# google/speedy

Hardware: AMD Instinct MI355X
Metric: Msamples/s processed (16 kHz mono, 3.5x nonlinear) (higher is better)
Workload: dtype int16 samples; f64 DFT, f32 features, int32 AMDF/OLA

## Files before the change

include/speedy_hip.h:

```cpp
#ifndef SPEEDY_HIP_H_
#define SPEEDY_HIP_H_
#include <stddef.h>
#include <stdint.h>
#ifdef __cplusplus
extern "C" {
#endif

#ifndef SPX_FEATURE_COUNT
#define SPX_FEATURE_COUNT 15
#endif

typedef struct spx_plan* spx_plan_t;

typedef struct {
  int64_t in_off;
  int64_t n_in;
  int64_t out_off;
  int64_t out_cap;
  int32_t channels;
  float speed;
  float nonlinear;
  float feedback;
} spx_stream_job;

typedef struct {
  float* tension;
  float* speed;
  float* features;
  float* spectrogram;
  float* normalized;
} spx_taps;

const char* spx_last_error(void);
int spx_abi_version(void);

spx_plan_t spx_plan_create(int sample_rate, int match_matlab);
void spx_plan_destroy(spx_plan_t plan);
int spx_plan_frame_step(spx_plan_t plan);
int spx_plan_window_size(spx_plan_t plan);
int spx_plan_fft_size(spx_plan_t plan);
int spx_plan_future(spx_plan_t plan);
int spx_plan_max_required(spx_plan_t plan);
int64_t spx_plan_frames(spx_plan_t plan, int64_t n_in);
int64_t spx_plan_out_capacity(spx_plan_t plan, int64_t n_in, float speed);
int64_t spx_plan_out_capacity_for(spx_plan_t plan, int64_t n_in, float speed, float nonlinear);

size_t spx_batch_workspace_bytes(spx_plan_t plan, const spx_stream_job* jobs, int n_streams);

int spx_batch_run(spx_plan_t plan, const spx_stream_job* jobs, int n_streams, const int16_t* in,
                  int16_t* out, int64_t* n_out, void* workspace, size_t workspace_bytes,
                  const spx_taps* taps, void* hip_stream);

int spx_batch_run_rate(spx_plan_t plan, const spx_stream_job* jobs, const float* rates, int n_streams, const int16_t* in,
                       int16_t* out, int64_t* n_out, void* workspace, size_t workspace_bytes,
                       const spx_taps* taps, void* hip_stream);
size_t spx_batch_workspace_bytes_rate(spx_plan_t plan, const spx_stream_job* jobs, const float* rates, int n_streams);
int64_t spx_plan_out_capacity_rate(spx_plan_t plan, int64_t n_in, float speed, float nonlinear, float rate);

int spx_batch_run_ahead(spx_plan_t plan, const spx_stream_job* jobs, int n_streams, const int16_t* in,
                        int16_t* out, int64_t* n_out, void* workspace, size_t workspace_bytes,
                        const spx_taps* taps, void* hip_stream);

int spx_batch_run_overlapped(spx_plan_t plan, const spx_stream_job* jobs, int n_streams, const int16_t* in,
                             int16_t* out, int64_t* n_out, void* workspace, size_t workspace_bytes,
                             const spx_taps* taps, void* hip_stream);

int spx_batch_run_ahead_when(spx_plan_t plan, const spx_stream_job* jobs, int n_streams, const int16_t* in,
                             int16_t* out, int64_t* n_out, void* workspace, size_t workspace_bytes,
                             const spx_taps* taps, void* hip_stream, void* in_ready_event);

typedef struct spx_pipeline* spx_pipeline_t;
#define SPX_PIPELINE_DEVICE_OUT 1u
spx_pipeline_t spx_pipeline_create(spx_plan_t plan, const spx_stream_job* jobs, int n_streams, int depth, unsigned flags);
spx_pipeline_t spx_pipeline_create_mixed(const spx_plan_t* plans, int n_plans, const spx_stream_job* jobs, const int* plan_index,
                                         int n_streams, int depth, unsigned flags);
void spx_pipeline_destroy(spx_pipeline_t p);
int spx_pipeline_depth(spx_pipeline_t p);
size_t spx_pipeline_input_values(spx_pipeline_t p);
int16_t* spx_pipeline_host_input(spx_pipeline_t p);
int64_t spx_pipeline_submit(spx_pipeline_t p, const int16_t* in, int in_is_device);
int spx_pipeline_input_consumed(spx_pipeline_t p, int64_t ticket);
int spx_pipeline_wait(spx_pipeline_t p, int64_t ticket, const int16_t** out, const int64_t** offsets, const int64_t** counts);
void* spx_host_alloc(size_t bytes);
void spx_host_free(void* p);

int spx_batch_analyze(spx_plan_t plan, const spx_stream_job* jobs, int n_streams, const int16_t* in,
                      void* workspace, size_t workspace_bytes, const spx_taps* taps, void* hip_stream);
int spx_batch_walk(spx_plan_t plan, const spx_stream_job* jobs, int n_streams, const int16_t* in,
                   int16_t* out, int64_t* n_out, void* workspace, size_t workspace_bytes,
                   const spx_taps* taps, void* hip_stream);

size_t spx_batch_workspace_bytes_mixed(const spx_plan_t* plans, int n_plans, const spx_stream_job* jobs,
                                       const int* plan_index, int n_streams);
int spx_batch_run_mixed(const spx_plan_t* plans, int n_plans, const spx_stream_job* jobs, const int* plan_index,
                        int n_streams, const int16_t* in, int16_t* out, int64_t* n_out, void* workspace,
                        size_t workspace_bytes, void* hip_stream);

int spx_batch_run_mixed_taps(const spx_plan_t* plans, int n_plans, const spx_stream_job* jobs, const int* plan_index,
                             int n_streams, const int16_t* in, int16_t* out, int64_t* n_out, void* workspace,
                             size_t workspace_bytes, const spx_taps* taps, void* hip_stream);
int spx_batch_run_mixed_ahead(const spx_plan_t* plans, int n_plans, const spx_stream_job* jobs, const int* plan_index,
                              int n_streams, const int16_t* in, int16_t* out, int64_t* n_out, void* workspace,
                              size_t workspace_bytes, void* hip_stream);

void spx_set_timing(int enabled);
void spx_set_pipeline_chunks(int chunks);
void spx_set_concurrent(int on);
int spx_timing_collect(double* sum_ms_analyze, double* sum_ms_walk, int* n_calls);
const char* spx_batch_kernel_names(spx_plan_t plan, int n_streams, int max_channels, int speedup_only);
const char* spx_batch_kernel_names_lean(spx_plan_t plan, int n_streams, int max_channels, int speedup_only);
int spx_debug_last_walk_form(void);
int spx_debug_kernel_vgprs(int which);
int spx_debug_walk_info(int sample_rate, int channels, int n_streams, int speedup_only, int short_jobs, int lean, int* out5);
int spx_debug_analysis_info(int sample_rate, int* out4);
int spx_debug_mode_resources(int sample_rate, int channels, int n_streams, int speedup_only, long long* out22);
long long spx_debug_fdiv_check(unsigned seed, unsigned denominators, int exp_lo, int exp_hi);
long long spx_debug_xfade_check(int n_lo, int n_hi);
long long spx_debug_arith_check(unsigned seed, unsigned threads, unsigned per_thread);
int spx_debug_log_check(unsigned first_block, unsigned end_block, unsigned long long* sums);
int spx_debug_last_call_concurrent(void);
double spx_timing_last_tension_ms(void);
double spx_timing_last_rate_ms(void);

int spx_batch_read_steps(spx_plan_t plan, const spx_stream_job* jobs, int n_streams, const void* workspace,
                         int32_t* steps, void* hip_stream);
int spx_batch_read_steps_mixed(const spx_plan_t* plans, int n_plans, const spx_stream_job* jobs, const int* plan_index,
                               int n_streams, const void* workspace, int32_t* steps, void* hip_stream);

void* spx_device_alloc(size_t bytes);
void spx_device_free(void* p);
int spx_batch_pack_outputs(const spx_stream_job* jobs, int n_streams, const int16_t* out, const int64_t* n_out,
                           int16_t* packed, int64_t* offsets, void* hip_stream);
int spx_copy_to_device(void* dst, const void* src, size_t bytes, void* hip_stream);
int spx_copy_to_host(void* dst, const void* src, size_t bytes, void* hip_stream);
int spx_stream_synchronize(void* hip_stream);

#ifdef __cplusplus
}
#endif
#endif
```

speedy_amd/_lib.py:

```python
import ctypes as C
import os
import subprocess

_HERE = os.path.dirname(os.path.abspath(__file__))
LIB_PATH = os.environ.get("SPEEDY_HIP_LIB") or os.path.join(_HERE, "lib", "libspeedy_hip.so")
_LIB = None

c_short_p = C.POINTER(C.c_short)
c_float_p = C.POINTER(C.c_float)
c_int64_p = C.POINTER(C.c_int64)


class StreamJob(C.Structure):
    _fields_ = [("in_off", C.c_int64), ("n_in", C.c_int64), ("out_off", C.c_int64), ("out_cap", C.c_int64),
                ("channels", C.c_int32), ("speed", C.c_float), ("nonlinear", C.c_float), ("feedback", C.c_float)]


class Taps(C.Structure):
    _fields_ = [("tension", C.c_void_p), ("speed", C.c_void_p), ("features", C.c_void_p),
                ("spectrogram", C.c_void_p), ("normalized", C.c_void_p)]


TENSION_FN = C.CFUNCTYPE(None, C.c_void_p, C.c_int, C.c_float)
FEATURES_FN = C.CFUNCTYPE(None, C.c_void_p, C.c_int, c_float_p)

SYMBOLS = {
    "spx_last_error": (C.c_char_p, []),
    "spx_abi_version": (C.c_int, []),
    "spx_plan_create": (C.c_void_p, [C.c_int, C.c_int]),
    "spx_plan_destroy": (None, [C.c_void_p]),
    "spx_plan_frame_step": (C.c_int, [C.c_void_p]),
    "spx_plan_window_size": (C.c_int, [C.c_void_p]),
    "spx_plan_fft_size": (C.c_int, [C.c_void_p]),
    "spx_plan_future": (C.c_int, [C.c_void_p]),
    "spx_plan_max_required": (C.c_int, [C.c_void_p]),
    "spx_plan_frames": (C.c_int64, [C.c_void_p, C.c_int64]),
    "spx_plan_out_capacity": (C.c_int64, [C.c_void_p, C.c_int64, C.c_float]),
    "spx_plan_out_capacity_for": (C.c_int64, [C.c_void_p, C.c_int64, C.c_float, C.c_float]),
    "spx_batch_workspace_bytes": (C.c_size_t, [C.c_void_p, C.POINTER(StreamJob), C.c_int]),
    "spx_batch_run": (C.c_int, [C.c_void_p, C.POINTER(StreamJob), C.c_int, C.c_void_p, C.c_void_p, C.c_void_p,
                                C.c_void_p, C.c_size_t, C.POINTER(Taps), C.c_void_p]),
    "spx_batch_run_rate": (C.c_int, [C.c_void_p, C.POINTER(StreamJob), c_float_p, C.c_int, C.c_void_p, C.c_void_p, C.c_void_p,
                                     C.c_void_p, C.c_size_t, C.POINTER(Taps), C.c_void_p]),
    "spx_batch_workspace_bytes_rate": (C.c_size_t, [C.c_void_p, C.POINTER(StreamJob), c_float_p, C.c_int]),
    "spx_plan_out_capacity_rate": (C.c_int64, [C.c_void_p, C.c_int64, C.c_float, C.c_float, C.c_float]),
    "spx_batch_run_ahead": (C.c_int, [C.c_void_p, C.POINTER(StreamJob), C.c_int, C.c_void_p, C.c_void_p, C.c_void_p,
                                      C.c_void_p, C.c_size_t, C.POINTER(Taps), C.c_void_p]),
    "spx_batch_run_overlapped": (C.c_int, [C.c_void_p, C.POINTER(StreamJob), C.c_int, C.c_void_p, C.c_void_p, C.c_void_p,
                                           C.c_void_p, C.c_size_t, C.POINTER(Taps), C.c_void_p]),
    "spx_batch_run_ahead_when": (C.c_int, [C.c_void_p, C.POINTER(StreamJob), C.c_int, C.c_void_p, C.c_void_p, C.c_void_p,
                                           C.c_void_p, C.c_size_t, C.POINTER(Taps), C.c_void_p, C.c_void_p]),
    "spx_batch_workspace_bytes_mixed": (C.c_size_t, [C.POINTER(C.c_void_p), C.c_int, C.POINTER(StreamJob), C.POINTER(C.c_int), C.c_int]),
    "spx_batch_run_mixed": (C.c_int, [C.POINTER(C.c_void_p), C.c_int, C.POINTER(StreamJob), C.POINTER(C.c_int), C.c_int,
                                      C.c_void_p, C.c_void_p, C.c_void_p, C.c_void_p, C.c_size_t, C.c_void_p]),
    "spx_batch_run_mixed_ahead": (C.c_int, [C.POINTER(C.c_void_p), C.c_int, C.POINTER(StreamJob), C.POINTER(C.c_int), C.c_int,
                                      C.c_void_p, C.c_void_p, C.c_void_p, C.c_void_p, C.c_size_t, C.c_void_p]),
    "spx_batch_run_mixed_taps": (C.c_int, [C.POINTER(C.c_void_p), C.c_int, C.POINTER(StreamJob), C.POINTER(C.c_int), C.c_int,
                                           C.c_void_p, C.c_void_p, C.c_void_p, C.c_void_p, C.c_size_t, C.POINTER(Taps), C.c_void_p]),
    "spx_batch_read_steps": (C.c_int, [C.c_void_p, C.POINTER(StreamJob), C.c_int, C.c_void_p, C.POINTER(C.c_int32), C.c_void_p]),
    "spx_batch_read_steps_mixed": (C.c_int, [C.POINTER(C.c_void_p), C.c_int, C.POINTER(StreamJob), C.POINTER(C.c_int), C.c_int,
                                             C.c_void_p, C.POINTER(C.c_int32), C.c_void_p]),
    "spx_batch_analyze": (C.c_int, [C.c_void_p, C.POINTER(StreamJob), C.c_int, C.c_void_p, C.c_void_p,
                                    C.c_size_t, C.POINTER(Taps), C.c_void_p]),
    "spx_batch_walk": (C.c_int, [C.c_void_p, C.POINTER(StreamJob), C.c_int, C.c_void_p, C.c_void_p, C.c_void_p,
                                 C.c_void_p, C.c_size_t, C.POINTER(Taps), C.c_void_p]),
    "spx_set_timing": (None, [C.c_int]),
    "spx_set_pipeline_chunks": (None, [C.c_int]),
    "spx_set_concurrent": (None, [C.c_int]),
    "spx_timing_collect": (C.c_int, [C.POINTER(C.c_double), C.POINTER(C.c_double), C.POINTER(C.c_int)]),
    "spx_timing_last_tension_ms": (C.c_double, []),
    "spx_timing_last_rate_ms": (C.c_double, []),
    "spx_batch_kernel_names": (C.c_char_p, [C.c_void_p, C.c_int, C.c_int, C.c_int]),
    "spx_batch_kernel_names_lean": (C.c_char_p, [C.c_void_p, C.c_int, C.c_int, C.c_int]),
    "spx_debug_last_walk_form": (C.c_int, []),
    "spx_debug_kernel_vgprs": (C.c_int, [C.c_int]),
    "spx_debug_last_call_concurrent": (C.c_int, []),
    "spx_debug_fdiv_check": (C.c_longlong, [C.c_uint, C.c_uint, C.c_int, C.c_int]),
    "spx_debug_xfade_check": (C.c_longlong, [C.c_int, C.c_int]),
    "spx_debug_arith_check": (C.c_longlong, [C.c_uint, C.c_uint, C.c_uint]),
    "spx_debug_log_check": (C.c_int, [C.c_uint, C.c_uint, C.POINTER(C.c_ulonglong)]),
    "spx_debug_walk_info": (C.c_int, [C.c_int, C.c_int, C.c_int, C.c_int, C.c_int, C.c_int, C.POINTER(C.c_int)]),
    "spx_debug_analysis_info": (C.c_int, [C.c_int, C.POINTER(C.c_int)]),
    "spx_debug_mode_resources": (C.c_int, [C.c_int, C.c_int, C.c_int, C.c_int, C.POINTER(C.c_longlong)]),
    "spx_pipeline_create": (C.c_void_p, [C.c_void_p, C.POINTER(StreamJob), C.c_int, C.c_int, C.c_uint]),
    "spx_pipeline_create_mixed": (C.c_void_p, [C.POINTER(C.c_void_p), C.c_int, C.POINTER(StreamJob), C.POINTER(C.c_int), C.c_int, C.c_int, C.c_uint]),
    "spx_pipeline_destroy": (None, [C.c_void_p]),
    "spx_pipeline_depth": (C.c_int, [C.c_void_p]),
    "spx_pipeline_input_values": (C.c_size_t, [C.c_void_p]),
    "spx_pipeline_host_input": (C.c_void_p, [C.c_void_p]),
    "spx_pipeline_submit": (C.c_int64, [C.c_void_p, C.c_void_p, C.c_int]),
    "spx_pipeline_input_consumed": (C.c_int, [C.c_void_p, C.c_int64]),
    "spx_pipeline_wait": (C.c_int, [C.c_void_p, C.c_int64, C.POINTER(C.c_void_p), C.POINTER(C.c_void_p), C.POINTER(C.c_void_p)]),
    "spx_host_alloc": (C.c_void_p, [C.c_size_t]),
    "spx_host_free": (None, [C.c_void_p]),
    "spx_device_alloc": (C.c_void_p, [C.c_size_t]),
    "spx_device_free": (None, [C.c_void_p]),
    "spx_copy_to_device": (C.c_int, [C.c_void_p, C.c_void_p, C.c_size_t, C.c_void_p]),
    "spx_copy_to_host": (C.c_int, [C.c_void_p, C.c_void_p, C.c_size_t, C.c_void_p]),
    "spx_batch_pack_outputs": (C.c_int, [C.c_void_p, C.c_int, C.c_void_p, C.c_void_p, C.c_void_p, C.c_void_p, C.c_void_p]),
    "spx_stream_synchronize": (C.c_int, [C.c_void_p]),
    "sonicCreateStream": (C.c_void_p, [C.c_int, C.c_int]),
    "sonicDestroyStream": (None, [C.c_void_p]),
    "sonicWriteShortToStream": (C.c_int, [C.c_void_p, c_short_p, C.c_int]),
    "sonicReadShortFromStream": (C.c_int, [C.c_void_p, c_short_p, C.c_int]),
    "sonicWriteFloatToStream": (C.c_int, [C.c_void_p, c_float_p, C.c_int]),
    "sonicReadFloatFromStream": (C.c_int, [C.c_void_p, c_float_p, C.c_int]),
    "sonicSetRate": (None, [C.c_void_p, C.c_float]),
    "sonicSetSpeed": (None, [C.c_void_p, C.c_float]),
    "sonicFlushStream": (C.c_int, [C.c_void_p]),
    "sonicEnableNonlinearSpeedup": (None, [C.c_void_p, C.c_float]),
    "sonicSetDurationFeedbackStrength": (None, [C.c_void_p, C.c_float]),
    "getSonicBufferSize": (C.c_int, [C.c_void_p]),
    "sonicSpectrogramSize": (C.c_int, [C.c_void_p]),
    "sonicTensionCallback": (None, [C.c_void_p, TENSION_FN]),
    "getSonicTensionCallback": (C.c_void_p, [C.c_void_p]),
    "sonicSpeedCallback": (None, [C.c_void_p, TENSION_FN]),
    "getSonicSpeedCallback": (C.c_void_p, [C.c_void_p]),
    "sonicFeaturesCallback": (None, [C.c_void_p, FEATURES_FN]),
    "getSonicFeaturesCallback": (C.c_void_p, [C.c_void_p]),
    "sonicSpectrogramCallback": (None, [C.c_void_p, FEATURES_FN]),
    "getSonicSpectrogramCallback": (C.c_void_p, [C.c_void_p]),
    "sonicNormalizedSpectrogramCallback": (None, [C.c_void_p, FEATURES_FN]),
    "getSonicNormalizedSpectrogramCallback": (C.c_void_p, [C.c_void_p]),
    "sonicIntGetNumChannels": (C.c_int, [C.c_void_p]),
    "sonicIntGetSampleRate": (C.c_int, [C.c_void_p]),
    "sonicIntGetSpeed": (C.c_float, [C.c_void_p]),
    "sonicIntCreateStream": (C.c_void_p, [C.c_int, C.c_int]),
    "sonicIntDestroyStream": (None, [C.c_void_p]),
    "sonicIntSetSpeed": (None, [C.c_void_p, C.c_float]),
    "sonicIntSetRate": (None, [C.c_void_p, C.c_float]),
    "sonicIntWriteShortToStream": (C.c_int, [C.c_void_p, c_short_p, C.c_int]),
    "sonicIntWriteFloatToStream": (C.c_int, [C.c_void_p, c_float_p, C.c_int]),
    "sonicIntReadShortFromStream": (C.c_int, [C.c_void_p, c_short_p, C.c_int]),
    "sonicIntReadFloatFromStream": (C.c_int, [C.c_void_p, c_float_p, C.c_int]),
    "sonicIntFlushStream": (C.c_int, [C.c_void_p]),
    "sonicIntSamplesAvailable": (C.c_int, [C.c_void_p]),
    "sonicIntSetUserData": (None, [C.c_void_p, C.c_void_p]),
    "sonicIntGetUserData": (C.c_void_p, [C.c_void_p]),
    "speedyCreateStream": (C.c_void_p, [C.c_int]),
    "speedyDestroyStream": (None, [C.c_void_p]),
    "speedyInputFrameSize": (C.c_int, [C.c_void_p]),
    "speedyInputFrameStep": (C.c_int, [C.c_void_p]),
    "speedyFFTSize": (C.c_int, [C.c_void_p]),
    "speedyBinToFreq": (C.c_float, [C.c_void_p, C.c_int]),
    "speedyFreqToBin": (C.c_int, [C.c_void_p, C.c_float]),
    "speedyAddData": (None, [C.c_void_p, c_float_p, C.c_int64]),
    "speedyAddDataShort": (None, [C.c_void_p, c_short_p, C.c_int64]),
    "speedyComputeTension": (C.c_int, [C.c_void_p, C.c_int64, c_float_p]),
    "speedyComputeSpeedFromTension": (C.c_float, [C.c_float, C.c_float, C.c_float, C.c_void_p]),
    "speedyGetCurrentTime": (C.c_int64, [C.c_void_p]),
    "speedySpectrogram": (c_float_p, [C.c_void_p, c_float_p]),
    "speedyGetSpectrogram": (c_float_p, [C.c_void_p]),
    "speedyGetSpectrogramAtTime": (c_float_p, [C.c_void_p, C.c_int64]),
    "speedyGetNormalizedSpectrogram": (c_float_p, [C.c_void_p]),
    "speedyGetInternalState": (c_float_p, [C.c_void_p]),
    "speedyGetEnergyCompressed": (C.c_float, [C.c_void_p]),
    "speedyGetSpeechChanges": (C.c_float, [C.c_void_p]),
    "speedyHipHysteresisFuture": (C.c_int, [C.c_void_p]),
    "speedyHipHysteresisPast": (C.c_int, [C.c_void_p]),
    "speedyComputeSpectralDifference": (None, [C.c_void_p, c_float_p, c_float_p, C.c_int64]),
    "speedyComputeLocalEnergy": (None, [C.c_void_p, c_float_p, C.c_int64]),
    "speedySaveSpectrogramData": (None, [C.c_void_p, c_float_p, C.c_int64]),
    "speedyPreemphasisFilter": (None, [C.c_void_p, c_float_p, C.c_int]),
    "speedyEvaluateHysteresis": (C.c_float, [C.c_void_p, C.c_int64]),
    "speedyAddToHysteresisBuffer": (None, [C.c_void_p, C.c_float, C.c_int64]),
    "speedyGetInternalSpectrogram": (c_float_p, [C.c_void_p]),
    "speedyGetInternalNormalizedSpectrogram": (c_float_p, [C.c_void_p]),
    "speedyNormalizeByEnergy": (C.c_float, [c_float_p, c_float_p, C.c_int]),
    "CreateFirstOrderFilter": (C.c_void_p, [C.c_float]),
    "DesignFirstOrderLowpassFilter": (None, [C.c_void_p, C.c_float]),
    "IterateFirstOrderFilter": (C.c_float, [C.c_void_p, C.c_float]),
    "ResetFirstOrderFilter": (None, [C.c_void_p]),
    "DeleteFirstOrderFilter": (None, [C.c_void_p]),
    "speedyHipSetMatchMatlab": (None, [C.c_int]),
    "speedyHipCreateSonicStream": (C.c_void_p, [C.c_int, C.c_int, C.c_int]),
    "speedyHipSetCoalescing": (None, [C.c_int]),
    "speedyHipGetCoalescing": (C.c_int, []),
    "speedyHipCreateSonicStreamEx": (C.c_void_p, [C.c_int, C.c_int, C.c_int, C.c_int]),
    "speedyHipPoolStats": (None, [C.POINTER(C.c_ulonglong), C.POINTER(C.c_ulonglong)]),
    "sonicSamplesAvailable": (C.c_int, [C.c_void_p]),
    "speedyHipLastError": (C.c_char_p, []),
}


def build():
    subprocess.check_call(["make", "-s", "-C", os.path.join(_HERE, "csrc")])


def lib():
    global _LIB
    if _LIB is not None:
        return _LIB
    if not os.path.exists(LIB_PATH):
        raise RuntimeError(f"{LIB_PATH} is missing: run `python -c 'import __graft_entry__ as g; g.build()'` "
                           "(the product has no CPU fallback)")
    import torch
    L = C.CDLL(LIB_PATH)
    for name, (res, args) in SYMBOLS.items():
        if os.environ.get("SPEEDY_HIP_LIB") and not hasattr(L, name):
            continue
        fn = getattr(L, name)
        fn.restype = res
        fn.argtypes = args
    _LIB = L
    return L
```

speedy_amd/csrc/spx_analysis.hip:

```cpp
#include <stdlib.h>

#include "spx_internal.h"
#include "spx_walk_common.h"

#ifndef SPX_TF
#define SPX_TF 16
#endif

#ifdef SPX_STAMPS
__device__ unsigned long long g_spx_astamps[16];
#define ASTAMP_DECL unsigned long long as_last = __builtin_readcyclecounter(), as_acc[10] = {0,0,0,0,0,0,0,0,0,0};
#define ASTAMP(i) do { const unsigned long long t_ = __builtin_readcyclecounter(); as_acc[i] += t_ - as_last; as_last = t_; } while (0)
#define ASTAMP_FLUSH if (threadIdx.x == 0 && blockIdx.x == 7) for (int i_ = 0; i_ < 10; i_++) g_spx_astamps[i_] += as_acc[i_];
extern "C" void spx_debug_astamps(unsigned long long* out, int reset) {
  (void)hipMemcpyFromSymbol(out, HIP_SYMBOL(g_spx_astamps), sizeof(unsigned long long) * 16);
  if (reset) { unsigned long long z[16] = {0}; (void)hipMemcpyToSymbol(HIP_SYMBOL(g_spx_astamps), z, sizeof(z)); }
}
#else
#define ASTAMP_DECL
#define ASTAMP(i)
#define ASTAMP_FLUSH
#endif

#ifndef SPX_TF_SMALL
#define SPX_TF_SMALL 8
#endif
#define SPX_TF_TINY 4
int spx_analysis_tile_frames() { return SPX_TF; }
int spx_analysis_small_tile_frames() { return SPX_TF_SMALL; }
int spx_analysis_tiny_tile_frames() { return SPX_TF_TINY; }

#define SPX_CB 24
static __host__ __device__ constexpr int spx_mag_stride(int W) { return (W + 4) & ~3; }
static __host__ __device__ constexpr int spx_cb(int tf) { return tf <= 8 ? 2 * SPX_CB : SPX_CB; }
#ifdef SPX_LOG_V1
#define SPX_LOG_LDS_BYTES 0
#else
#define SPX_LOG_LDS_BYTES 2048
#endif
static __host__ __device__ inline size_t terms_bytes(int W, int tf, bool ct) {
  const size_t b = ct ? (size_t)2 * tf * (spx_cb(tf) + 1) * sizeof(double)
                      : (size_t)tf * (W + 1) * sizeof(double);
  return (b + 15) & ~(size_t)15;
}
static __host__ __device__ inline size_t work_bytes(int W, int tf, bool ct = false, int dft_waves = 4) {
  if (dft_waves < 1 || dft_waves > 4) dft_waves = 4;
  const size_t a = ct ? (size_t)4 * 2 * W * sizeof(double)
                      : (size_t)dft_waves * 2 * 2 * W * sizeof(double);
  const size_t b = terms_bytes(W, tf, ct) + SPX_LOG_LDS_BYTES;
  return (a > b ? a : b);
}
static inline int plan_ct_window(const SpxPlanDev& P) {
  auto is = [](const int* r, int n, std::initializer_list<int> want) {
    if (n != (int)want.size()) return false;
    int k = 0;
    for (int w : want) if (r[k++] != w) return false;
    return true;
  };
  if (!P.rader && P.W == 240 && is(P.radix, P.nstages, {4, 4, 3, 5})) return 240;
  if (!P.rader && P.W == 330 && is(P.radix, P.nstages, {2, 3, 5, 11})) return 330;
  if (P.tile_frames == SPX_TF_SMALL && P.dft_waves == 4) {
    if (!P.rader && P.W == 720 && is(P.radix, P.nstages, {4, 4, 3, 3, 5})) return 720;
    if (P.rader && P.W == 661 && is(P.radixM, P.nstagesM, {4, 3, 5, 11})) return 661;
  }
  if (!P.rader && P.dft_waves == 4) {
    if (P.W == 120 && is(P.radix, P.nstages, {4, 2, 3, 5}) && (P.tile_frames == SPX_TF || P.tile_frames == SPX_TF_SMALL)) return 120;
    if (P.W == 180 && is(P.radix, P.nstages, {4, 3, 3, 5}) && P.tile_frames == SPX_TF) return 180;
    if (P.W == 360 && is(P.radix, P.nstages, {4, 2, 3, 3, 5}) && P.tile_frames == SPX_TF) return 360;
    if (P.W == 480 && is(P.radix, P.nstages, {4, 4, 2, 3, 5}) && P.tile_frames == SPX_TF) return 480;
  }
  return 0;
}
int spx_analysis_prefers_small_tile(const SpxPlanDev& P) {
  SpxPlanDev Q = P;
  Q.tile_frames = SPX_TF_SMALL;
  Q.dft_waves = 4;
  const int w = plan_ct_window(Q);
  return w == 720 || w == 661;
}
static __host__ __device__ inline size_t stage_samples(const SpxPlanDev& P, int tf) {
  return (size_t)(tf + 1) * P.B + (P.W - P.B) + 8;
}
static size_t analysis_lds_bytes(const SpxPlanDev& P, bool ct) {
  const int tf = P.tile_frames > 0 ? P.tile_frames : SPX_TF;
  size_t mags = (size_t)(tf + 1) * spx_mag_stride(P.W) * sizeof(float);
  size_t small = (size_t)3 * (tf + 1) * sizeof(float);
  size_t stage = (stage_samples(P, tf) * sizeof(short) + 15) & ~(size_t)15;
  return work_bytes(P.W, tf, ct, P.dft_waves) + ((mags + 15) & ~(size_t)15) + ((small + 15) & ~(size_t)15) + stage;
}
size_t spx_analysis_lds_bytes(const SpxPlanDev& P) { return analysis_lds_bytes(P, plan_ct_window(P) != 0); }
int spx_analysis_ct_window(const SpxPlanDev& P) { return plan_ct_window(P); }

__device__ __forceinline__ void wave_sync() {
  __builtin_amdgcn_fence(__ATOMIC_RELEASE, "wavefront");
  __builtin_amdgcn_wave_barrier();
  __builtin_amdgcn_fence(__ATOMIC_ACQUIRE, "wavefront");
}

#include "spx_log.h"

__device__ __forceinline__ float spx_untangle_mag(double ar, double ai, double b_r, double b_i, double2 w) {
  const double dr = ar - b_r, di = ai - b_i;
#ifdef SPX_DFT_V1
  const double er = 0.5 * (ar + b_r), ei = 0.5 * (ai + b_i);
  const double o_r = 0.5 * di, o_i = -0.5 * dr;
  const double xr = er + (w.x * o_r - w.y * o_i);
  const double xi = ei + (w.x * o_i + w.y * o_r);
  return spx_sqrt64_to_f32(xr * xr + xi * xi);
#else
  const double xr2 = __builtin_fma(w.x, di, __builtin_fma(w.y, dr, ar + b_r));
  const double xi2 = __builtin_fma(w.y, di, __builtin_fma(-w.x, dr, ai + b_i));
  return spx_sqrt64_to_f32(0.25 * __builtin_fma(xr2, xr2, xi2 * xi2));
#endif
}

#define C5_1 0.30901699437494742
#define C5_2 (-0.80901699437494742)
#define S5_1 0.95105651629515357
#define S5_2 0.58778525229247313
#define S3_1 0.86602540378443865

struct cplx {
  double r, i;
};

#ifdef SPX_DFT_V1
#define SPX_FMA_OR(a, b, c, unfused) (unfused)
#else
#define SPX_FMA_OR(a, b, c, unfused) __builtin_fma((a), (b), (c))
#endif
__host__ __device__ __forceinline__ cplx spx_cmul(cplx b, double wx, double wy) {
  return {SPX_FMA_OR(b.r, wx, -(b.i * wy), b.r * wx - b.i * wy), SPX_FMA_OR(b.r, wy, b.i * wx, b.r * wy + b.i * wx)};
}
__host__ __device__ __forceinline__ double spx_bf3h(double a0, double t1) { return SPX_FMA_OR(-0.5, t1, a0, a0 - 0.5 * t1); }
__host__ __device__ __forceinline__ double spx_bf5m(double a0, double c1, double t1, double c2, double t2) {
  return SPX_FMA_OR(c2, t2, __builtin_fma(c1, t1, a0), (a0 + c1 * t1) + c2 * t2);
}
__host__ __device__ __forceinline__ double spx_bf5n(double s1, double t3, double s2, double t4) { return SPX_FMA_OR(s1, t3, s2 * t4, s1 * t3 + s2 * t4); }
__host__ __device__ __forceinline__ double spx_bf5d(double s2, double t3, double s1, double t4) { return SPX_FMA_OR(s2, t3, -(s1 * t4), s2 * t3 - s1 * t4); }
__host__ __device__ __forceinline__ double spx_acc(double p, double w, double u) { return SPX_FMA_OR(w, u, p, p + w * u); }

__host__ __device__ __forceinline__ cplx ld(const double* buf, int idx) {
  const double2 v = *reinterpret_cast<const double2*>(buf + 2 * idx);
  return {v.x, v.y};
}
__host__ __device__ __forceinline__ void st_tw(double* buf, int idx, cplx b, const double* tw, int t) {
  const double2 w = *reinterpret_cast<const double2*>(tw + 2 * t);
  const cplx v = spx_cmul(b, w.x, w.y);
  *reinterpret_cast<double2*>(buf + 2 * idx) = make_double2(v.r, v.i);
}

__host__ __device__ void dft_stage(const int W, const double* tw, int r, int s, int cur, const double* x, double* y,
                                   int lane, const int nl) {
  const int m = cur / r;
  const int span = W / r;
  const unsigned inv_s = ((1u << 20) + (unsigned)s - 1u) / (unsigned)s;
  if (r == 4) {
    for (int b = lane; b < span; b += nl) {
      const int p = (int)(((unsigned)b * inv_s) >> 20), q = b - p * s;
      cplx a0 = ld(x, b), a1 = ld(x, b + span), a2 = ld(x, b + 2 * span), a3 = ld(x, b + 3 * span);
      cplx t0 = {a0.r + a2.r, a0.i + a2.i}, t1 = {a0.r - a2.r, a0.i - a2.i};
      cplx t2 = {a1.r + a3.r, a1.i + a3.i}, t3 = {a1.r - a3.r, a1.i - a3.i};
      cplx b0 = {t0.r + t2.r, t0.i + t2.i}, b2 = {t0.r - t2.r, t0.i - t2.i};
      cplx b1 = {t1.r + t3.i, t1.i - t3.r}, b3 = {t1.r - t3.i, t1.i + t3.r};
      const int o = q + s * 4 * p;
      const int tp = s * p;
      st_tw(y, o, b0, tw, 0);
      st_tw(y, o + s, b1, tw, tp);
      st_tw(y, o + 2 * s, b2, tw, 2 * tp);
      st_tw(y, o + 3 * s, b3, tw, 3 * tp);
    }
  } else if (r == 2) {
    for (int b = lane; b < span; b += nl) {
      const int p = (int)(((unsigned)b * inv_s) >> 20), q = b - p * s;
      cplx a0 = ld(x, b), a1 = ld(x, b + span);
      cplx b0 = {a0.r + a1.r, a0.i + a1.i}, b1 = {a0.r - a1.r, a0.i - a1.i};
      const int o = q + s * 2 * p;
      st_tw(y, o, b0, tw, 0);
      st_tw(y, o + s, b1, tw, s * p);
    }
  } else if (r == 3) {
    for (int b = lane; b < span; b += nl) {
      const int p = (int)(((unsigned)b * inv_s) >> 20), q = b - p * s;
      cplx a0 = ld(x, b), a1 = ld(x, b + span), a2 = ld(x, b + 2 * span);
      cplx t1 = {a1.r + a2.r, a1.i + a2.i};
      cplx t2 = {spx_bf3h(a0.r, t1.r), spx_bf3h(a0.i, t1.i)};
      cplx t3 = {S3_1 * (a1.r - a2.r), S3_1 * (a1.i - a2.i)};
      cplx b0 = {a0.r + t1.r, a0.i + t1.i};
      cplx b1 = {t2.r + t3.i, t2.i - t3.r}, b2 = {t2.r - t3.i, t2.i + t3.r};
      const int o = q + s * 3 * p;
      const int tp = s * p;
      st_tw(y, o, b0, tw, 0);
      st_tw(y, o + s, b1, tw, tp);
      st_tw(y, o + 2 * s, b2, tw, 2 * tp);
    }
  } else if (r == 5) {
    for (int b = lane; b < span; b += nl) {
      const int p = (int)(((unsigned)b * inv_s) >> 20), q = b - p * s;
      cplx a0 = ld(x, b), a1 = ld(x, b + span), a2 = ld(x, b + 2 * span), a3 = ld(x, b + 3 * span),
           a4 = ld(x, b + 4 * span);
      cplx t1 = {a1.r + a4.r, a1.i + a4.i}, t2 = {a2.r + a3.r, a2.i + a3.i};
      cplx t3 = {a1.r - a4.r, a1.i - a4.i}, t4 = {a2.r - a3.r, a2.i - a3.i};
      cplx b0 = {(a0.r + t1.r) + t2.r, (a0.i + t1.i) + t2.i};
      cplx m1 = {spx_bf5m(a0.r, C5_1, t1.r, C5_2, t2.r), spx_bf5m(a0.i, C5_1, t1.i, C5_2, t2.i)};
      cplx m2 = {spx_bf5m(a0.r, C5_2, t1.r, C5_1, t2.r), spx_bf5m(a0.i, C5_2, t1.i, C5_1, t2.i)};
      cplx n1 = {spx_bf5n(S5_1, t3.r, S5_2, t4.r), spx_bf5n(S5_1, t3.i, S5_2, t4.i)};
      cplx n2 = {spx_bf5d(S5_2, t3.r, S5_1, t4.r), spx_bf5d(S5_2, t3.i, S5_1, t4.i)};
      cplx b1 = {m1.r + n1.i, m1.i - n1.r}, b4 = {m1.r - n1.i, m1.i + n1.r};
      cplx b2 = {m2.r + n2.i, m2.i - n2.r}, b3 = {m2.r - n2.i, m2.i + n2.r};
      const int o = q + s * 5 * p;
      const int tp = s * p;
      st_tw(y, o, b0, tw, 0);
      st_tw(y, o + s, b1, tw, tp);
      st_tw(y, o + 2 * s, b2, tw, 2 * tp);
      st_tw(y, o + 3 * s, b3, tw, 3 * tp);
      st_tw(y, o + 4 * s, b4, tw, 4 * tp);
    }
  } else {
    const int step = W / r;
    const int h = (r - 1) >> 1;
    for (int item = lane; item < span * h; item += nl) {
      const int b = item / h, j = item - b * h + 1;
      const int p = (int)(((unsigned)b * inv_s) >> 20), q = b - p * s;
      const cplx a0 = ld(x, b);
      cplx P = a0, Q = {0.0, 0.0}, B0 = a0;
      int t = 0;
      for (int i = 1; i <= h; i++) {
        t += j;
        t -= (t >= r) ? r : 0;
        const cplx ai = ld(x, b + i * span), ar = ld(x, b + (r - i) * span);
        const cplx u = {ai.r + ar.r, ai.i + ar.i}, v = {ai.r - ar.r, ai.i - ar.i};
        const double2 w = *reinterpret_cast<const double2*>(tw + 2 * (t * step));
        B0.r = B0.r + u.r; B0.i = B0.i + u.i;
        P.r = spx_acc(P.r, w.x, u.r); P.i = spx_acc(P.i, w.x, u.i);
        if (i == 1) { Q.r = w.y * v.r; Q.i = w.y * v.i; }
        else { Q.r = spx_acc(Q.r, w.y, v.r); Q.i = spx_acc(Q.i, w.y, v.i); }
      }
      const cplx bj = {P.r - Q.i, P.i + Q.r}, brj = {P.r + Q.i, P.i - Q.r};
      const int o = q + s * r * p;
      st_tw(y, o + s * j, bj, tw, s * p * j);
      st_tw(y, o + s * (r - j), brj, tw, s * p * (r - j));
      if (j == 1) st_tw(y, o, B0, tw, 0);
    }
  }
  (void)m;
}

void spx_host_dft(int n, const int* radix, int nstages, const double* tw, const double* in, double* out) {
  double* a = new double[4 * (size_t)n];
  double* x = a;
  double* y = a + 2 * (size_t)n;
  for (int i = 0; i < 2 * n; i++) x[i] = in[i];
  int s = 1, cur = n;
  for (int st = 0; st < nstages; st++) {
    dft_stage(n, tw, radix[st], s, cur, x, y, 0, 1);
    double* t = x; x = y; y = t;
    s *= radix[st];
    cur /= radix[st];
  }
  for (int i = 0; i < 2 * n; i++) out[i] = x[i];
  delete[] a;
}

__device__ __forceinline__ int mono_sample(const int16_t* __restrict__ in, int64_t a, int C) {
  if (C == 1) return in[a];
  int sum = 0;
  const int16_t* p = in + a * C;
  for (int c = 0; c < C; c++) sum += p[c];
  return sum / C;
}

__device__ __forceinline__ cplx cmul_tw(cplx b, double2 w) { return spx_cmul(b, w.x, w.y); }
__device__ __forceinline__ void st(double* buf, int idx, cplx v) {
  *reinterpret_cast<double2*>(buf + 2 * idx) = make_double2(v.r, v.i);
}

template <int R>
__device__ __forceinline__ void ct_bfly(const cplx (&a)[R], cplx (&o)[R]) {
  static_assert(R == 2 || R == 3 || R == 4 || R == 5, "fixed-formula radices");
  if constexpr (R == 2) {
    o[0] = {a[0].r + a[1].r, a[0].i + a[1].i};
    o[1] = {a[0].r - a[1].r, a[0].i - a[1].i};
  } else if constexpr (R == 3) {
    const cplx t1 = {a[1].r + a[2].r, a[1].i + a[2].i};
    const cplx t2 = {spx_bf3h(a[0].r, t1.r), spx_bf3h(a[0].i, t1.i)};
    const cplx t3 = {S3_1 * (a[1].r - a[2].r), S3_1 * (a[1].i - a[2].i)};
    o[0] = {a[0].r + t1.r, a[0].i + t1.i};
    o[1] = {t2.r + t3.i, t2.i - t3.r};
    o[2] = {t2.r - t3.i, t2.i + t3.r};
  } else if constexpr (R == 4) {
    const cplx t0 = {a[0].r + a[2].r, a[0].i + a[2].i}, t1 = {a[0].r - a[2].r, a[0].i - a[2].i};
    const cplx t2 = {a[1].r + a[3].r, a[1].i + a[3].i}, t3 = {a[1].r - a[3].r, a[1].i - a[3].i};
    o[0] = {t0.r + t2.r, t0.i + t2.i};
    o[2] = {t0.r - t2.r, t0.i - t2.i};
    o[1] = {t1.r + t3.i, t1.i - t3.r};
    o[3] = {t1.r - t3.i, t1.i + t3.r};
  } else {
    const cplx t1 = {a[1].r + a[4].r, a[1].i + a[4].i}, t2 = {a[2].r + a[3].r, a[2].i + a[3].i};
    const cplx t3 = {a[1].r - a[4].r, a[1].i - a[4].i}, t4 = {a[2].r - a[3].r, a[2].i - a[3].i};
    o[0] = {(a[0].r + t1.r) + t2.r, (a[0].i + t1.i) + t2.i};
    const cplx m1 = {spx_bf5m(a[0].r, C5_1, t1.r, C5_2, t2.r), spx_bf5m(a[0].i, C5_1, t1.i, C5_2, t2.i)};
    const cplx m2 = {spx_bf5m(a[0].r, C5_2, t1.r, C5_1, t2.r), spx_bf5m(a[0].i, C5_2, t1.i, C5_1, t2.i)};
    const cplx n1 = {spx_bf5n(S5_1, t3.r, S5_2, t4.r), spx_bf5n(S5_1, t3.i, S5_2, t4.i)};
    const cplx n2 = {spx_bf5d(S5_2, t3.r, S5_1, t4.r), spx_bf5d(S5_2, t3.i, S5_1, t4.i)};
    o[1] = {m1.r + n1.i, m1.i - n1.r};
    o[4] = {m1.r - n1.i, m1.i + n1.r};
    o[2] = {m2.r + n2.i, m2.i - n2.r};
    o[3] = {m2.r - n2.i, m2.i + n2.r};
  }
}

template <int W> struct ct_plan { static constexpr int n = 0; };
template <> struct ct_plan<120> { static constexpr int n = 4; static constexpr int r[4] = {4, 2, 3, 5}; };
template <> struct ct_plan<180> { static constexpr int n = 4; static constexpr int r[4] = {4, 3, 3, 5}; };
template <> struct ct_plan<360> { static constexpr int n = 5; static constexpr int r[5] = {4, 2, 3, 3, 5}; };
template <> struct ct_plan<480> { static constexpr int n = 5; static constexpr int r[5] = {4, 4, 2, 3, 5}; };
template <> struct ct_plan<720> { static constexpr int n = 5; static constexpr int r[5] = {4, 4, 3, 3, 5}; };

template <int NPTS, int R, int S, class Load>
__device__ __forceinline__ void ct_stage(double* buf, const double2* __restrict__ twp, const int lane, Load load) {
  constexpr int SPAN = NPTS / R, NP = (SPAN + 63) / 64;
  constexpr bool LAST = (S * R == NPTS);
  cplx a[NP][R];
#pragma unroll
  for (int u = 0; u < NP; u++) {
#pragma unroll
    for (int i = 0; i < R; i++) a[u][i] = load(u, i);
  }
  wave_sync();
#pragma unroll
  for (int u = 0; u < NP; u++) {
    const int b = lane + 64 * u;
    if (b < SPAN) {
      cplx o[R];
      ct_bfly<R>(a[u], o);
      const int p = b / S, q = b - p * S;
      const int base = q + S * R * p, tp = S * p;
      st(buf, base, o[0]);
#pragma unroll
      for (int j = 1; j < R; j++) st(buf, base + j * S, LAST ? o[j] : cmul_tw(o[j], twp[j * tp]));
    }
  }
  wave_sync();
}
template <int NPTS, int R>
struct ct_from_buf {
  const double* buf;
  int lane;
  __device__ __forceinline__ cplx operator()(int u, int i) const {
    constexpr int SPAN = NPTS / R;
    const int b = (lane + 64 * u < SPAN) ? lane + 64 * u : 0;
    return ld(buf, b + i * SPAN);
  }
};

template <int W, int ST, int S>
__device__ __forceinline__ void ct_stages_from(double* buf, const double2* __restrict__ twp, const int lane) {
  if constexpr (ST < ct_plan<W>::n) {
    constexpr int R = ct_plan<W>::r[ST];
    ct_stage<W, R, S>(buf, twp, lane, ct_from_buf<W, R>{buf, lane});
    ct_stages_from<W, ST + 1, S * R>(buf, twp, lane);
  }
}

template <int NPTS, int R>
__device__ __forceinline__ void ct_stage_prime_last(double* buf, const int lane, const double (&wc)[R - 1], const double (&ws)[R - 1]) {
  constexpr int SPAN = NPTS / R, H = (R - 1) / 2;
  static_assert(SPAN <= 64, "one pass");
  if (lane < SPAN) {
    cplx a[R];
#pragma unroll
    for (int i = 0; i < R; i++) a[i] = ld(buf, lane + SPAN * i);
    cplx uu[H], vv[H];
    cplx B0 = a[0];
#pragma unroll
    for (int i = 1; i <= H; i++) {
      uu[i - 1] = {a[i].r + a[R - i].r, a[i].i + a[R - i].i};
      vv[i - 1] = {a[i].r - a[R - i].r, a[i].i - a[R - i].i};
      B0.r = B0.r + uu[i - 1].r; B0.i = B0.i + uu[i - 1].i;
    }
    st(buf, lane, B0);
#pragma unroll
    for (int jj = 1; jj <= H; jj++) {
      cplx Pj = a[0], Qj = {0.0, 0.0};
#pragma unroll
      for (int i = 1; i <= H; i++) {
        const double wx = wc[(i * jj) % R - 1], wy = ws[(i * jj) % R - 1];
        Pj.r = spx_acc(Pj.r, wx, uu[i - 1].r); Pj.i = spx_acc(Pj.i, wx, uu[i - 1].i);
        if (i == 1) { Qj.r = wy * vv[0].r; Qj.i = wy * vv[0].i; }
        else { Qj.r = spx_acc(Qj.r, wy, vv[i - 1].r); Qj.i = spx_acc(Qj.i, wy, vv[i - 1].i); }
      }
      st(buf, lane + SPAN * jj, cplx{Pj.r - Qj.i, Pj.i + Qj.r});
      st(buf, lane + SPAN * (R - jj), cplx{Pj.r + Qj.i, Pj.i - Qj.r});
    }
  }
  wave_sync();
}

template <class T>
__device__ __forceinline__ const T* per_frame(const T* p) {
  asm volatile("" : "+s"(p));
  return p;
}
__device__ __forceinline__ double uniform_f64(double v) {
  return __longlong_as_double(((long long)__builtin_amdgcn_readfirstlane((int)(__double_as_longlong(v) >> 32)) << 32) |
                              (unsigned)__builtin_amdgcn_readfirstlane((int)__double_as_longlong(v)));
}

#ifdef SPX_PREEMPH_V1
#define SPX_WIN_SCALE 1.0f
__device__ __forceinline__ float spx_preemph_win_f32(double md, double mpd, float w) {
  const float x = (float)(md / 32768.0), xp = (float)(mpd / 32768.0);
  const float y = (float)(1.0 * (double)x - 0.97 * (double)xp);
  return y * w;
}
#else
#define SPX_WIN_SCALE 0x1p-15f
__device__ __forceinline__ float spx_preemph_win_f32(double md, double mpd, float w15) {
  const float yy = (float)(md - 0.97 * mpd);
  return yy * w15;
}
#endif
__device__ __forceinline__ double spx_preemph_win(double md, double mpd, float w) { return (double)spx_preemph_win_f32(md, mpd, w); }
__device__ __forceinline__ cplx packed_point(const short* fr, int n, int j, int prev0, float w0, float w1) {
  const int i0 = 2 * n;
  const int m0 = fr[i0], m1 = fr[i0 + 1];
  const int mp0 = (i0 > 0) ? (int)fr[i0 - 1] : ((j > 0) ? (int)fr[prev0] : 0);
  const double d0 = (double)m0;
  return {spx_preemph_win(d0, (double)mp0, w0 * SPX_WIN_SCALE), spx_preemph_win((double)m1, d0, w1 * SPX_WIN_SCALE)};
}

#ifndef SPX_AN_W_330
#define SPX_AN_W_330 3
#endif
#ifndef SPX_AN_W_BIG
#define SPX_AN_W_BIG 2
#endif
template <int TF, int WCT>
__global__ void __launch_bounds__(SPX_BLOCK, (WCT == 240 || WCT == 120 || WCT == 180) ? 4 : WCT == 330 ? SPX_AN_W_330 : (WCT == 661 || WCT == 720) ? SPX_AN_W_BIG : (WCT == 480 || WCT == 360) ? 2 : 1)
spx_analysis_kernel(SpxPlanDev P, const SpxStreamDev* __restrict__ streams, int n_streams,
                    const int16_t* __restrict__ in_base, SpxFrameRec* __restrict__ rec, SpxTapsDev taps,
                    const int* __restrict__ tile_order, int* tile_flags, const float* __restrict__ frames,
                    int frame_mode) {
  extern __shared__ __attribute__((aligned(16))) unsigned char lds[];
  const int W = WCT ? WCT : P.W, B = P.B, N = 2 * W;
  const int tid = threadIdx.x, lane = tid & 63, wave = tid >> 6;

  const int tile = tile_order ? tile_order[blockIdx.x] : (int)blockIdx.x;
  int lo = 0, hi = n_streams - 1;
  while (lo < hi) {
    int mid = (lo + hi + 1) >> 1;
    if (streams[mid].first_tile <= tile) lo = mid; else hi = mid - 1;
  }
  const SpxStreamDev S = streams[lo];
  const int T = S.n_frames;
  const int j0 = S.frame_begin + (tile - S.first_tile) * TF;
  const int j1 = min(j0 + TF, T);
  const int C = S.channels;
  const int16_t* __restrict__ in = in_base + S.in_off;

  double* work = reinterpret_cast<double*>(lds);
  const size_t wb = work_bytes(W, TF, WCT != 0, (WCT != 0) ? 4 : P.dft_waves);
  float* mags = reinterpret_cast<float*>(lds + wb);
  const size_t mags_b = (((size_t)(TF + 1) * spx_mag_stride(W) * sizeof(float)) + 15) & ~(size_t)15;
  float* fE = reinterpret_cast<float*>(lds + wb + mags_b);
  float* fThr = fE + (TF + 1);
  float* fInv = fThr + (TF + 1);
  const int MS = spx_mag_stride(W);

  const size_t small_b = (((size_t)3 * (TF + 1) * sizeof(float)) + 15) & ~(size_t)15;
  const double* ltw = P.tw;
  const double* ltw2 = P.tw2;
  short* smono = reinterpret_cast<short*>(lds + wb + mags_b + small_b);

  double* bufA = work + (size_t)wave * (WCT != 0 ? 2 : 4) * W;
  double* bufB = (WCT != 0) ? bufA : bufA + 2 * W;

  const int jfirst = (j0 > 0) ? j0 - 1 : 0;
  const int64_t sbase = (int64_t)jfirst * B;
  const int nstage = (j1 - jfirst) * B + (W - B);
  if (frames != nullptr) {
  } else if (C == 1) {
    const int16_t* __restrict__ src = in + sbase;
    for (int k0 = tid; k0 < nstage; k0 += 8 * SPX_BLOCK) {
      short v[8];
#pragma unroll
      for (int u = 0; u < 8; u++) { const int k = k0 + u * SPX_BLOCK; v[u] = (k < nstage) ? src[k] : (short)0; }
#pragma unroll
      for (int u = 0; u < 8; u++) { const int k = k0 + u * SPX_BLOCK; if (k < nstage) smono[k] = v[u]; }
    }
  } else {
    for (int k = tid; k < nstage; k += SPX_BLOCK) smono[k] = (short)mono_sample(in, sbase + k, C);
  }
  __syncthreads();

  ASTAMP_DECL
  if constexpr (WCT == 240) {
    const double2* twp = reinterpret_cast<const double2*>(P.tw);
    const double2* tw2p = reinterpret_cast<const double2*>(P.tw2);
    const int b = lane;
    const bool on60 = b < 60, on48 = b < 48;
    const int bb = on60 ? b : 0;
    double2 w1[3], w2[3], w3[2][2], wu[4];
    float wn[4];
#pragma unroll
    for (int j = 1; j < 4; j++) { w1[j - 1] = twp[bb * j]; w2[j - 1] = twp[4 * (bb >> 2) * j]; }
#pragma unroll
    for (int u = 0; u < 2; u++) {
      const int b3 = lane + 64 * u, p3 = (b3 < 80) ? (b3 >> 4) : 0;
      w3[u][0] = twp[16 * p3];
      w3[u][1] = twp[32 * p3];
    }
#pragma unroll
    for (int u = 0; u < 4; u++) { const int k = lane + 64 * u; wu[u] = tw2p[k < 240 ? k : 0]; }
    wn[0] = P.window[2 * bb]; wn[1] = P.window[2 * bb + 1]; wn[2] = P.window[2 * bb + 120]; wn[3] = P.window[2 * bb + 121];
#pragma unroll
    for (int k = 0; k < 4; k++) wn[k] *= SPX_WIN_SCALE;
    for (int s = wave; s <= TF; s += 4) {
      const int j = j0 - 1 + s;
      float* mrow = mags + (size_t)s * MS;
      if (j < 0 || j >= j1) {
        for (int k = lane; k < 240; k += SPX_WAVE) mrow[k] = 0.0f;
        continue;
      }
      const short* fr = smono + (size_t)(j - jfirst) * B;
      if (on60) {
        const int i0 = 2 * b, i1 = 2 * b + 120;
        const int m0 = fr[i0], m1 = fr[i0 + 1], m2 = fr[i1], m3 = fr[i1 + 1];
        const int mp0 = (i0 > 0) ? (int)fr[i0 - 1] : ((j > 0) ? (int)fr[(240 - B) - 1] : 0);
        const int mp2 = fr[i1 - 1];
        const double d0 = (double)m0, d2 = (double)m2;
        const cplx a0 = {spx_preemph_win(d0, (double)mp0, wn[0]), spx_preemph_win((double)m1, d0, wn[1])},
                   a1 = {spx_preemph_win(d2, (double)mp2, wn[2]), spx_preemph_win((double)m3, d2, wn[3])};
        const cplx b0 = {a0.r + a1.r, a0.i + a1.i}, b2 = {a0.r - a1.r, a0.i - a1.i};
        const cplx b1 = {a0.r + a1.i, a0.i - a1.r}, b3 = {a0.r - a1.i, a0.i + a1.r};
        st(bufA, 4 * b, b0);
        st(bufA, 4 * b + 1, cmul_tw(b1, w1[0]));
        st(bufA, 4 * b + 2, cmul_tw(b2, w1[1]));
        st(bufA, 4 * b + 3, cmul_tw(b3, w1[2]));
      }
      wave_sync();
      ASTAMP(0);
      if (on60) {
        const cplx a0 = ld(bufA, b), a1 = ld(bufA, b + 60), a2 = ld(bufA, b + 120), a3 = ld(bufA, b + 180);
        wave_sync();
        const cplx t0 = {a0.r + a2.r, a0.i + a2.i}, t1 = {a0.r - a2.r, a0.i - a2.i};
        const cplx t2 = {a1.r + a3.r, a1.i + a3.i}, t3 = {a1.r - a3.r, a1.i - a3.i};
        const cplx b0 = {t0.r + t2.r, t0.i + t2.i}, b2 = {t0.r - t2.r, t0.i - t2.i};
        const cplx b1 = {t1.r + t3.i, t1.i - t3.r}, b3 = {t1.r - t3.i, t1.i + t3.r};
        const int o = (b & 3) + 16 * (b >> 2);
        st(bufB, o, b0);
        st(bufB, o + 4, cmul_tw(b1, w2[0]));
        st(bufB, o + 8, cmul_tw(b2, w2[1]));
        st(bufB, o + 12, cmul_tw(b3, w2[2]));
      }
      wave_sync();
      {
        cplx q0[2], q1[2], q2[2];
#pragma unroll
        for (int u = 0; u < 2; u++) {
          const int b3i = (lane + 64 * u < 80) ? lane + 64 * u : 0;
          q0[u] = ld(bufB, b3i); q1[u] = ld(bufB, b3i + 80); q2[u] = ld(bufB, b3i + 160);
        }
        wave_sync();
#pragma unroll
        for (int u = 0; u < 2; u++) {
          const int b3i = lane + 64 * u;
          if (b3i < 80) {
            const cplx a0 = q0[u], a1 = q1[u], a2 = q2[u];
            const cplx t1 = {a1.r + a2.r, a1.i + a2.i};
            const cplx t2 = {spx_bf3h(a0.r, t1.r), spx_bf3h(a0.i, t1.i)};
            const cplx t3 = {S3_1 * (a1.r - a2.r), S3_1 * (a1.i - a2.i)};
            const cplx b0 = {a0.r + t1.r, a0.i + t1.i};
            const cplx b1 = {t2.r + t3.i, t2.i - t3.r}, b2 = {t2.r - t3.i, t2.i + t3.r};
            const int o = (b3i & 15) + 48 * (b3i >> 4);
            st(bufA, o, b0);
            st(bufA, o + 16, cmul_tw(b1, w3[u][0]));
            st(bufA, o + 32, cmul_tw(b2, w3[u][1]));
          }
        }
      }
      wave_sync();
      if (on48) {
        const cplx a0 = ld(bufA, b), a1 = ld(bufA, b + 48), a2 = ld(bufA, b + 96), a3 = ld(bufA, b + 144),
                   a4 = ld(bufA, b + 192);
        wave_sync();
        const cplx t1 = {a1.r + a4.r, a1.i + a4.i}, t2 = {a2.r + a3.r, a2.i + a3.i};
        const cplx t3 = {a1.r - a4.r, a1.i - a4.i}, t4 = {a2.r - a3.r, a2.i - a3.i};
        const cplx b0 = {(a0.r + t1.r) + t2.r, (a0.i + t1.i) + t2.i};
        const cplx m1 = {spx_bf5m(a0.r, C5_1, t1.r, C5_2, t2.r), spx_bf5m(a0.i, C5_1, t1.i, C5_2, t2.i)};
        const cplx m2 = {spx_bf5m(a0.r, C5_2, t1.r, C5_1, t2.r), spx_bf5m(a0.i, C5_2, t1.i, C5_1, t2.i)};
        const cplx n1 = {spx_bf5n(S5_1, t3.r, S5_2, t4.r), spx_bf5n(S5_1, t3.i, S5_2, t4.i)};
        const cplx n2 = {spx_bf5d(S5_2, t3.r, S5_1, t4.r), spx_bf5d(S5_2, t3.i, S5_1, t4.i)};
        const cplx b1 = {m1.r + n1.i, m1.i - n1.r}, b4 = {m1.r - n1.i, m1.i + n1.r};
        const cplx b2 = {m2.r + n2.i, m2.i - n2.r}, b3 = {m2.r - n2.i, m2.i + n2.r};
        st(bufB, b, b0);
        st(bufB, b + 48, b1);
        st(bufB, b + 96, b2);
        st(bufB, b + 144, b3);
        st(bufB, b + 192, b4);
      }
      wave_sync();
      ASTAMP(1);
      float* spec_out = taps.spectrogram ? taps.spectrogram + (size_t)(S.frame_off + j) * 480 : nullptr;
#pragma unroll
      for (int u = 0; u < 4; u++) {
        const int k = lane + 64 * u;
        if (k < 240) {
          const int k2 = (k == 0) ? 0 : 240 - k;
          const cplx a = ld(bufB, k), c = ld(bufB, k2);
          const double b_r = c.r, b_i = -c.i;
          const float mag = spx_untangle_mag(a.r, a.i, b_r, b_i, wu[u]);
          mrow[k] = mag;
          if (spec_out) {
            spec_out[k] = mag;
            if (k > 0) spec_out[480 - k] = mag;
            else spec_out[240] = (float)__builtin_fabs(a.r - a.i);
          }
        }
      }
      wave_sync();
      ASTAMP(2);
    }
  } else if constexpr (WCT == 330) {
    const double2* twp = reinterpret_cast<const double2*>(P.tw);
    const double2* tw2p = reinterpret_cast<const double2*>(P.tw2);
    double2 w1[3], w2[2][2];
    float wn[3][2];
#pragma unroll
    for (int u = 0; u < 3; u++) {
      const int b1 = (lane + 64 * u < 165) ? lane + 64 * u : 0;
      w1[u] = twp[b1];
      wn[u][0] = P.window[2 * b1] * SPX_WIN_SCALE; wn[u][1] = P.window[2 * b1 + 1] * SPX_WIN_SCALE;
    }
#pragma unroll
    for (int u = 0; u < 2; u++) {
      const int p2 = (lane + 64 * u < 110) ? ((lane + 64 * u) >> 1) : 0;
      w2[u][0] = twp[2 * p2];
      w2[u][1] = twp[4 * p2];
    }
    double wc[10], ws[10];
#pragma unroll
    for (int k = 1; k <= 10; k++) {
      const double2 w = twp[k * 30];
      wc[k - 1] = __longlong_as_double(((long long)__builtin_amdgcn_readfirstlane((int)(__double_as_longlong(w.x) >> 32)) << 32) |
                                       (unsigned)__builtin_amdgcn_readfirstlane((int)__double_as_longlong(w.x)));
      ws[k - 1] = __longlong_as_double(((long long)__builtin_amdgcn_readfirstlane((int)(__double_as_longlong(w.y) >> 32)) << 32) |
                                       (unsigned)__builtin_amdgcn_readfirstlane((int)__double_as_longlong(w.y)));
    }
    for (int s = wave; s <= TF; s += 4) {
      const int j = j0 - 1 + s;
      float* mrow = mags + (size_t)s * MS;
      if (j < 0 || j >= j1) {
        for (int k = lane; k < 330; k += SPX_WAVE) mrow[k] = 0.0f;
        continue;
      }
      const short* fr = smono + (size_t)(j - jfirst) * B;
#pragma unroll
      for (int u = 0; u < 3; u++) {
        const int b = lane + 64 * u;
        if (b < 165) {
          const int i0 = 2 * b;
          const int m0 = fr[i0], m1 = fr[i0 + 1];
          const int mp0 = (i0 > 0) ? (int)fr[i0 - 1] : ((j > 0) ? (int)fr[(330 - B) - 1] : 0);
          const double d0 = (double)m0;
          const cplx a0 = {spx_preemph_win(d0, (double)mp0, wn[u][0]), spx_preemph_win((double)m1, d0, wn[u][1])};
          st(bufA, 2 * b, a0);
          st(bufA, 2 * b + 1, cmul_tw(a0, w1[u]));
        }
      }
      wave_sync();
      ASTAMP(0);
      {
        cplx q0[2], q1[2], q2[2];
#pragma unroll
        for (int u = 0; u < 2; u++) {
          const int b = (lane + 64 * u < 110) ? lane + 64 * u : 0;
          q0[u] = ld(bufA, b); q1[u] = ld(bufA, b + 110); q2[u] = ld(bufA, b + 220);
        }
        wave_sync();
#pragma unroll
        for (int u = 0; u < 2; u++) {
          const int b = lane + 64 * u;
          if (b < 110) {
            const cplx a0 = q0[u], a1 = q1[u], a2 = q2[u];
            const cplx t1 = {a1.r + a2.r, a1.i + a2.i};
            const cplx t2 = {spx_bf3h(a0.r, t1.r), spx_bf3h(a0.i, t1.i)};
            const cplx t3 = {S3_1 * (a1.r - a2.r), S3_1 * (a1.i - a2.i)};
            const cplx b0 = {a0.r + t1.r, a0.i + t1.i};
            const cplx b1 = {t2.r + t3.i, t2.i - t3.r}, b2 = {t2.r - t3.i, t2.i + t3.r};
            const int o = (b & 1) + 6 * (b >> 1);
            st(bufA, o, b0);
            st(bufA, o + 2, cmul_tw(b1, w2[u][0]));
            st(bufA, o + 4, cmul_tw(b2, w2[u][1]));
          }
        }
      }
      wave_sync();
      {
        cplx q[2][5];
#pragma unroll
        for (int u = 0; u < 2; u++) {
          const int b = (lane + 64 * u < 66) ? lane + 64 * u : 0;
#pragma unroll
          for (int i = 0; i < 5; i++) q[u][i] = ld(bufA, b + 66 * i);
        }
        wave_sync();
#pragma unroll
        for (int u = 0; u < 2; u++) {
          const int b = lane + 64 * u;
          if (b < 66) {
            const cplx a0 = q[u][0], a1 = q[u][1], a2 = q[u][2], a3 = q[u][3], a4 = q[u][4];
            const cplx t1 = {a1.r + a4.r, a1.i + a4.i}, t2 = {a2.r + a3.r, a2.i + a3.i};
            const cplx t3 = {a1.r - a4.r, a1.i - a4.i}, t4 = {a2.r - a3.r, a2.i - a3.i};
            const cplx b0 = {(a0.r + t1.r) + t2.r, (a0.i + t1.i) + t2.i};
            const cplx m1 = {spx_bf5m(a0.r, C5_1, t1.r, C5_2, t2.r), spx_bf5m(a0.i, C5_1, t1.i, C5_2, t2.i)};
            const cplx m2 = {spx_bf5m(a0.r, C5_2, t1.r, C5_1, t2.r), spx_bf5m(a0.i, C5_2, t1.i, C5_1, t2.i)};
            const cplx n1 = {spx_bf5n(S5_1, t3.r, S5_2, t4.r), spx_bf5n(S5_1, t3.i, S5_2, t4.i)};
            const cplx n2 = {spx_bf5d(S5_2, t3.r, S5_1, t4.r), spx_bf5d(S5_2, t3.i, S5_1, t4.i)};
            const cplx b1 = {m1.r + n1.i, m1.i - n1.r}, b4 = {m1.r - n1.i, m1.i + n1.r};
            const cplx b2 = {m2.r + n2.i, m2.i - n2.r}, b3 = {m2.r - n2.i, m2.i + n2.r};
            const int p = (int)(((unsigned)b * 10923u) >> 16);
            const int o = (b - 6 * p) + 30 * p, tp = 6 * p;
            st(bufA, o, b0);
            st(bufA, o + 6, cmul_tw(b1, twp[tp]));
            st(bufA, o + 12, cmul_tw(b2, twp[2 * tp]));
            st(bufA, o + 18, cmul_tw(b3, twp[3 * tp]));
            st(bufA, o + 24, cmul_tw(b4, twp[4 * tp]));
          }
        }
      }
      wave_sync();
      if (lane < 30) {
        cplx a[11];
#pragma unroll
        for (int i = 0; i < 11; i++) a[i] = ld(bufA, lane + 30 * i);
        cplx u5[5], v5[5];
        cplx B0 = a[0];
#pragma unroll
        for (int i = 1; i <= 5; i++) {
          u5[i - 1] = {a[i].r + a[11 - i].r, a[i].i + a[11 - i].i};
          v5[i - 1] = {a[i].r - a[11 - i].r, a[i].i - a[11 - i].i};
          B0.r = B0.r + u5[i - 1].r; B0.i = B0.i + u5[i - 1].i;
        }
        st(bufA, lane, B0);
#pragma unroll
// ... 248 lines not shown
            const double2 b = *reinterpret_cast<const double2*>(P.bfft + 2 * k);
            const cplx cc = spx_cmul(a, b.x, b.y);
            *reinterpret_cast<double2*>(x + 2 * k) = make_double2(cc.r, -cc.i);
          }
          wave_sync();
        }
      }
      const double inv = 1.0 / (double)M;
      const double* abuf = (P.nstagesM & 1) ? y : x;
      const cplx A0 = ld(abuf, M);
      wave_sync();
      for (int q = lane; q < M; q += SPX_WAVE) {
        const cplx c = ld(x, q);
        const double cr = c.r * inv, ci = -c.i * inv;
        *reinterpret_cast<double2*>(y + 2 * P.iperm[q]) = make_double2(x0.r + cr, x0.i + ci);
      }
      if (lane == 0) *reinterpret_cast<double2*>(y) = make_double2(x0.r + A0.r, x0.i + A0.i);
      wave_sync();
      { double* t = x; x = y; y = t; }
    } else {
      int sprod = 1, cur = W;
      for (int stg = 0; stg < P.nstages; stg++) {
        const int r = P.radix[stg];
        dft_stage(W, ltw, r, sprod, cur, x, y, lane, SPX_WAVE);
        wave_sync();
        double* t = x; x = y; y = t;
        sprod *= r;
        cur /= r;
      }
    }
    ASTAMP(1);
    float* spec_out = taps.spectrogram ? taps.spectrogram + (size_t)(S.frame_off + j) * N : nullptr;
    for (int k = lane; k < W; k += SPX_WAVE) {
      const int k2 = (k == 0) ? 0 : W - k;
      cplx a = ld(x, k), bb = ld(x, k2);
      const double b_r = bb.r, b_i = -bb.i;
      const float mag = spx_untangle_mag(a.r, a.i, b_r, b_i, *reinterpret_cast<const double2*>(ltw2 + 2 * k));
      mrow[k] = mag;
      if (spec_out) {
        spec_out[k] = mag;
        if (k > 0) spec_out[N - k] = mag;
        else spec_out[W] = (float)__builtin_fabs(a.r - a.i);
      }
    }
    wave_sync();
    ASTAMP(2);
  }
  ASTAMP(3);
  __syncthreads();
  ASTAMP(4);

  if (wave > 0) {
#ifdef SPX_ROWMAX_V1
    for (int s = wave - 1; s <= TF; s += 3) {
      const float* mrow = mags + (size_t)s * MS;
      float mx = 0.0f;
      for (int i = 1 + lane; i < W; i += SPX_WAVE) mx = fmaxf(mx, mrow[i]);
#pragma unroll
      for (int d = 32; d >= 1; d >>= 1) mx = fmaxf(mx, __shfl_xor(mx, d));
      if (lane == 0) fThr[s] = (float)((double)mx / 100.0);
    }
#else
    unsigned keep = 0u;
    int nrows = 0;
    for (int s = wave - 1; s <= TF; s += 3, nrows++) {
      const unsigned* mrow = reinterpret_cast<const unsigned*>(mags + (size_t)s * MS);
      unsigned m = 0u;
      for (int q = lane; 4 * q < W; q += SPX_WAVE) {
        const uint4 v = *reinterpret_cast<const uint4*>(mrow + 4 * q);
        const unsigned a = (q == 0) ? 0u : v.x;
        const unsigned b = (4 * q + 1 < W) ? v.y : 0u, c = (4 * q + 2 < W) ? v.z : 0u, d = (4 * q + 3 < W) ? v.w : 0u;
        const unsigned ab = a > b ? a : b, cd = c > d ? c : d;
        const unsigned abcd = ab > cd ? ab : cd;
        m = m > abcd ? m : abcd;
      }
      const float mx = wave_max_f(__builtin_bit_cast(float, m));
      if (lane == nrows) keep = __builtin_bit_cast(unsigned, mx);
    }
    if (lane < nrows) fThr[wave - 1 + 3 * lane] = (float)((double)__builtin_bit_cast(float, keep) / 100.0);
#endif
#ifndef SPX_LOG_V1
    if (tid < SPX_WAVE + 128)
      reinterpret_cast<uint4*>(reinterpret_cast<unsigned char*>(work) + terms_bytes(W, TF, WCT != 0))[tid - SPX_WAVE] =
          reinterpret_cast<const uint4*>(spx_log_table_dev)[tid - SPX_WAVE];
#endif
  } else if (tid <= TF) {
    const float4* r4 = reinterpret_cast<const float4*>(mags + (size_t)tid * MS);
    float e = 0.0f;
    __builtin_amdgcn_s_setprio(3);
    auto acc8 = [&](const float4& p, const float4& q) {
      const float4 pp = {p.x * p.x, p.y * p.y, p.z * p.z, p.w * p.w}, qq = {q.x * q.x, q.y * q.y, q.z * q.z, q.w * q.w};
      e += pp.x; e += pp.y; e += pp.z; e += pp.w;
      e += qq.x; e += qq.y; e += qq.z; e += qq.w;
    };
    {
      const float4 h = r4[0];
      if (1 < W) e += h.y * h.y;
      if (2 < W) e += h.z * h.z;
      if (3 < W) e += h.w * h.w;
    }
    int i = 4;
    float4 c0 = r4[1], c1 = r4[2], c2 = r4[3], c3 = r4[4];
#pragma unroll 1
    for (; i + 16 <= W; i += 16) {
      const float4 n0 = r4[(i >> 2) + 4], n1 = r4[(i >> 2) + 5], n2 = r4[(i >> 2) + 6], n3 = r4[(i >> 2) + 7];
      __builtin_amdgcn_sched_barrier(0);
      acc8(c0, c1);
      acc8(c2, c3);
      c0 = n0; c1 = n1; c2 = n2; c3 = n3;
    }
    {
      const float t[16] = {c0.x, c0.y, c0.z, c0.w, c1.x, c1.y, c1.z, c1.w, c2.x, c2.y, c2.z, c2.w, c3.x, c3.y, c3.z, c3.w};
#pragma unroll
      for (int u = 0; u < 16; u++)
        if (i + u < W) e += t[u] * t[u];
    }
    __builtin_amdgcn_s_setprio(0);
    const float eps = 2.2204e-16f;
    fE[tid] = e;
    fInv[tid] = (float)(1.0 / (__builtin_sqrt((double)e) + (double)eps));
  }
  __syncthreads();
  ASTAMP(5);

  const int nfr = j1 - j0;
#ifndef SPX_LOG_V1
  const SpxLogEntry* ltab = reinterpret_cast<const SpxLogEntry*>(reinterpret_cast<const unsigned char*>(work) + terms_bytes(W, TF, WCT != 0));
  auto log_of_ratio = [&](float ratio) -> double {
    double v = spx_log_v2_f32(ratio, ltab);
    if (__builtin_expect(!spx_log_v2_domain(ratio), 0)) v = spx_log_v1((double)ratio);
    return v;
  };
#else
  auto log_of_ratio = [&](float ratio) -> double { return spx_log_v1((double)ratio); };
#endif
  auto log_term = [&](int f, int i) -> double {
    const int sl = f + 1;
    const float cur = mags[(size_t)sl * MS + i], last = mags[(size_t)(sl - 1) * MS + i];
    const float thr = fThr[sl];
    double term = 0.0;
    if (cur > thr && last > thr) {
      const float eps = 2.2204e-16f;
      const float nc = cur * fInv[sl], nl = last * fInv[sl - 1];
      const float ratio = spx_fdiv32(nc + eps, nl + eps);
      term = __builtin_fabs(log_of_ratio(ratio));
    }
    return term;
  };
  auto write_rec = [&](int f, float lsd) {
    const float lowthr = (float)(0.04 * (double)1.41421f);
    const float e = fE[f + 1];
    SpxFrameRec r;
    r.energy = e;
    r.lsd = (e <= lowthr) ? 0.0f : lsd;
    rec[S.frame_off + j0 + f] = r;
  };
  if (taps.normalized) {
    for (int idx = tid; idx < nfr * W; idx += SPX_BLOCK) {
      const int f = idx / W, i = idx - f * W;
      const int j = j0 + f;
      const int row = j + (S.unit_time0 ? 0 : 1);
      if (row < T + (S.unit_time0 ? 1 : 0))
        taps.normalized[(size_t)(S.frame_off + row) * W + i] = mags[(size_t)(f + 1) * MS + i] * fInv[f + 1];
    }
    if (S.unit_time0) {
    } else if (j0 == 0) {
      for (int i = tid; i < W; i += SPX_BLOCK) taps.normalized[(size_t)S.frame_off * W + i] = 0.0f;
    } else if (j0 == S.frame_begin) {
      for (int i = tid; i < W; i += SPX_BLOCK)
        taps.normalized[(size_t)(S.frame_off + j0) * W + i] = mags[i] * fInv[0];
    }
  }
  if constexpr (WCT != 0) {
    constexpr int CB = spx_cb(TF);
    constexpr int CBS = CB + 1;
    static_assert(TF * CB == 2 * (SPX_BLOCK - SPX_WAVE), "two terms per lane of waves 1..3 and block");
    double* tblk = work;
    constexpr int NBLK = (WCT - 1 + CB - 1) / CB;
    float lsd = 0.0f;
    int fi[2], ci[2];
    bool ok[2];
#ifndef SPX_TERMS_V1
    const float* rowc[2];
    const float* rowl[2];
    float thrv[2], invc[2], invl[2];
#endif
#pragma unroll
    for (int t = 0; t < 2; t++) {
      const int it = tid - SPX_WAVE + t * (SPX_BLOCK - SPX_WAVE);
      fi[t] = wave > 0 ? it / CB : 0;
      ci[t] = wave > 0 ? it - fi[t] * CB : 0;
      ok[t] = wave > 0 && fi[t] < nfr;
#ifndef SPX_TERMS_V1
      const int fl = ok[t] ? fi[t] : 0;
      rowc[t] = mags + (size_t)(fl + 1) * MS;
      rowl[t] = mags + (size_t)fl * MS;
      thrv[t] = fThr[fl + 1];
      invc[t] = fInv[fl + 1];
      invl[t] = fInv[fl];
#endif
    }
    for (int k = 0; k <= NBLK; k++) {
      if (wave > 0) {
        if (k < NBLK) {
          double* tb = tblk + (size_t)(k & 1) * TF * CBS;
          bool gate[2];
          float xr[2];
#pragma unroll
          for (int t = 0; t < 2; t++) {
            const int i = 1 + k * CB + ci[t];
            const bool in = ok[t] && i < WCT;
#ifdef SPX_TERMS_V1
            const int fl = in ? fi[t] : 0, il = in ? i : 1;
            const float cur = mags[(size_t)(fl + 1) * MS + il], last = mags[(size_t)fl * MS + il];
            const float thr = fThr[fl + 1];
            const float fic = fInv[fl + 1], fil = fInv[fl];
#else
            const int il = (i < WCT) ? i : 1;
            const float cur = rowc[t][il], last = rowl[t][il];
            const float thr = thrv[t], fic = invc[t], fil = invl[t];
#endif
            gate[t] = in && cur > thr && last > thr;
            const float eps = 2.2204e-16f;
            const float nc = cur * fic, nl = last * fil;
            const float ratio = spx_fdiv32(nc + eps, nl + eps);
            xr[t] = gate[t] ? ratio : 2.0f;
          }
#ifdef SPX_LOG_V1
          const spx_log_parts p0 = spx_log_main((double)xr[0]), p1 = spx_log_main((double)xr[1]);
          const double t0 = gate[0] ? __builtin_fabs(spx_log_finish(p0, (double)xr[0])) : 0.0;
          const double t1 = gate[1] ? __builtin_fabs(spx_log_finish(p1, (double)xr[1])) : 0.0;
#else
          const double l0 = log_of_ratio(xr[0]), l1 = log_of_ratio(xr[1]);
          const double t0 = gate[0] ? __builtin_fabs(l0) : 0.0;
          const double t1 = gate[1] ? __builtin_fabs(l1) : 0.0;
#endif
          if (ok[0]) tb[fi[0] * CBS + ci[0]] = t0;
          if (ok[1]) tb[fi[1] * CBS + ci[1]] = t1;
        }
      } else if (k > 0 && tid < nfr) {
        const double* tb = tblk + (size_t)((k - 1) & 1) * TF * CBS + tid * CBS;
        const int i0 = 1 + (k - 1) * CB;
        __builtin_amdgcn_s_setprio(3);
        (void)i0;
        static_assert(CB % 8 == 0, "batches of eight");
        double tv[8];
#pragma unroll
        for (int u = 0; u < 8; u++) tv[u] = tb[u];
#pragma unroll
        for (int c = 0; c < CB; c += 8) {
          double nx[8];
          if (c + 8 < CB) {
#pragma unroll
            for (int u = 0; u < 8; u++) nx[u] = tb[c + 8 + u];
          }
#pragma unroll
          for (int u = 0; u < 8; u++) lsd = (float)((double)lsd + tv[u]);
          if (c + 8 < CB) {
#pragma unroll
            for (int u = 0; u < 8; u++) tv[u] = nx[u];
          }
        }
        __builtin_amdgcn_s_setprio(0);
      }
      ASTAMP(6);
      __syncthreads();
      ASTAMP(7);
    }
    if (tid < nfr) write_rec(tid, lsd);
  } else {
  double* terms = work;
  for (int idx = tid; idx < nfr * (W - 1); idx += SPX_BLOCK) {
    const int f = idx / (W - 1);
    const int i = 1 + (idx - f * (W - 1));
    terms[(size_t)f * (W + 1) + i] = log_term(f, i);
  }
  __syncthreads();
  ASTAMP(6);

  if (tid < nfr) {
    const double* trow = terms + (size_t)tid * (W + 1);
    float lsd = 0.0f;
    int i = 1;
    for (; i + 8 <= W; i += 8) {
      double tv[8];
#pragma unroll
      for (int u = 0; u < 8; u++) tv[u] = trow[i + u];
#pragma unroll
      for (int u = 0; u < 8; u++) lsd = (float)((double)lsd + tv[u]);
    }
    for (; i < W; i++) lsd = (float)((double)lsd + trow[i]);
    write_rec(tid, lsd);
  }
  }
  if (tile_flags) {
    asm volatile("s_waitcnt vmcnt(0)" ::: "memory");
    __syncthreads();
    if (tid == 0) {
      __builtin_amdgcn_fence(__ATOMIC_RELEASE, "agent");
      asm volatile("s_waitcnt vmcnt(0)" ::: "memory");
      __hip_atomic_store(&tile_flags[tile], 1, __ATOMIC_RELAXED, __HIP_MEMORY_SCOPE_AGENT);
    }
  }
  ASTAMP(7);
  ASTAMP_FLUSH
}

__global__ void spx_arith_check_kernel(unsigned seed, unsigned per_thread, unsigned long long* bad) {
  unsigned long long st = (unsigned long long)seed * 0x9E3779B97F4A7C15ull + (blockIdx.x * blockDim.x + threadIdx.x) * 0xD1B54A32D192ED03ull + 1;
  auto next = [&]() { st ^= st >> 12; st ^= st << 25; st ^= st >> 27; return st * 0x2545F4914F6CDD1Dull; };
  unsigned long long miss = 0;
  for (unsigned i = 0; i < per_thread; i++) {
    const unsigned long long a = next(), b = next(), c = next();
    const float fn = __uint_as_float((unsigned)((127 - 53 + (a % 57)) << 23) | (unsigned)((a >> 8) & 0x7fffff));
    const float fd = __uint_as_float((unsigned)((127 - 53 + (b % 57)) << 23) | (unsigned)((b >> 8) & 0x7fffff));
    if (__float_as_uint(spx_fdiv32(fn, fd)) != __float_as_uint(fn / fd)) miss++;
    const long long fb = ((long long)(1023 - 21 + (c % 20)) << 52) | (long long)((c >> 8) & 0xfffffffffffffll) | ((c >> 63) ? (1ll << 63) : 0);
    const double f = __longlong_as_double(fb);
    if (__double_as_longlong(spx_fdiv64(f, 2.0 + f)) != __double_as_longlong(f / (2.0 + f))) miss++;
    const long long xb = ((long long)(1023 - 800 + (a >> 33) % 1811) << 52) | (long long)((b >> 10) & 0xfffffffffffffll);
    const double x = ((c & 1023) == 0) ? 0.0 : __longlong_as_double(xb);
    if (__float_as_uint(spx_sqrt64_to_f32(x)) != __float_as_uint((float)__builtin_sqrt(x))) miss++;
  }
  if (miss) atomicAdd(bad, miss);
}
extern "C" long long spx_debug_arith_check(unsigned seed, unsigned threads, unsigned per_thread) {
  unsigned long long* d = nullptr;
  unsigned long long h = 0;
  if (hipMalloc(&d, sizeof(h)) != hipSuccess) return -1;
  if (hipMemcpy(d, &h, sizeof(h), hipMemcpyHostToDevice) != hipSuccess) { (void)hipFree(d); return -1; }
  const unsigned blocks = (threads + 255) / 256;
  hipLaunchKernelGGL(spx_arith_check_kernel, dim3(blocks), dim3(256), 0, nullptr, seed, per_thread, d);
  const bool ok = hipDeviceSynchronize() == hipSuccess && hipMemcpy(&h, d, sizeof(h), hipMemcpyDeviceToHost) == hipSuccess;
  (void)hipFree(d);
  return ok ? (long long)h : -1;
}

__global__ void __launch_bounds__(256) spx_log_check_kernel(unsigned first_block, unsigned long long* __restrict__ sums) {
#ifndef SPX_LOG_V1
  __shared__ SpxLogEntry tab[128];
  __shared__ unsigned long long acc;
  if (threadIdx.x < 128) reinterpret_cast<uint4*>(tab)[threadIdx.x] = reinterpret_cast<const uint4*>(spx_log_table_dev)[threadIdx.x];
  if (threadIdx.x == 0) acc = 0;
  __syncthreads();
  const unsigned b = first_block + blockIdx.x;
  unsigned long long sum = 0;
  for (unsigned i = threadIdx.x; i < (1u << 20); i += 256) {
    const float x = __uint_as_float((b << 20) | i);
    sum += (unsigned long long)__double_as_longlong(spx_log_v2_f32(x, tab));
  }
  atomicAdd(&acc, sum);
  __syncthreads();
  if (threadIdx.x == 0) sums[b] = acc;
#endif
}
extern "C" int spx_debug_log_check(unsigned first_block, unsigned end_block, unsigned long long* sums) {
#ifdef SPX_LOG_V1
  (void)first_block; (void)end_block; (void)sums;
  return -3;
#else
  if (first_block < 8) first_block = 8;
  if (end_block > 2040) end_block = 2040;
  if (!sums || first_block >= end_block) return -1;
  unsigned long long* d = nullptr;
  if (hipMalloc(&d, 2040 * sizeof(unsigned long long)) != hipSuccess) return -1;
  bool ok = hipMemset(d, 0, 2040 * sizeof(unsigned long long)) == hipSuccess;
  if (ok) hipLaunchKernelGGL(spx_log_check_kernel, dim3(end_block - first_block), dim3(256), 0, nullptr, first_block, d);
  ok = ok && hipDeviceSynchronize() == hipSuccess && hipMemcpy(sums, d, 2040 * sizeof(unsigned long long), hipMemcpyDeviceToHost) == hipSuccess;
  (void)hipFree(d);
  return ok ? 0 : -1;
#endif
}

void spx_launch_analysis(const SpxPlanDev& P, const SpxStreamDev* streams, int n_streams, int n_tiles,
                         const int16_t* in, SpxFrameRec* rec, SpxTapsDev taps, const int* tile_order, int* tile_flags,
                         hipStream_t st) {
  if (n_tiles <= 0) return;
  const size_t lds = spx_analysis_lds_bytes(P);
  const int ctw = plan_ct_window(P);
#define SPX_LAUNCH_ANALYSIS(TFV, WV)                                                                                   \
  hipLaunchKernelGGL((spx_analysis_kernel<TFV, WV>), dim3(n_tiles), dim3(SPX_BLOCK), lds, st, P, streams, n_streams, in, \
                     rec, taps, tile_order, tile_flags, (const float*)nullptr, 0)
  if (P.tile_frames == SPX_TF_TINY) {
    SPX_LAUNCH_ANALYSIS(SPX_TF_TINY, 0);
  } else if (P.tile_frames == SPX_TF_SMALL) {
    if (ctw == 240) SPX_LAUNCH_ANALYSIS(SPX_TF_SMALL, 240); else if (ctw == 330) SPX_LAUNCH_ANALYSIS(SPX_TF_SMALL, 330);
    else if (ctw == 720) SPX_LAUNCH_ANALYSIS(SPX_TF_SMALL, 720); else if (ctw == 661) SPX_LAUNCH_ANALYSIS(SPX_TF_SMALL, 661);
    else if (ctw == 120) SPX_LAUNCH_ANALYSIS(SPX_TF_SMALL, 120);
    else SPX_LAUNCH_ANALYSIS(SPX_TF_SMALL, 0);
  } else {
    if (ctw == 240) SPX_LAUNCH_ANALYSIS(SPX_TF, 240); else if (ctw == 330) SPX_LAUNCH_ANALYSIS(SPX_TF, 330);
    else if (ctw == 120) SPX_LAUNCH_ANALYSIS(SPX_TF, 120); else if (ctw == 360) SPX_LAUNCH_ANALYSIS(SPX_TF, 360);
    else if (ctw == 180) SPX_LAUNCH_ANALYSIS(SPX_TF, 180);
    else if (ctw == 480) SPX_LAUNCH_ANALYSIS(SPX_TF, 480);
    else SPX_LAUNCH_ANALYSIS(SPX_TF, 0);
  }
#undef SPX_LAUNCH_ANALYSIS
}

int spx_analysis_vgprs(const SpxPlanDev& P, int* scratch_bytes) {
  const int ctw = plan_ct_window(P);
  const bool small = P.tile_frames == SPX_TF_SMALL;
  const void* fn;
#define SPX_AN_FN(TFV, WV) reinterpret_cast<const void*>(spx_analysis_kernel<TFV, WV>)
  if (P.tile_frames == SPX_TF_TINY) fn = SPX_AN_FN(SPX_TF_TINY, 0);
  else if (small) fn = ctw == 240 ? SPX_AN_FN(SPX_TF_SMALL, 240) : ctw == 330 ? SPX_AN_FN(SPX_TF_SMALL, 330)
                     : ctw == 720 ? SPX_AN_FN(SPX_TF_SMALL, 720) : ctw == 661 ? SPX_AN_FN(SPX_TF_SMALL, 661)
                     : ctw == 120 ? SPX_AN_FN(SPX_TF_SMALL, 120) : SPX_AN_FN(SPX_TF_SMALL, 0);
  else fn = ctw == 240 ? SPX_AN_FN(SPX_TF, 240) : ctw == 330 ? SPX_AN_FN(SPX_TF, 330) : ctw == 120 ? SPX_AN_FN(SPX_TF, 120)
          : ctw == 360 ? SPX_AN_FN(SPX_TF, 360) : ctw == 480 ? SPX_AN_FN(SPX_TF, 480) : ctw == 180 ? SPX_AN_FN(SPX_TF, 180)
          : SPX_AN_FN(SPX_TF, 0);
#undef SPX_AN_FN
  return spx_kernel_vgprs(fn, scratch_bytes);
}

void spx_launch_analysis_frames(const SpxPlanDev& P, const SpxStreamDev* streams, int n_tiles, const float* frames,
                                bool preemph, SpxFrameRec* rec, SpxTapsDev taps, hipStream_t st) {
  if (n_tiles <= 0) return;
  SpxPlanDev Q = P;
  if (Q.tile_frames != SPX_TF_SMALL && Q.tile_frames != SPX_TF_TINY) Q.tile_frames = SPX_TF;
  const size_t lds = analysis_lds_bytes(Q, false);
  if (Q.tile_frames == SPX_TF_TINY)
    hipLaunchKernelGGL((spx_analysis_kernel<SPX_TF_TINY, 0>), dim3(n_tiles), dim3(SPX_BLOCK), lds, st, Q, streams, 1,
                       (const int16_t*)nullptr, rec, taps, (const int*)nullptr, (int*)nullptr, frames, preemph ? 1 : 2);
  else if (Q.tile_frames == SPX_TF_SMALL)
    hipLaunchKernelGGL((spx_analysis_kernel<SPX_TF_SMALL, 0>), dim3(n_tiles), dim3(SPX_BLOCK), lds, st, Q, streams, 1,
                       (const int16_t*)nullptr, rec, taps, (const int*)nullptr, (int*)nullptr, frames, preemph ? 1 : 2);
  else
    hipLaunchKernelGGL((spx_analysis_kernel<SPX_TF, 0>), dim3(n_tiles), dim3(SPX_BLOCK), lds, st, Q, streams, 1,
                       (const int16_t*)nullptr, rec, taps, (const int*)nullptr, (int*)nullptr, frames, preemph ? 1 : 2);
}
```

speedy_amd/csrc/spx_diag.hip:

```cpp
#include "spx_engine.h"

extern "C" {
static const char* kernel_names(spx_plan_t plan, int n_streams, int max_channels, int speedup_only, bool lean);
const char* spx_batch_kernel_names(spx_plan_t plan, int n_streams, int max_channels, int speedup_only) {
  return kernel_names(plan, n_streams, max_channels, speedup_only, false);
}
const char* spx_batch_kernel_names_lean(spx_plan_t plan, int n_streams, int max_channels, int speedup_only) {
  return kernel_names(plan, n_streams, max_channels, speedup_only, true);
}
static const char* kernel_names(spx_plan_t plan, int n_streams, int max_channels, int speedup_only, bool lean) {
  static thread_local char buf[256];
  const SpxPlanDev& d = plan->dev;
  const SpxWalkConfig c = spx_walk_config(d, n_streams, max_channels < 1 ? 1 : max_channels, speedup_only != 0, false, lean, speedup_only == 0);
  char walk[96];
  if (c.fast_kernel && c.slow)
    snprintf(walk, sizeof(walk), "spx_walk_fast_kernel<%d, %d, 0, 0, %d>", c.nwm, c.nwc, max_channels > 1 ? 3 : 2);
  else if (c.fast_kernel)
    {
      const bool ct_rate = d.rate == 16000 || d.rate == 22050;
      const bool lng = ct_rate && c.nwm == 4 && c.nwc == 4 && c.wcap == 8192;
      snprintf(walk, sizeof(walk), "spx_walk_fast_kernel<%d, %d, %d, %d, %d>", c.nwm, c.nwc,
               (ct_rate && (lng || c.wcap == ((c.nwc == 0 && c.nwm <= 2) ? 1536 : 4096))) ? d.rate : 0, lng ? 1 : 0, max_channels > 1 ? 1 : 0);
    }
  else
    snprintf(walk, sizeof(walk), "spx_walk_kernel<%d, %d>", c.nw, c.mode);
  snprintf(buf, sizeof(buf), "spx_analysis_kernel<%d, %d>;spx_tension_kernel;%s", d.tile_frames, spx_analysis_ct_window(d), walk);
  return buf;
}

int spx_debug_last_call_concurrent(void) { return g_last_concurrent.load(std::memory_order_relaxed); }
int spx_debug_kernel_vgprs(int which) {
  if (which == 0) return spx_tension_vgprs();
  const int rate = (which == 2 || which == 4) ? 22050 : 16000;
  const SpxPlanDev* P = spx_internal_shared_plan(rate, 0);
  if (!P) return -1;
  switch (which) {
    case 1: return spx_walk_vgprs(*P, 256, 1, true, false);
    case 2: return spx_walk_vgprs(*P, 256, 1, true, true);
    case 3: case 4: return spx_analysis_vgprs(*P);
    case 5: return spx_walk_vgprs(*P, 256, 2, true, false);
    default: return -1;
  }
}

int spx_debug_walk_info(int sample_rate, int channels, int n_streams, int speedup_only, int short_jobs, int lean, int* out) {
  const SpxPlanDev* P = spx_internal_shared_plan(sample_rate, 0);
  if (!P || !out) return -1;
  const SpxWalkConfig c = spx_walk_config(*P, n_streams, channels < 1 ? 1 : channels, speedup_only != 0, short_jobs != 0, lean != 0, speedup_only == 0);
  int scratch = -1;
  out[0] = spx_walk_kernel_regs(*P, n_streams, channels, speedup_only != 0, short_jobs != 0, lean != 0, &scratch, speedup_only == 0);
  out[1] = scratch;
  out[2] = (int)c.lds;
  out[3] = c.fast_kernel ? 16 * c.nwm + c.nwc : 0;
  out[4] = c.waves;
  return 0;
}
int spx_debug_analysis_info(int sample_rate, int* out) {
  const SpxPlanDev* P = spx_internal_shared_plan(sample_rate, 0);
  if (!P || !out) return -1;
  int scratch = -1;
  out[0] = spx_analysis_vgprs(*P, &scratch);
  out[1] = scratch;
  out[2] = (int)spx_analysis_lds_bytes(*P);
  out[3] = P->dft_waves;
  return 0;
}

void spx_set_timing(int enabled) { g_timing = enabled != 0; }
void spx_set_concurrent(int on) { g_concurrent = on != 0; }
void spx_set_pipeline_chunks(int chunks) { g_chunks_set = true; g_chunks = chunks < 1 ? 1 : (chunks > SPX_MAX_CHUNKS ? SPX_MAX_CHUNKS : chunks); }
static double g_last_tension_ms = 0.0, g_last_rate_ms = 0.0;
double spx_timing_last_tension_ms(void) { return g_last_tension_ms; }
double spx_timing_last_rate_ms(void) { return g_last_rate_ms; }
int spx_timing_collect(double* sum_ms_analyze, double* sum_ms_walk, int* n_calls) {
  std::lock_guard<std::mutex> g(g_tmu);
  double a = 0, w = 0, t = 0, r = 0;
  for (auto& ev : g_ev_pending) {
    HIPCHK(hipEventSynchronize(ev.b));
    float ms = 0;
    HIPCHK(hipEventElapsedTime(&ms, ev.a, ev.b));
    if (ev.kind == 0) a += ms; else if (ev.kind == 1) w += ms; else if (ev.kind == 3) r += ms; else t += ms;
    g_ev_free.push_back(ev.a);
    g_ev_free.push_back(ev.b);
  }
  g_ev_pending.clear();
  g_last_tension_ms = t;
  g_last_rate_ms = r;
  if (sum_ms_analyze) *sum_ms_analyze = a;
  if (sum_ms_walk) *sum_ms_walk = w;
  if (n_calls) *n_calls = g_calls_pending;
  g_calls_pending = 0;
  return 0;
}

void* spx_device_alloc(size_t bytes) {
  void* p = nullptr;
  if (hipMalloc(&p, bytes ? bytes : 1) != hipSuccess) { fail(-2, "spx_device_alloc failed"); return nullptr; }
  return p;
}
void spx_device_free(void* p) { if (p) (void)hipFree(p); }
int spx_copy_to_device(void* dst, const void* src, size_t bytes, void* hs) {
  HIPCHK(hipMemcpyAsync(dst, src, bytes, hipMemcpyHostToDevice, static_cast<hipStream_t>(hs)));
  return 0;
}
}

__global__ void __launch_bounds__(256)
spx_pack_offsets_kernel(const int64_t* __restrict__ n_out, const int* __restrict__ channels,
                        const int64_t* __restrict__ caps, int n, int64_t* __restrict__ offsets) {
  __shared__ int64_t sh[256];
  __shared__ int64_t carry;
  const int t = threadIdx.x;
  if (t == 0) carry = 0;
  __syncthreads();
  for (int i0 = 0; i0 < n; i0 += 256) {
    const int i = i0 + t;
    int64_t v = 0;
    if (i < n) {
      const int64_t k = n_out[i];
      int64_t f = (k == INT64_MIN ? 0 : (k > 0 ? k : -k));
      if (f > caps[i]) f = caps[i];
      v = f * channels[i];
    }
    sh[t] = v;
    __syncthreads();
    for (int d = 1; d < 256; d <<= 1) {
      const int64_t add = (t >= d) ? sh[t - d] : 0;
      __syncthreads();
      sh[t] += add;
      __syncthreads();
    }
    const int64_t base = carry;
    if (i < n) offsets[i] = base + sh[t] - v;
    __syncthreads();
    if (t == 255) carry = base + sh[255];
    __syncthreads();
  }
  if (t == 0) offsets[n] = carry;
}
__global__ void __launch_bounds__(256)
spx_pack_copy_kernel(const int16_t* __restrict__ out, const int64_t* __restrict__ out_offs,
                     const int64_t* __restrict__ offsets, int16_t* __restrict__ packed) {
  const int i = blockIdx.x;
  const int16_t* src = out + out_offs[i];
  int16_t* dst = packed + offsets[i];
  const int64_t cnt = offsets[i + 1] - offsets[i];
  const int64_t stride = (int64_t)gridDim.y * 256 * 8;
  for (int64_t e0 = ((int64_t)blockIdx.y * 256 + threadIdx.x); e0 < cnt; e0 += stride) {
    int16_t v[8];
#pragma unroll
    for (int u = 0; u < 8; u++) { const int64_t e = e0 + (int64_t)u * gridDim.y * 256; v[u] = (e < cnt) ? src[e] : (int16_t)0; }
#pragma unroll
    for (int u = 0; u < 8; u++) { const int64_t e = e0 + (int64_t)u * gridDim.y * 256; if (e < cnt) dst[e] = v[u]; }
  }
}

extern "C" {
int spx_batch_pack_outputs(const spx_stream_job* jobs, int n, const int16_t* out, const int64_t* n_out, int16_t* packed,
                           int64_t* offsets, void* hs) {
  if (!jobs || n <= 0 || !out || !n_out || !packed || !offsets) return fail(-1, "spx_batch_pack_outputs: bad arguments");
  hipStream_t st = static_cast<hipStream_t>(hs);
  const size_t need = (size_t)n * (2 * sizeof(int64_t) + sizeof(int));
  void* d_tab = nullptr;
  if (hipMallocAsync(&d_tab, need, st) != hipSuccess) return fail(-2, "spx_batch_pack_outputs: allocation failed");
  static thread_local SpxStage G;
  if (G.done) HIPCHK(hipEventSynchronize(G.done));
  else HIPCHK(hipEventCreateWithFlags(&G.done, hipEventDisableTiming));
  if (G.cap < need) {
    if (G.p) (void)hipHostFree(G.p);
    G.p = nullptr; G.cap = 0;
    HIPCHK(hipHostMalloc(&G.p, need * 2 + 1024, hipHostMallocDefault));
    G.cap = need * 2 + 1024;
  }
  unsigned char* h = static_cast<unsigned char*>(G.p);
  int64_t* h_off = reinterpret_cast<int64_t*>(h);
  int64_t* h_cap = h_off + n;
  int* h_ch = reinterpret_cast<int*>(h + (size_t)n * 2 * sizeof(int64_t));
  for (int i = 0; i < n; i++) { h_off[i] = jobs[i].out_off; h_cap[i] = jobs[i].out_cap; h_ch[i] = jobs[i].channels; }
  HIPCHK(hipMemcpyAsync(d_tab, h, need, hipMemcpyHostToDevice, st));
  HIPCHK(hipEventRecord(G.done, st));
  const int64_t* d_off = reinterpret_cast<const int64_t*>(d_tab);
  const int* d_ch = reinterpret_cast<const int*>(static_cast<unsigned char*>(d_tab) + (size_t)n * 2 * sizeof(int64_t));
  hipLaunchKernelGGL(spx_pack_offsets_kernel, dim3(1), dim3(256), 0, st, n_out, d_ch, d_off + n, n, offsets);
  hipLaunchKernelGGL(spx_pack_copy_kernel, dim3(n, 4), dim3(256), 0, st, out, d_off, offsets, packed);
  (void)hipFreeAsync(d_tab, st);
  HIPCHK(hipGetLastError());
  return 0;
}

int spx_copy_to_host(void* dst, const void* src, size_t bytes, void* hs) {
  HIPCHK(hipMemcpyAsync(dst, src, bytes, hipMemcpyDeviceToHost, static_cast<hipStream_t>(hs)));
  return 0;
}
int spx_stream_synchronize(void* hs) {
  HIPCHK(hipStreamSynchronize(static_cast<hipStream_t>(hs)));
  return 0;
}

}
```

speedy_amd/csrc/spx_engine.h:

```cpp
#pragma once
#include <algorithm>
#include <math.h>
#include <cmath>
#include <stdio.h>
#include <string.h>

#include <atomic>
#include <map>
#include <mutex>
#include <string>
#include <vector>

#include "../../include/speedy_hip.h"
#include "spx_internal.h"
#include "spx_mode.h"

#ifndef M_PI
#define M_PI 3.14159265358979323846
#endif


extern thread_local std::string g_spx_err;
static inline int fail(int code, const std::string& msg) {
  g_spx_err = msg;
  return code;
}
#define HIPCHK(expr)                                                                          \
  do {                                                                                        \
    hipError_t e_ = (expr);                                                                   \
    if (e_ != hipSuccess) return fail(-2, std::string(#expr) + ": " + hipGetErrorString(e_)); \
  } while (0)

#include <dlfcn.h>
struct SpxRoctx {
  int (*push)(const char*) = nullptr;
  int (*pop)() = nullptr;
  SpxRoctx() {
    void* h = dlopen("librocprofiler-sdk-roctx.so", RTLD_LAZY | RTLD_LOCAL);
    if (!h) h = dlopen("librocprofiler-sdk-roctx.so.1", RTLD_LAZY | RTLD_LOCAL);
    if (!h) h = dlopen("libroctx64.so", RTLD_LAZY | RTLD_LOCAL);
    if (!h) h = dlopen("libroctx64.so.4", RTLD_LAZY | RTLD_LOCAL);
    if (h) {
      push = reinterpret_cast<int (*)(const char*)>(dlsym(h, "roctxRangePushA"));
      pop = reinterpret_cast<int (*)()>(dlsym(h, "roctxRangePop"));
      if (!push || !pop) { push = nullptr; pop = nullptr; }
    }
  }
};
struct SpxRange {
  static SpxRoctx& api() { static SpxRoctx a; return a; }
  explicit SpxRange(const char* name) { if (api().push) api().push(name); }
  ~SpxRange() { if (api().pop) api().pop(); }
};

#define SPX_MAX_CHUNKS 16
#define SPX_MAX_WALK_STREAMS 4
#define SPX_RING (2 * SPX_MAX_WALK_STREAMS)
struct SpxStage {
  void* p = nullptr;
  size_t cap = 0;
  hipEvent_t done = nullptr;
};
struct spx_plan {
  SpxPlanDev dev;
  int device = 0;
  int cu_count = 1;
  size_t lds_per_cu = 65536;
  std::mutex mu;
  SpxStage stage[2];
  int stage_next = 0;
  struct Trial {
    SpxModeTrial state = {-1, 0, -1};
    hipEvent_t ev[4] = {nullptr, nullptr, nullptr, nullptr};
  } trial;
  std::map<long long, SpxModeResources> res_cache;
  std::map<const void*, int> split_of;
  void* tables = nullptr;
  hipStream_t side = nullptr;
  hipStream_t side2 = nullptr;
  hipEvent_t ev_tension = nullptr;
  hipEvent_t ev_start = nullptr;
  hipEvent_t ev_chunk[SPX_MAX_CHUNKS] = {};
  hipEvent_t ev_walk[SPX_RING] = {};
  bool ev_walk_valid[SPX_RING] = {};
  void* ring_ws[SPX_RING] = {};
  hipStream_t ring_st[SPX_RING] = {};
  int ahead_calls = 0;
  hipEvent_t ev_call[2] = {nullptr, nullptr};
  const void* ahead_last_out = nullptr;
  const void* ahead_last_nout = nullptr;
  bool ev_call_valid[2] = {false, false};
  hipStream_t ev_call_st[2] = {nullptr, nullptr};
  std::vector<std::pair<const int*, int>> mixed_started;
  const int* ahead_started = nullptr;
  int ahead_n = 0;
  hipStream_t mix = nullptr;
  hipEvent_t ev_join = nullptr, ev_fork = nullptr, ev_an = nullptr;
  std::mutex mix_mu;
  SpxStage mix_stage[2];
  int mix_next = 0;
};

struct EvPair { hipEvent_t a, b; int kind; };
extern std::atomic<bool> g_timing;
extern std::atomic<int> g_last_concurrent;
extern std::atomic<int> g_concurrent;
extern std::atomic<bool> g_chunks_set;
extern std::atomic<int> g_chunks;
extern std::mutex g_tmu;
extern std::vector<EvPair> g_ev_pending;
extern std::vector<hipEvent_t> g_ev_free;
extern int g_calls_pending;
struct SpxDevGuard {
  std::mutex mu;
  hipEvent_t last = nullptr;
  hipStream_t last_stream = nullptr;
  bool valid = false;
};
extern SpxDevGuard g_guard[64];

static inline int64_t frames_for(const SpxPlanDev& d, int64_t n_in) {
  if (n_in < d.W + 1) return 0;
  return (n_in - d.W - 1) / d.B + 1;
}
spx_plan* shared_plan_full(int sample_rate, int match_matlab);

struct Layout {
  size_t off_streams, off_states, off_rec, off_scratch, off_order, off_flags, off_ready, total;
  int64_t max_tiles;
  int64_t total_frames;
};
Layout layout_for(const SpxPlanDev& d, const spx_stream_job* jobs, int n);
int dev_side_streams(int dev, hipStream_t* side, hipStream_t* side2);
int walk_stream_count();
int dev_walk_streams(int dev, hipStream_t* w, int n);
int ring_note(spx_plan* plan, hipStream_t st);
int ring_wait(spx_plan* plan, hipStream_t sa, const void* ws, hipStream_t st, bool* waited_prev);
bool ring_previous_in_flight(spx_plan* plan);
int ring_record(spx_plan* plan, hipStream_t on, void* ws, hipStream_t st, const void* out, const void* n_out, bool detached = false);
SpxModeEnv mode_env();
bool device_ours_cb(void* ctx);
struct SpxSpeedClass { int maxC; bool speedup_only, any_speed; };
SpxSpeedClass speed_class(const spx_stream_job* jobs, int n);
SpxModeWalk mode_walk(const SpxPlanDev& d, int n, int maxC, bool speedup_only, bool lean, bool any_speed = false, bool short_window = false);
void spx_launch_gate(const int* started, int n_walk, unsigned max_spins, hipStream_t st);
struct SpxForce { int concurrent; bool idle_start; int total_streams; hipEvent_t after_analysis; hipStream_t ahead_sa; const int** started_out;
                  bool no_exclusive;
};
struct SpxRateCall {
  std::vector<int64_t> walk_out_off, walk_out_cap;
  std::vector<unsigned char> no_trunc;
  std::vector<int> table;
  SpxRateJob* d_table = nullptr;
  int64_t* d_tsm_n = nullptr;
  const int16_t* tsm_base = nullptr;
  int max_blocks = 1;
};
struct SpxCallOpts {
  const SpxForce* force = nullptr;
  const SpxRateCall* rate = nullptr;
  bool ahead_req = false;
  bool overlap_req = false;
  void* in_ready = nullptr;
  bool split_part = false;
  bool sub = false;
  void* done_event = nullptr;
  bool detached = false;
};
int run_impl(spx_plan_t plan, const spx_stream_job* jobs, int n, const int16_t* in, int16_t* out, int64_t* n_out, void* ws, size_t ws_bytes,
             const spx_taps* taps, void* hs, bool do_a, bool do_w, const SpxCallOpts& opt = SpxCallOpts());
int spx_read_steps(const SpxPlanDev& d, const spx_stream_job* jobs, int n, const void* ws, int32_t* steps, hipStream_t st);
```

speedy_amd/csrc/spx_engine.hip:

```cpp
#include "spx_engine.h"

__attribute__((constructor(101))) static void spx_default_hw_queues() {
  if (getenv("SPX_KEEP_HW_QUEUES") || getenv("GPU_MAX_HW_QUEUES")) return;
  setenv("GPU_MAX_HW_QUEUES", "8", 0);
  if (getenv("SPX_DEBUG_MODE")) fprintf(stderr, "[spx] GPU_MAX_HW_QUEUES was unset: set to 8 at load time (SPX_KEEP_HW_QUEUES=1 leaves the environment alone)\n");
}

thread_local std::string g_spx_err;

std::atomic<bool> g_timing{false};
std::atomic<int> g_last_concurrent{0};
std::atomic<int> g_concurrent{1};
std::atomic<bool> g_chunks_set{false};
std::atomic<int> g_chunks{1};
std::mutex g_tmu;
std::vector<EvPair> g_ev_pending;
std::vector<hipEvent_t> g_ev_free;
int g_calls_pending = 0;

SpxDevGuard g_guard[64];

int spx_kernel_vgprs(const void* fn, int* scratch_bytes) {
  static std::mutex mu;
  static std::map<const void*, std::pair<int, int>> cache;
  std::lock_guard<std::mutex> g(mu);
  auto it = cache.find(fn);
  if (it == cache.end()) {
    hipFuncAttributes a;
    int regs = 128, scratch = -1;
    if (hipFuncGetAttributes(&a, fn) == hipSuccess) { regs = (a.numRegs + 7) & ~7; scratch = (int)a.localSizeBytes; }
    (void)hipGetLastError();
    it = cache.emplace(fn, std::make_pair(regs, scratch)).first;
  }
  if (scratch_bytes) *scratch_bytes = it->second.second;
  return it->second.first;
}

#include <fcntl.h>
#include <sys/file.h>
#include <unistd.h>
static bool device_is_ours(int dev) {
  static std::mutex mu;
  static int state[64];
  static int lock_fd[64];
  static pid_t owner = 0;
  if (dev < 0 || dev >= 64) return false;
  std::lock_guard<std::mutex> g(mu);
  if (owner != getpid()) {
    for (int d = 0; d < 64; d++) { if (owner && state[d] > 0 && lock_fd[d] > 0) close(lock_fd[d]); state[d] = 0; lock_fd[d] = -1; }
    owner = getpid();
  }
  if (state[dev]) return state[dev] > 0;
  state[dev] = -1;
  if (getenv("SPX_SHARED_GPU")) return false;
  char bus[64] = "dev";
  if (hipDeviceGetPCIBusId(bus, (int)sizeof(bus), dev) != hipSuccess) { (void)hipGetLastError(); snprintf(bus, sizeof(bus), "ordinal%d", dev); }
  for (char* c = bus; *c; c++) if (*c == ':' || *c == '/') *c = '_';
  const char* dir = getenv("SPX_LOCK_DIR");
  if (!dir) dir = "/tmp";
  char path[256];
  snprintf(path, sizeof(path), "%s/spx_concurrent_%s.lock", dir, bus);
  int fd = open(path, O_CREAT | O_RDWR | O_CLOEXEC | O_NOFOLLOW, 0644);
  if (fd < 0) fd = open(path, O_RDONLY | O_CLOEXEC | O_NOFOLLOW);
  if (fd < 0) return false;
  if (flock(fd, LOCK_EX | LOCK_NB) != 0) { close(fd); return false; }
  state[dev] = 1;
  lock_fd[dev] = fd;
  return true;
}

extern "C" {

}
Layout layout_for(const SpxPlanDev& d, const spx_stream_job* jobs, int n) {
  Layout L;
  int64_t tf = 0;
  for (int i = 0; i < n; i++) tf += (jobs[i].nonlinear != 0.0f) ? frames_for(d, jobs[i].n_in) : 0;
  L.total_frames = tf;
  size_t o = 0;
  L.off_streams = o; o += ((sizeof(SpxStreamDev) * (size_t)n * SPX_MAX_CHUNKS + 255) & ~(size_t)255);
  L.off_states = o;  o += ((sizeof(SpxStreamState) * (size_t)n + 255) & ~(size_t)255);
  L.off_rec = o;     o += ((sizeof(SpxFrameRec) * (size_t)(tf + 1) + 255) & ~(size_t)255);
  L.off_scratch = o; o += ((sizeof(float) * 4 * (size_t)(tf + 1) + 255) & ~(size_t)255);
  const int TFr = std::min(spx_analysis_small_tile_frames(), d.tile_frames > 0 ? d.tile_frames : spx_analysis_small_tile_frames());
  L.max_tiles = tf / TFr + n + 1;
  L.off_order = o;   o += ((sizeof(int) * (size_t)L.max_tiles + 255) & ~(size_t)255);
  L.off_flags = o;   o += ((sizeof(int) * (size_t)L.max_tiles + 255) & ~(size_t)255);
  L.off_ready = o;   o += ((sizeof(int) * ((size_t)n + 1) + 255) & ~(size_t)255);
  L.total = o;
  return L;
}


static int build_streams(const SpxPlanDev& d, const spx_stream_job* jobs, int n, int nch,
                         std::vector<SpxStreamDev>& v, std::vector<int>& tiles_per_chunk, const SpxRateCall* rc = nullptr) {
  v.resize((size_t)n * nch);
  tiles_per_chunk.assign(nch, 0);
  int64_t fo = 0;
  const int TF = d.tile_frames;
  for (int i = 0; i < n; i++) {
    const spx_stream_job& j = jobs[i];
    if (j.channels < 1 || j.n_in < 0 || j.in_off < 0 || j.out_off < 0 || j.out_cap < 0)
      return fail(-1, "spx_batch: bad job (channels < 1 or a negative count / offset)");
    if (!(j.speed > 0.0f) || !std::isfinite(j.speed)) return fail(-1, "spx_batch: speed must be finite and > 0");
    if (!(j.nonlinear >= 0.0f && j.nonlinear <= 1.0f))
      return fail(-1, "spx_batch: nonlinear factor outside [0, 1] (sonic2.h:73-76; the blended speed could reach 0)");
    if (!std::isfinite(j.feedback)) return fail(-1, "spx_batch: feedback strength is not finite");
    if (j.nonlinear != 0.0f && !spx_internal_analysis_fits(d))
      return fail(-1, "spx_batch: sample rate too high for the nonlinear path (the analysis tile does not fit one CU's LDS); linear jobs only");
    if (j.n_in >= (1ll << 30)) return fail(-1, "spx_batch: stream of 2^30 frames or more (in-kernel positions are 32-bit)");
    const bool nonlinear = j.nonlinear != 0.0f;
    const int64_t Ttot = nonlinear ? frames_for(d, j.n_in) : 0;
    if (Ttot > 0x7fffff00) return fail(-1, "spx_batch: stream too long");
    int64_t Tprev = 0;
    for (int c = 0; c < nch; c++) {
      int64_t n_c = j.n_in;
      if (c < nch - 1) n_c = (j.n_in * (c + 1) / nch) / d.B * d.B;
      SpxStreamDev& s = v[(size_t)c * n + i];
      s.in_off = j.in_off; s.n_in = n_c; s.out_off = j.out_off; s.out_cap = j.out_cap;
      s.channels = j.channels; s.speed = j.speed; s.nonlinear = j.nonlinear; s.feedback = j.feedback;
      const int64_t T = nonlinear ? frames_for(d, n_c) : 0;
      s.n_frames = (int32_t)T;
      s.frame_begin = (int32_t)Tprev;
      s.flags = (c == 0 ? SPX_F_INIT : 0) | (c == nch - 1 ? SPX_F_FLUSH : 0);
      if (rc) {
        s.out_off = rc->walk_out_off[i]; s.out_cap = rc->walk_out_cap[i];
        if (rc->no_trunc[i]) s.flags |= SPX_F_NO_TRUNC;
      }
      s.frame_off = fo;
      s.first_tile = tiles_per_chunk[c];
      tiles_per_chunk[c] += (int)((T - Tprev + TF - 1) / TF);
      Tprev = T;
    }
    fo += Ttot;
  }
  return 0;
}

static SpxTapsDev taps_of(const spx_taps* t) {
  SpxTapsDev d = {nullptr, nullptr, nullptr, nullptr, nullptr};
  if (t) { d.tension = t->tension; d.speed = t->speed; d.features = t->features;
           d.spectrogram = t->spectrogram; d.normalized = t->normalized; }
  return d;
}

__global__ void spx_gate_kernel(const int* started, int n_walk, unsigned max_spins) {
  if (threadIdx.x == 0) {
    for (unsigned i = 0; i < max_spins; i++) {
      if (__hip_atomic_load(started, __ATOMIC_RELAXED, __HIP_MEMORY_SCOPE_AGENT) >= n_walk) break;
      __builtin_amdgcn_s_sleep(8);
    }
  }
}
void spx_launch_gate(const int* started, int n_walk, unsigned max_spins, hipStream_t st) {
  hipLaunchKernelGGL(spx_gate_kernel, dim3(1), dim3(64), 0, st, started, n_walk, max_spins);
}
__global__ void __launch_bounds__(256)
spx_stage_kernel(const unsigned* __restrict__ src, unsigned* __restrict__ dst_a, unsigned n_a, unsigned* __restrict__ dst_b,
                 unsigned n_b, unsigned* __restrict__ zero_a, unsigned nz_a, unsigned* __restrict__ zero_b, unsigned nz_b,
                 const int* gate_started, int gate_n, unsigned gate_spins) {
  const unsigned stride = gridDim.x * blockDim.x, t0 = blockIdx.x * blockDim.x + threadIdx.x;
  for (unsigned i = t0; i < n_a; i += stride) dst_a[i] = src[i];
  for (unsigned i = t0; i < n_b; i += stride) dst_b[i] = src[n_a + i];
  for (unsigned i = t0; i < nz_a; i += stride) zero_a[i] = 0u;
  for (unsigned i = t0; i < nz_b; i += stride) zero_b[i] = 0u;
  if (gate_started != nullptr && t0 == 0) {
    for (unsigned i = 0; i < gate_spins; i++) {
      if (__hip_atomic_load(gate_started, __ATOMIC_RELAXED, __HIP_MEMORY_SCOPE_AGENT) >= gate_n) break;
      __builtin_amdgcn_s_sleep(8);
    }
  }
}
extern "C" {

static hipEvent_t take_event() {
  std::lock_guard<std::mutex> g(g_tmu);
  if (!g_ev_free.empty()) { hipEvent_t e = g_ev_free.back(); g_ev_free.pop_back(); return e; }
  hipEvent_t e;
  (void)hipEventCreate(&e);
  return e;
}

}
int dev_side_streams(int dev, hipStream_t* side, hipStream_t* side2) {
  static std::mutex mu;
  static hipStream_t s1[64], s2[64];
  const int d = (dev >= 0 && dev < 64) ? dev : 0;
  std::lock_guard<std::mutex> g(mu);
  if (!s1[d]) {
    if (hipStreamCreateWithFlags(&s1[d], hipStreamNonBlocking) != hipSuccess) { s1[d] = nullptr; return -1; }
    if (hipStreamCreateWithFlags(&s2[d], hipStreamNonBlocking) != hipSuccess) { (void)hipStreamDestroy(s1[d]); s1[d] = nullptr; s2[d] = nullptr; return -1; }
  }
  *side = s1[d]; *side2 = s2[d];
  return 0;
}

int walk_stream_count() { return 2; }
int dev_walk_streams(int dev, hipStream_t* w, int n) {
  static std::mutex mu;
  static hipStream_t s3[64][SPX_MAX_WALK_STREAMS];
  hipStream_t side = nullptr, side2 = nullptr;
  if (dev_side_streams(dev, &side, &side2)) return -1;
  const int d = (dev >= 0 && dev < 64) ? dev : 0;
  std::lock_guard<std::mutex> g(mu);
  w[0] = side2;
  for (int i = 1; i < n && i < SPX_MAX_WALK_STREAMS; i++) {
    if (!s3[d][i] && hipStreamCreateWithFlags(&s3[d][i], hipStreamNonBlocking) != hipSuccess) { s3[d][i] = nullptr; return -1; }
    w[i] = s3[d][i];
  }
  return 0;
}

int ring_note(spx_plan* plan, hipStream_t st) {
  const int cur = plan->ahead_calls & 1;
  if (!plan->ev_call[cur]) HIPCHK(hipEventCreateWithFlags(&plan->ev_call[cur], hipEventDisableTiming));
  HIPCHK(hipEventRecord(plan->ev_call[cur], st));
  plan->ev_call_valid[cur] = true;
  plan->ev_call_st[cur] = st;
  return 0;
}
int ring_wait(spx_plan* plan, hipStream_t sa, const void* ws, hipStream_t st, bool* waited_prev) {
  const int c = plan->ahead_calls % SPX_RING;
  if (waited_prev) *waited_prev = false;
  for (int back = SPX_RING; back >= 1; back--) {
    const int j = (c + SPX_RING - back) % SPX_RING;
    if (!plan->ev_walk_valid[j]) continue;
    if (back > SPX_RING / 2 || plan->ring_ws[j] == ws || plan->ring_st[j] != st) {
      HIPCHK(hipStreamWaitEvent(sa, plan->ev_walk[j], 0));
      if (back == 1 && waited_prev) *waited_prev = true;
    }
  }
  return 0;
}
bool ring_previous_in_flight(spx_plan* plan) {
  const int j = (plan->ahead_calls + SPX_RING - 1) % SPX_RING;
  const bool f = plan->ev_walk_valid[j] && hipEventQuery(plan->ev_walk[j]) == hipErrorNotReady;
  (void)hipGetLastError();
  return f;
}
int ring_record(spx_plan* plan, hipStream_t on, void* ws, hipStream_t st, const void* out, const void* n_out, bool detached) {
  const int c = plan->ahead_calls % SPX_RING;
  if (!plan->ev_walk[c]) HIPCHK(hipEventCreateWithFlags(&plan->ev_walk[c], hipEventDisableTiming));
  HIPCHK(hipEventRecord(plan->ev_walk[c], on));
  if (on != st && !detached) HIPCHK(hipStreamWaitEvent(st, plan->ev_walk[c], 0));
  plan->ev_walk_valid[c] = true;
  plan->ring_ws[c] = ws;
  plan->ring_st[c] = st;
  plan->ahead_last_out = out;
  plan->ahead_last_nout = n_out;
  plan->ahead_calls++;
  return 0;
}

SpxModeEnv mode_env() {
  SpxModeEnv e;
  e.concurrent_enabled = g_concurrent.load() != 0;
  e.chunks_set = g_chunks_set.load();
  e.chunks = g_chunks.load();
  return e;
}
bool device_ours_cb(void* ctx) { return device_is_ours(*static_cast<int*>(ctx)); }
SpxSpeedClass speed_class(const spx_stream_job* jobs, int n) {
  SpxSpeedClass c = {1, true, true};
  for (int i = 0; i < n; i++) {
    if (jobs[i].channels > c.maxC) c.maxC = jobs[i].channels;
    const bool ok = jobs[i].speed > 0.0f && jobs[i].speed < SPX_FAST_MAX_SPEED && jobs[i].nonlinear >= 0.0f && jobs[i].nonlinear <= 1.0f;
    if (!(ok && jobs[i].speed > 1.0f)) c.speedup_only = false;
    if (!ok) c.any_speed = false;
  }
  if (c.speedup_only) c.any_speed = false;
  return c;
}
SpxModeWalk mode_walk(const SpxPlanDev& d, int n, int maxC, bool speedup_only, bool lean, bool any_speed, bool short_window) {
  const SpxWalkConfig c = spx_walk_config(d, n, maxC, speedup_only, false, lean, any_speed, short_window);
  SpxModeWalk w;
  w.lds = c.lds; w.waves = c.waves; w.fast_kernel = c.fast_kernel; w.nwc = c.nwc;
  w.vgprs = spx_walk_vgprs(d, n, maxC, speedup_only, lean, any_speed, short_window);
  return w;
}
static const SpxModeResources& mode_resources(spx_plan* plan, int n, int maxC, bool speedup_only, bool any_speed = false, bool short_window = false) {
  const long long key = ((long long)n << 16) ^ ((long long)maxC << 3) ^ (short_window ? 4 : 0) ^ (any_speed ? 2 : 0) ^ (speedup_only ? 1 : 0);
  auto it = plan->res_cache.find(key);
  if (it != plan->res_cache.end()) return it->second;
  const SpxPlanDev& d = plan->dev;
  SpxModeResources R;
  memset(&R, 0, sizeof(R));
  R.cu_count = plan->cu_count;
  R.lds_per_cu = plan->lds_per_cu;
  R.walk = mode_walk(d, n, maxC, speedup_only, false, any_speed, short_window);
  R.walk_lean = R.walk;
  if (maxC == 1 && n <= plan->cu_count && R.walk.fast_kernel && R.walk.nwc > 0) {
    R.walk_lean = mode_walk(d, n, maxC, speedup_only, true, any_speed);
    R.lean_valid = true;
  }
  R.tension_lds = spx_tension_lds_bytes();
  R.tension_vgprs = spx_tension_vgprs();
  R.tile_default = d.tile_frames;
  R.tile_big = spx_analysis_tile_frames();
  R.tile_small = spx_analysis_small_tile_frames();
  SpxPlanDev d8 = d;
  d8.tile_frames = R.tile_small;
  R.an_lds_default = spx_analysis_lds_bytes(d);
  R.an_vgprs_default = spx_analysis_vgprs(d);
  R.an_lds_small = spx_analysis_lds_bytes(d8);
  R.an_vgprs_small = spx_analysis_vgprs(d8);
  if (plan->res_cache.size() > 64) plan->res_cache.clear();
  return plan->res_cache.emplace(key, R).first->second;
}
extern "C" int spx_debug_mode_resources(int sample_rate, int channels, int n_streams, int speedup_only, long long* out) {
  spx_plan* plan = shared_plan_full(sample_rate, 0);
  if (!plan || !out || n_streams < 1) return -1;
  std::lock_guard<std::mutex> g(plan->mu);
  const SpxModeResources& R = mode_resources(plan, n_streams, channels < 1 ? 1 : channels, speedup_only != 0, speedup_only == 0);
  const long long v[22] = {R.cu_count, (long long)R.lds_per_cu, (long long)R.walk.lds, R.walk.waves, R.walk.vgprs, R.walk.fast_kernel, R.walk.nwc,
                           (long long)R.walk_lean.lds, R.walk_lean.waves, R.walk_lean.vgprs, R.walk_lean.fast_kernel, R.walk_lean.nwc, R.lean_valid,
                           (long long)R.tension_lds, R.tension_vgprs, R.tile_default, R.tile_big, R.tile_small, (long long)R.an_lds_default,
                           (long long)R.an_lds_small, R.an_vgprs_default, R.an_vgprs_small};
  for (int i = 0; i < 22; i++) out[i] = v[i];
  return 0;
}

static int stage_tables(spx_plan* plan, const std::vector<SpxStreamDev>& sv, const std::vector<int>& order, SpxStreamDev* dstreams,
                        int* d_order, int* d_flags, unsigned n_flags, int* d_ready, unsigned n_ready, hipStream_t on, hipEvent_t* done,
                        const int* gate_started = nullptr, int gate_n = 0, unsigned gate_spins = 0) {
  const size_t b_sv = sizeof(SpxStreamDev) * sv.size(), b_or = sizeof(int) * order.size();
  SpxStage& G = plan->stage[plan->stage_next];
  plan->stage_next ^= 1;
  if (G.done) HIPCHK(hipEventSynchronize(G.done));
  else HIPCHK(hipEventCreateWithFlags(&G.done, hipEventDisableTiming));
  if (G.cap < b_sv + b_or) {
    if (G.p) (void)hipHostFree(G.p);
    G.p = nullptr; G.cap = 0;
    const size_t cap = (b_sv + b_or) * 2 + 4096;
    HIPCHK(hipHostMalloc(&G.p, cap, hipHostMallocDefault));
    G.cap = cap;
  }
  unsigned char* hp = static_cast<unsigned char*>(G.p);
  memcpy(hp, sv.data(), b_sv);
  if (b_or) memcpy(hp + b_sv, order.data(), b_or);
  hipLaunchKernelGGL(spx_stage_kernel, dim3(64), dim3(256), 0, on, reinterpret_cast<const unsigned*>(hp),
                     reinterpret_cast<unsigned*>(dstreams), (unsigned)(b_sv / 4), reinterpret_cast<unsigned*>(d_order), (unsigned)(b_or / 4),
                     reinterpret_cast<unsigned*>(d_flags), n_flags, reinterpret_cast<unsigned*>(d_ready), n_ready, gate_started, gate_n, gate_spins);
  HIPCHK(hipEventRecord(G.done, on));
  *done = G.done;
  return 0;
}

struct SpxTimed {
  hipEvent_t a = nullptr, b = nullptr;
  hipStream_t s = nullptr;
  int kind = 0;
  SpxTimed(bool on, int kind_, hipStream_t s_) : s(s_), kind(kind_) {
    if (on) { a = take_event(); b = take_event(); (void)hipEventRecord(a, s); }
  }
  ~SpxTimed() {
    if (!a) return;
    (void)hipEventRecord(b, s);
    std::lock_guard<std::mutex> g(g_tmu);
    g_ev_pending.push_back({a, b, kind});
  }
};

int run_impl(spx_plan_t plan, const spx_stream_job* jobs, int n, const int16_t* in, int16_t* out,
             int64_t* n_out, void* ws, size_t ws_bytes, const spx_taps* taps, void* hs, bool do_a,
             bool do_w, const SpxCallOpts& opt) {
  if (!plan || !jobs || n <= 0) return fail(-1, "spx_batch: bad arguments");
  SpxRange range_(do_a && do_w ? "spx_batch_run" : (do_a ? "spx_batch_analyze" : "spx_batch_walk"));
  const SpxForce* force = opt.force;
  SpxPlanDev d = plan->dev;
  Layout L = layout_for(d, jobs, n);
  if (ws_bytes < L.total || !ws) return fail(-1, "spx_batch: workspace too small");
  const SpxSpeedClass SC = speed_class(jobs, n);
  const int maxC = SC.maxC;
  const bool speedup_only = SC.speedup_only && !opt.rate, any_speed = SC.any_speed && !opt.rate;
  std::lock_guard<std::mutex> plan_lock(plan->mu);
  if (!opt.split_part) plan->split_of.erase(ws);
  const bool short_window_res = opt.force && opt.force->no_exclusive;
  const SpxModeResources& R = mode_resources(plan, n, maxC, speedup_only, any_speed, short_window_res);
  if (R.walk.lds > 160 * 1024)
    return fail(-1, "spx_batch: too many channels for the walk kernel's LDS window");
  hipStream_t st = static_cast<hipStream_t>(hs);
  SpxModeShape S;
  S.n = n; S.max_channels = maxC; S.do_a = do_a; S.do_w = do_w; S.has_frames = L.total_frames > 0;
  S.forced = force != nullptr;
  S.force_concurrent = force && force->concurrent != 0;
  S.force_ahead = force && force->ahead_sa != nullptr;
  S.force_total_streams = force ? force->total_streams : n;
  S.ahead_req = opt.ahead_req; S.overlap_req = opt.overlap_req;
  SpxModeEnv E = mode_env();
  if (opt.rate) E.concurrent_enabled = false;
  SpxModeRuntime T;
  memset(&T, 0, sizeof(T));
  const int two_back = (plan->ahead_calls + SPX_RING - 2) % SPX_RING;
  T.two_workspaces = plan->ev_walk_valid[two_back] && plan->ring_ws[two_back] == ws;
  T.trial_key = ((long long)n << 40) ^ ((long long)L.total_frames << 8) ^ (maxC << 3) ^ (any_speed ? 4 : 0) ^ (speedup_only ? 2 : 0) ^ (opt.overlap_req ? 1 : 0);
  T.device_ours = device_ours_cb;
  T.device_ctx = &plan->device;
  spx_plan::Trial& TR = plan->trial;
  if (TR.state.key == T.trial_key && TR.state.choice < 0 && TR.state.calls >= 3 && TR.ev[1] && TR.ev[3] &&
      hipEventQuery(TR.ev[1]) == hipSuccess && hipEventQuery(TR.ev[3]) == hipSuccess)
    T.trial_times_ready = hipEventElapsedTime(&T.ms_seq, TR.ev[0], TR.ev[1]) == hipSuccess &&
                          hipEventElapsedTime(&T.ms_con, TR.ev[2], TR.ev[3]) == hipSuccess;
  (void)hipGetLastError();
  SpxMode M = spx_choose_mode(S, R, E, T, TR.state);
  SpxDevGuard& guard = g_guard[(plan->device >= 0 && plan->device < 64) ? plan->device : 0];
  std::unique_lock<std::mutex> guard_lock(guard.mu, std::defer_lock);
  bool idle_start = force ? force->idle_start : false;
  if (M.want_concurrent && !force) {
    guard_lock.lock();
    const hipError_t q = guard.valid ? hipEventQuery(guard.last) : hipSuccess;
    (void)hipGetLastError();
    idle_start = (q == hipSuccess);
    if (guard.valid && guard.last_stream != st && q == hipErrorNotReady) {
      T.guard_busy = true;
      M = spx_choose_mode(S, R, E, T, TR.state);
      guard_lock.unlock();
    }
  }
  static const bool dbg_trial = getenv("SPX_DEBUG_TRIAL") != nullptr;
  if (dbg_trial && TR.state.choice < 0 && M.trial_next.choice >= 0 && T.trial_times_ready)
    fprintf(stderr, "[spx trial] n=%d maxC=%d: concurrent %.3f ms, in sequence %.3f ms -> %s\n", n, maxC, T.ms_con, T.ms_seq,
            M.trial_next.choice ? "concurrent" : "sequence");
  TR.state = M.trial_next;
  d.tile_frames = M.tile_frames;
  const int nch = M.nch;
  const bool concurrent = M.concurrent, ahead = M.ahead;
  const bool chunk_ahead = M.chunk_ahead && !force;
  std::vector<SpxStreamDev> sv;
  std::vector<int> tiles;
  int rc = build_streams(d, jobs, n, nch, sv, tiles, opt.rate);
  if (rc) return rc;
  if (opt.rate && (concurrent || ahead || chunk_ahead || !do_a || !do_w || force)) return fail(-1, "spx_batch_run_rate: internal: not a plain call in sequence");
  unsigned char* w = static_cast<unsigned char*>(ws);
  SpxStreamDev* dstreams = reinterpret_cast<SpxStreamDev*>(w + L.off_streams);
  SpxStreamState* states = reinterpret_cast<SpxStreamState*>(w + L.off_states);
  SpxFrameRec* rec = reinterpret_cast<SpxFrameRec*>(w + L.off_rec);
  float* scratch = reinterpret_cast<float*>(w + L.off_scratch);
  int* d_order = reinterpret_cast<int*>(w + L.off_order);
  int* d_flags = reinterpret_cast<int*>(w + L.off_flags);
  int* d_ready = reinterpret_cast<int*>(w + L.off_ready);
  SpxTapsDev td = taps_of(taps);
  const bool timed = g_timing.load() && do_a && do_w;
  if (do_a && do_w) g_last_concurrent.store(concurrent ? 1 : (ahead ? 2 : 0), std::memory_order_relaxed);
  static const bool dbg_mode = getenv("SPX_DEBUG_MODE") != nullptr;
  if (dbg_mode)
    fprintf(stderr, "[spx mode] rate %d n %d maxC %d: co_resident %d doubtful %d lean %d want_concurrent %d chunks %d tiles %d -> %s%s\n",
            d.rate, n, maxC, (int)M.co_resident, (int)M.doubtful, (int)M.launch_lean, (int)M.want_concurrent, nch, tiles[0],
            concurrent ? "concurrent" : (ahead ? (M.seq_ahead ? "ahead (kernels in sequence)" : "ahead") : (chunk_ahead ? "sequence, producers ahead" : "sequence")),
            M.walk2 ? ", walk kernels overlapping" : "");
  hipStream_t stw = st;
  const bool detached = opt.detached && M.walk2 && !force;
  if (do_w && !force && !detached && ring_note(plan, st)) return -2;
  if (do_w && !force && detached) { plan->ev_call_valid[plan->ahead_calls & 1] = false; plan->ev_call_st[plan->ahead_calls & 1] = nullptr; }
  if (M.walk2) {
    hipStream_t wst[SPX_MAX_WALK_STREAMS];
    const int nws = walk_stream_count();
    if (dev_walk_streams(plan->device, wst, nws)) return fail(-1, "spx_batch: no walk streams");
    const int cur = plan->ahead_calls & 1;
    stw = wst[plan->ahead_calls % nws];
    const bool same_out = !opt.sub && (out == plan->ahead_last_out || n_out == plan->ahead_last_nout);
    const bool foreign_prev = !plan->ev_call_valid[cur ^ 1] || plan->ev_call_st[cur ^ 1] != st;
    if (detached) { }
    else if (same_out || (foreign_prev && plan->ahead_calls > 0)) HIPCHK(hipStreamWaitEvent(stw, plan->ev_call[cur], 0));
    else if (plan->ev_call_valid[cur ^ 1]) HIPCHK(hipStreamWaitEvent(stw, plan->ev_call[cur ^ 1], 0));
  }
  hipStream_t sa = st;
  if (nch > 1 || concurrent || ahead) {
    if (!plan->side) {
      if (dev_side_streams(plan->device, &plan->side, &plan->side2)) return fail(-1, "spx_batch: no side streams");
      HIPCHK(hipEventCreateWithFlags(&plan->ev_start, hipEventDisableTiming));
      HIPCHK(hipEventCreateWithFlags(&plan->ev_tension, hipEventDisableTiming));
      for (auto& e : plan->ev_chunk) HIPCHK(hipEventCreateWithFlags(&e, hipEventDisableTiming));
    }
    sa = M.ahead_forced ? force->ahead_sa : plan->side;
  }
  std::vector<int> order;
  if (concurrent) {
    order.reserve((size_t)tiles[0]);
    std::vector<int> cnt(n);
    int maxT = 0;
    for (int i = 0; i < n; i++) {
      cnt[i] = (i + 1 < n ? sv[i + 1].first_tile : tiles[0]) - sv[i].first_tile;
      if (cnt[i] > maxT) maxT = cnt[i];
    }
    for (int t = 0; t < maxT; t++)
      for (int i = 0; i < n; i++)
        if (t < cnt[i]) order.push_back(sv[i].first_tile + t);
  }
  bool waited_prev = false;
  if ((ahead || chunk_ahead) && !force) {
    if (ring_wait(plan, sa, ws, st, &waited_prev)) return -2;
    if (opt.in_ready) HIPCHK(hipStreamWaitEvent(sa, static_cast<hipEvent_t>(opt.in_ready), 0));
  }
  if (!ahead && !chunk_ahead && opt.in_ready) HIPCHK(hipStreamWaitEvent(st, static_cast<hipEvent_t>(opt.in_ready), 0));
  hipEvent_t staged_ev = nullptr;
  const bool ahead_gate = ahead && !force && plan->ahead_started != nullptr && plan->ahead_n > 0 && !waited_prev &&
                          ring_previous_in_flight(plan);
  rc = stage_tables(plan, sv, opt.rate ? opt.rate->table : order, dstreams, opt.rate ? reinterpret_cast<int*>(opt.rate->d_table) : d_order, d_flags, concurrent ? (unsigned)tiles[0] : 0u, d_ready,
                    (concurrent || ahead) ? (unsigned)n + 1u : 0u, (ahead || chunk_ahead) ? sa : st, &staged_ev,
                    ahead_gate ? plan->ahead_started : nullptr, plan->ahead_n, 8000u);
  if (rc) return rc;
  if (M.trial_slot >= 0) {
    hipEvent_t& e0 = TR.ev[2 * M.trial_slot];
    if (!e0) HIPCHK(hipEventCreate(&e0));
    HIPCHK(hipEventRecord(e0, st));
  }
  if (sa != st && !ahead && !chunk_ahead) {
    HIPCHK(hipStreamWaitEvent(sa, staged_ev, 0));
    if (concurrent) HIPCHK(hipStreamWaitEvent(plan->side2, staged_ev, 0));
  }
  for (int c = 0; c < nch; c++) {
    SpxStreamDev* dj = dstreams + (size_t)c * n;
    if (concurrent && do_w && idle_start)
      hipLaunchKernelGGL(spx_gate_kernel, dim3(1), dim3(64), 0, sa, d_ready + n, n, 1200u);
    if (do_a && tiles[c] > 0) {
      SpxTimed tm(timed, 0, sa);
      spx_launch_analysis(d, dj, n, tiles[c], in, rec, td, concurrent ? d_order : nullptr, concurrent ? d_flags : nullptr, sa);
    }
    if (force && force->after_analysis && c == nch - 1) HIPCHK(hipEventRecord(force->after_analysis, sa));
    if (sa != st) HIPCHK(hipEventRecord(plan->ev_chunk[c], sa));
    if (sa != st && !concurrent && !ahead) HIPCHK(hipStreamWaitEvent(st, plan->ev_chunk[c], 0));
    if (do_w) {
      hipStream_t stn = concurrent ? plan->side2 : (ahead ? sa : st);
      {
        SpxTimed tm(timed, 2, stn);
        spx_launch_tension(d, dj, n, states, rec, scratch, td, concurrent ? d_flags : nullptr, (concurrent || ahead) ? d_ready : nullptr, stn);
      }
      if (concurrent || ahead) HIPCHK(hipEventRecord(plan->ev_tension, stn));
      if (ahead) HIPCHK(hipStreamWaitEvent(stw, plan->ev_tension, 0));
      {
        SpxTimed tm(timed, 1, stw);
        spx_launch_walk(d, dj, n, maxC, in, out, opt.rate ? opt.rate->d_tsm_n : n_out, states, scratch, (concurrent || ahead) ? d_ready : nullptr,
                        speedup_only, stw, false, (M.exclusive_cu && !(force && force->no_exclusive)) ? R.lds_per_cu / 2 + 1024 : 0, M.launch_lean, any_speed,
                        short_window_res || (!force && M.walk2 && !M.launch_lean && maxC > 1));
      }
      if (opt.rate && c == nch - 1) {
        SpxTimed tm(timed, 3, stw);
        spx_launch_rate_batch(opt.rate->d_table, n, opt.rate->max_blocks, states, opt.rate->d_tsm_n, opt.rate->tsm_base, out, n_out, stw);
      }
      if (M.ahead_forced && force->started_out) *force->started_out = d_ready + n;
      if (c == nch - 1 && !force) {
        if (ring_record(plan, stw, ws, st, out, n_out, detached)) return -2;
        plan->ahead_started = (concurrent || ahead) ? d_ready + n : nullptr;
        plan->ahead_n = n;
        plan->mixed_started.clear();
      }
    }
    if (concurrent) {
      HIPCHK(hipStreamWaitEvent(st, plan->ev_chunk[c], 0));
      HIPCHK(hipStreamWaitEvent(st, plan->ev_tension, 0));
    }
  }
  if (concurrent && !force) {
    if (!guard.last) HIPCHK(hipEventCreateWithFlags(&guard.last, hipEventDisableTiming));
    HIPCHK(hipEventRecord(guard.last, st));
    guard.last_stream = st;
    guard.valid = true;
  }
  if (M.trial_slot >= 0) {
    hipEvent_t& e1 = TR.ev[2 * M.trial_slot + 1];
    if (!e1) HIPCHK(hipEventCreate(&e1));
    HIPCHK(hipEventRecord(e1, st));
  }
  if (opt.done_event && do_w) HIPCHK(hipEventRecord(static_cast<hipEvent_t>(opt.done_event), detached ? stw : st));
  if (timed) { std::lock_guard<std::mutex> g(g_tmu); g_calls_pending++; }
  HIPCHK(hipGetLastError());
  return 0;
}

#define SPX_SPLIT_LIMIT 4
struct SplitPlan { int k; std::vector<int> first; std::vector<size_t> ws_off, ws_bytes; size_t total; };
static SplitPlan split_geometry(const spx_plan* plan, const spx_stream_job* jobs, int n, int max_mult) {
  SplitPlan P;
  P.k = 1; P.total = 0;
  const int cu = plan->cu_count > 0 ? plan->cu_count : 1;
  if (max_mult > SPX_SPLIT_LIMIT) max_mult = SPX_SPLIT_LIMIT;
  if (n <= cu || n > max_mult * cu) return P;
  P.k = (n + cu - 1) / cu;
  size_t o = 0;
  for (int i = 0; i < P.k; i++) {
    const int a = (int)((long long)n * i / P.k), b = (int)((long long)n * (i + 1) / P.k);
    P.first.push_back(a);
    const size_t bytes = layout_for(plan->dev, jobs + a, b - a).total;
    P.ws_off.push_back(o); P.ws_bytes.push_back(bytes);
    o += (bytes + 255) & ~(size_t)255;
  }
  P.first.push_back(n);
  P.total = o;
  return P;
}
static int run_split(spx_plan_t plan, const spx_stream_job* jobs, int n, const int16_t* in, int16_t* out, int64_t* n_out, void* ws,
                     size_t ws_bytes, const spx_taps* taps, void* hs, const SpxCallOpts& opt) {
  if (!plan || !jobs || n <= 0) return fail(-1, "spx_batch: bad arguments");
  SplitPlan P = split_geometry(plan, jobs, n, opt.ahead_req && opt.overlap_req ? 2 : 1);
  if (P.k > 1 && (g_chunks_set.load() || ws_bytes < P.total)) P.k = 1;
  if (P.k > 1) {
    const SpxSpeedClass SC = speed_class(jobs, n);
    const int maxC = SC.maxC;
    std::lock_guard<std::mutex> plan_lock(plan->mu);
    const int m = P.first[1] - P.first[0];
    const SpxModeResources& R = mode_resources(plan, m, maxC, SC.speedup_only, SC.any_speed);
    SpxModeShape S;
    memset(&S, 0, sizeof(S));
    S.n = m; S.max_channels = maxC; S.do_a = S.do_w = true; S.has_frames = true; S.force_total_streams = m;
    S.ahead_req = S.overlap_req = true;
    SpxModeRuntime T;
    memset(&T, 0, sizeof(T));
    T.trial_key = -2;
    T.device_ours = device_ours_cb;
    T.device_ctx = &plan->device;
    const SpxModeTrial none = {-1, 0, -1};
    const SpxMode M = spx_choose_mode(S, R, mode_env(), T, none);
    if (!(M.ahead && M.walk2)) P.k = 1;
  }
  if (P.k <= 1) return run_impl(plan, jobs, n, in, out, n_out, ws, ws_bytes, taps, hs, true, true, opt);
  { std::lock_guard<std::mutex> g(plan->mu); if (plan->split_of.size() > 64) plan->split_of.clear(); plan->split_of[ws] = P.k; }
  int64_t rows = 0;
  for (int i = 0; i < P.k; i++) {
    const int a = P.first[i], m = P.first[i + 1] - a;
    spx_taps t;
    if (taps) {
      t = *taps;
      if (t.tension) t.tension += rows;
      if (t.speed) t.speed += rows;
      if (t.features) t.features += rows * SPX_FEATURE_COUNT;
      if (t.spectrogram) t.spectrogram += rows * (int64_t)plan->dev.N;
      if (t.normalized) t.normalized += rows * (int64_t)plan->dev.W;
      for (int j = a; j < a + m; j++) rows += jobs[j].nonlinear != 0.0f ? frames_for(plan->dev, jobs[j].n_in) : 0;
    }
    SpxCallOpts o;
    o.ahead_req = o.overlap_req = true;
    o.split_part = true;
    o.sub = i > 0;
    o.in_ready = opt.in_ready;
    if (i == P.k - 1) o.done_event = opt.done_event;
    const int rc = run_impl(plan, jobs + a, m, in, out, n_out + a, static_cast<unsigned char*>(ws) + P.ws_off[i], P.ws_bytes[i],
                            taps ? &t : nullptr, hs, true, true, o);
    if (rc) return rc;
  }
  return 0;
}

int spx_internal_run(spx_plan_t plan, const spx_stream_job* jobs, int n, const int16_t* in, int16_t* out, int64_t* n_out, void* ws,
                     size_t ws_bytes, const spx_taps* taps, void* hs, bool ahead, bool overlap, void* in_ready, void* done_event,
                     bool detached) {
  SpxCallOpts o;
  o.ahead_req = ahead; o.overlap_req = overlap; o.in_ready = in_ready; o.done_event = done_event; o.detached = detached;
  return run_split(plan, jobs, n, in, out, n_out, ws, ws_bytes, taps, hs, o);
}

extern "C" {
size_t spx_batch_workspace_bytes(spx_plan_t plan, const spx_stream_job* jobs, int n_streams) {
  if (!plan || !jobs || n_streams < 1) return 0;
  return std::max(layout_for(plan->dev, jobs, n_streams).total, split_geometry(plan, jobs, n_streams, SPX_SPLIT_LIMIT).total);
}
int spx_batch_run(spx_plan_t plan, const spx_stream_job* jobs, int n, const int16_t* in, int16_t* out,
                  int64_t* n_out, void* ws, size_t ws_bytes, const spx_taps* taps, void* hs) {
  return run_split(plan, jobs, n, in, out, n_out, ws, ws_bytes, taps, hs, SpxCallOpts());
}
int spx_batch_run_ahead(spx_plan_t plan, const spx_stream_job* jobs, int n, const int16_t* in, int16_t* out,
                        int64_t* n_out, void* ws, size_t ws_bytes, const spx_taps* taps, void* hs) {
  return spx_internal_run(plan, jobs, n, in, out, n_out, ws, ws_bytes, taps, hs, true, false, nullptr, nullptr, false);
}
int spx_batch_run_overlapped(spx_plan_t plan, const spx_stream_job* jobs, int n, const int16_t* in, int16_t* out,
                             int64_t* n_out, void* ws, size_t ws_bytes, const spx_taps* taps, void* hs) {
  return spx_internal_run(plan, jobs, n, in, out, n_out, ws, ws_bytes, taps, hs, true, true, nullptr, nullptr, false);
}
int spx_batch_run_ahead_when(spx_plan_t plan, const spx_stream_job* jobs, int n, const int16_t* in, int16_t* out,
                             int64_t* n_out, void* ws, size_t ws_bytes, const spx_taps* taps, void* hs, void* in_ready_event) {
  return spx_internal_run(plan, jobs, n, in, out, n_out, ws, ws_bytes, taps, hs, true, false, in_ready_event, nullptr, false);
}
int spx_batch_analyze(spx_plan_t plan, const spx_stream_job* jobs, int n, const int16_t* in, void* ws,
                      size_t ws_bytes, const spx_taps* taps, void* hs) {
  return run_impl(plan, jobs, n, in, nullptr, nullptr, ws, ws_bytes, taps, hs, true, false);
}
int spx_batch_walk(spx_plan_t plan, const spx_stream_job* jobs, int n, const int16_t* in, int16_t* out,
                   int64_t* n_out, void* ws, size_t ws_bytes, const spx_taps* taps, void* hs) {
  return run_impl(plan, jobs, n, in, out, n_out, ws, ws_bytes, taps, hs, false, true);
}

}

static int rate_ratio(int sample_rate, float rate, int* old_rate, int* new_rate) {
  if (!(rate > 0.0f) || !std::isfinite(rate)) return fail(-1, "sonicSetRate: rate must be finite and > 0");
  const float q = sample_rate / rate;
  if (!(q < 2147483520.0f)) return fail(-1, "sonicSetRate: rate too small for this sample rate");
  int o = sample_rate, w = (int)q;
  while (w > (1 << 14) || o > (1 << 14)) { w >>= 1; o >>= 1; }
  if (w < 1) return fail(-1, "sonicSetRate: rate too large for this sample rate");
  if (o < 1) return fail(-1, "sonicSetRate: rate too small for this sample rate");
  *old_rate = o; *new_rate = w;
  return 0;
}
static int64_t rate_frames(int64_t m, int old_rate, int new_rate) {
  return m >= 2 ? ((m - 1) * (int64_t)new_rate + old_rate - 1) / old_rate : 0;
}
struct RateLayout { size_t off_table, off_tsm_n, off_tsm, total; std::vector<int64_t> tsm_off, tsm_cap; };
static int rate_layout(spx_plan_t plan, const spx_stream_job* jobs, const float* rates, int n, RateLayout& RL) {
  size_t o = (spx_batch_workspace_bytes(plan, jobs, n) + 255) & ~(size_t)255;
  RL.off_table = o; o += (sizeof(SpxRateJob) * (size_t)n + 255) & ~(size_t)255;
  RL.off_tsm_n = o; o += (sizeof(int64_t) * (size_t)n + 255) & ~(size_t)255;
  RL.off_tsm = o;
  RL.tsm_off.assign(n, 0); RL.tsm_cap.assign(n, 0);
  int64_t v = 0;
  for (int i = 0; i < n; i++) {
    if (rates[i] == 1.0f) continue;
    if (jobs[i].channels < 1 || jobs[i].n_in < 0) return fail(-1, "spx_batch: bad job (channels < 1 or a negative count / offset)");
    RL.tsm_off[i] = v;
    RL.tsm_cap[i] = spx_internal_out_bound(plan->dev, jobs[i].n_in, jobs[i].speed, jobs[i].nonlinear != 0.0f);
    v += (RL.tsm_cap[i] * jobs[i].channels + 7) & ~(int64_t)7;
  }
  RL.total = o + sizeof(int16_t) * (size_t)v + 128;
  return 0;
}
extern "C" {
int64_t spx_plan_out_capacity_rate(spx_plan_t plan, int64_t n_in, float speed, float nonlinear, float rate) {
  if (!plan) { fail(-1, "spx_plan_out_capacity_rate: bad arguments"); return -1; }
  const int64_t cap = spx_internal_out_bound(plan->dev, n_in, speed, nonlinear != 0.0f);
  if (rate == 1.0f) return cap;
  int o = 1, w = 1;
  if (rate_ratio(plan->dev.rate, rate, &o, &w)) return -1;
  return rate_frames(cap, o, w) + 1;
}
size_t spx_batch_workspace_bytes_rate(spx_plan_t plan, const spx_stream_job* jobs, const float* rates, int n_streams) {
  if (!rates) return spx_batch_workspace_bytes(plan, jobs, n_streams);
  if (!plan || !jobs || n_streams < 1) return 0;
  for (int i = 0; i < n_streams; i++) { int o, w; if (rate_ratio(plan->dev.rate, rates[i], &o, &w)) return 0; }
  RateLayout RL;
  if (rate_layout(plan, jobs, rates, n_streams, RL)) return 0;
  return RL.total;
}
int spx_batch_run_rate(spx_plan_t plan, const spx_stream_job* jobs, const float* rates, int n, const int16_t* in, int16_t* out,
                       int64_t* n_out, void* ws, size_t ws_bytes, const spx_taps* taps, void* hs) {
  if (!plan || !jobs || n <= 0) return fail(-1, "spx_batch: bad arguments");
  bool any = false;
  std::vector<int> oldR(n, 1), newR(n, 1);
  if (rates)
    for (int i = 0; i < n; i++) {
      if (rate_ratio(plan->dev.rate, rates[i], &oldR[i], &newR[i])) return -1;
      any = any || rates[i] != 1.0f;
    }
  if (!any) return spx_batch_run(plan, jobs, n, in, out, n_out, ws, ws_bytes, taps, hs);
  if (!in || !out || !n_out || !ws || (reinterpret_cast<uintptr_t>(out) & 1)) return fail(-1, "spx_batch_run_rate: bad arguments");
  RateLayout RL;
  if (rate_layout(plan, jobs, rates, n, RL)) return -1;
  if (ws_bytes < RL.total) return fail(-1, "spx_batch_run_rate: workspace too small (spx_batch_workspace_bytes_rate)");
  unsigned char* w = static_cast<unsigned char*>(ws);
  SpxRateCall RC;
  RC.d_table = reinterpret_cast<SpxRateJob*>(w + RL.off_table);
  RC.d_tsm_n = reinterpret_cast<int64_t*>(w + RL.off_tsm_n);
  RC.tsm_base = reinterpret_cast<const int16_t*>(w + RL.off_tsm);
  const int64_t tsm_from_out = (int64_t)((reinterpret_cast<intptr_t>(RC.tsm_base) - reinterpret_cast<intptr_t>(out)) / (intptr_t)sizeof(int16_t));
  RC.walk_out_off.resize(n); RC.walk_out_cap.resize(n); RC.no_trunc.resize(n);
  std::vector<SpxRateJob> tab((size_t)n);
  memset(tab.data(), 0, sizeof(SpxRateJob) * (size_t)n);
  for (int i = 0; i < n; i++) {
    const bool resample = rates[i] != 1.0f;
    SpxRateJob& J = tab[i];
    J.fin_off = jobs[i].out_off; J.fin_cap = jobs[i].out_cap;
    J.channels = jobs[i].channels; J.old_rate = oldR[i]; J.new_rate = newR[i]; J.rate = rates[i];
    J.bypass = resample ? 0 : 1;
    J.tsm_off = RL.tsm_off[i]; J.tsm_cap = RL.tsm_cap[i];
    J.n_blocks = 1;
    if (resample && jobs[i].out_cap > 0) J.n_blocks = spx_rate_batch_blocks(std::min(jobs[i].out_cap, rate_frames(J.tsm_cap, J.old_rate, J.new_rate)), J.channels);
    if (J.n_blocks > RC.max_blocks) RC.max_blocks = J.n_blocks;
    RC.no_trunc[i] = resample ? 1 : 0;
    RC.walk_out_off[i] = resample ? tsm_from_out + RL.tsm_off[i] : jobs[i].out_off;
    RC.walk_out_cap[i] = resample ? RL.tsm_cap[i] : jobs[i].out_cap;
  }
  static_assert(sizeof(SpxRateJob) % sizeof(int) == 0, "the staging kernel copies 32-bit words");
  RC.table.resize(sizeof(SpxRateJob) / sizeof(int) * (size_t)n);
  memcpy(RC.table.data(), tab.data(), sizeof(SpxRateJob) * (size_t)n);
  SpxCallOpts o;
  o.rate = &RC;
  return run_impl(plan, jobs, n, in, out, n_out, ws, ws_bytes, taps, hs, true, true, o);
}
}
int spx_read_steps(const SpxPlanDev& d, const spx_stream_job* jobs, int n, const void* ws, int32_t* steps, hipStream_t st) {
  const Layout L = layout_for(d, jobs, n);
  std::vector<SpxStreamState> h((size_t)n);
  HIPCHK(hipStreamSynchronize(st));
  HIPCHK(hipMemcpy(h.data(), static_cast<const unsigned char*>(ws) + L.off_states, sizeof(SpxStreamState) * (size_t)n, hipMemcpyDeviceToHost));
  for (int i = 0; i < n; i++) steps[i] = h[i].w.steps;
  return 0;
}
extern "C" {
int spx_batch_read_steps(spx_plan_t plan, const spx_stream_job* jobs, int n, const void* ws, int32_t* steps, void* hs) {
  if (!plan || !jobs || n <= 0 || !ws || !steps) return fail(-1, "spx_batch_read_steps: bad arguments");
  int k = 1;
  { std::lock_guard<std::mutex> g(plan->mu); auto it = plan->split_of.find(ws); if (it != plan->split_of.end()) k = it->second; }
  if (k <= 1) return spx_read_steps(plan->dev, jobs, n, ws, steps, static_cast<hipStream_t>(hs));
  const SplitPlan P = split_geometry(plan, jobs, n, SPX_SPLIT_LIMIT);
  if (P.k != k) return fail(-1, "spx_batch_read_steps: the jobs are not those of the call that last ran on this workspace");
  for (int i = 0; i < P.k; i++) {
    const int a = P.first[i], m = P.first[i + 1] - a;
    const int rc = spx_read_steps(plan->dev, jobs + a, m, static_cast<const unsigned char*>(ws) + P.ws_off[i], steps + a, static_cast<hipStream_t>(hs));
    if (rc) return rc;
  }
  return 0;
}
}
```

speedy_amd/csrc/spx_internal.h:

```cpp
#pragma once
#include <hip/hip_runtime.h>
#include <stdint.h>

#include <stdlib.h>


#define SPX_FAST_MAX_SPEED 1.0e18f

#define SPX_MAX_STAGES 16
#define SPX_WAVE 64
#define SPX_BLOCK 256
#define SPX_FEATURE_COUNT 15

struct SpxPlanDev {
  int rate;
  int B;
  int W;
  int N;
  int F;
  int Pp;
  int nstages;
  int radix[SPX_MAX_STAGES];
  int minPeriod, maxPeriod, maxRequired, skip;
  int tile_frames;
  int dft_waves;
  float alpha;
  float one_minus_alpha;
  const double* tw;
  const double* tw2;
  const float* window;
  const float* taperF;
  const float* taperP;
  int rader;
  int nstagesM;
  int radixM[SPX_MAX_STAGES];
  const double* twM;
  const double* bfft;
  const int* perm;
  const int* iperm;
  const int* qlog;
};

#define SPX_F_INIT 1
#define SPX_F_FLUSH 2
#define SPX_F_TENSION_RANGE 4
#define SPX_F_NO_SPEED 8
#define SPX_F_NO_TRUNC 16
#define SPX_F_SPEED_SET 32
#define SPX_F_KEEP_SPEED 64
#define SPX_F_HANDED_IN 128
struct SpxStreamDev {
  int64_t in_off, n_in, out_off, out_cap;
  int64_t frame_off;
  int32_t n_frames;
  int32_t frame_begin;
  int32_t channels;
  int32_t flags;
  float speed, nonlinear, feedback;
  int32_t first_tile;
  int64_t tsm_shift;
  int32_t tension_skip;
  int32_t unit_time0;
  int32_t tension_to;
  int32_t handed_in;
  int32_t ring_bufs;
  int32_t pad4;
};

struct SpxWalkState {
  int64_t base;
  int64_t out_n;
  int64_t avail;
  int remaining;
  int prevPeriod, prevMinDiff;
  int overflow;
  int prevPeriod_toggle;
  int steps;
};
struct SpxStreamState {
  SpxWalkState w;
  float lp;
  float lpf;
  float cur_dur;
  float des_dur;
  float curSpeed;
  int handed;
  int flush_remaining;
  int flush_out_mark;
  int tension_first;
  int pad2_;
};

#define SPX_RATE_MAX_CHANNELS 16
struct SpxRateState {
  int64_t tsm_seen;
  int64_t final_n;
  int32_t old_pos, new_pos;
  int32_t has_left;
  int32_t overflow;
  int16_t left[SPX_RATE_MAX_CHANNELS];
};
void spx_launch_rate(SpxRateState* rs, const SpxStreamState* st, const int64_t* tsm_n, const int16_t* tsm, int16_t* fin,
                     int64_t fin_cap, int channels, int old_rate, int new_rate, float rate, int bypass, int flush,
                     hipStream_t hs);

struct SpxRateJob {
  int64_t tsm_off;
  int64_t tsm_cap;
  int64_t fin_off;
  int64_t fin_cap;
  int32_t channels;
  int32_t old_rate, new_rate;
  int32_t bypass;
  float rate;
  int32_t n_blocks;
  int64_t pad_;
};
int spx_rate_batch_blocks(int64_t frames, int channels);
void spx_launch_rate_batch(const SpxRateJob* jobs, int n_streams, int max_blocks, const SpxStreamState* states, const int64_t* tsm_n,
                           const int16_t* tsm_base, int16_t* fin_base, int64_t* n_out, hipStream_t hs);

struct SpxFrameRec {
  float energy;
  float lsd;
};

struct SpxTapsDev {
  float* tension;
  float* speed;
  float* features;
  float* spectrogram;
  float* normalized;
};

void spx_launch_analysis(const SpxPlanDev& P, const SpxStreamDev* streams, int n_streams, int n_tiles,
                         const int16_t* in, SpxFrameRec* rec, SpxTapsDev taps, const int* tile_order, int* tile_flags,
                         hipStream_t st);
void spx_launch_analysis_frames(const SpxPlanDev& P, const SpxStreamDev* streams, int n_tiles, const float* frames,
                                bool preemph, SpxFrameRec* rec, SpxTapsDev taps, hipStream_t st);
void spx_launch_tension(const SpxPlanDev& P, const SpxStreamDev* streams, int n_streams, SpxStreamState* states,
                        const SpxFrameRec* rec, float* scratch, SpxTapsDev taps, const int* tile_flags, int* speed_ready,
                        hipStream_t st);
void spx_launch_walk(const SpxPlanDev& P, const SpxStreamDev* streams, int n_streams, int max_channels,
                     const int16_t* in, int16_t* out, int64_t* n_out, SpxStreamState* states, const float* scratch,
                     const int* speed_ready, bool speedup_only, hipStream_t st, bool short_jobs = false, size_t lds_min = 0,
                     bool lean = false, bool any_speed = false, bool short_window = false);
size_t spx_analysis_lds_bytes(const SpxPlanDev& P);
int spx_analysis_ct_window(const SpxPlanDev& P);
void spx_host_dft(int n, const int* radix, int nstages, const double* tw, const double* in, double* out);
size_t spx_walk_lds_bytes(const SpxPlanDev& P, int max_channels, bool speedup_only);
struct SpxWalkConfig {
  int mode;
  bool fast_kernel;
  int nw;
  int nwm, nwc, wcap;
  int waves;
  size_t lds;
  bool slow;
};
SpxWalkConfig spx_walk_config(const SpxPlanDev& P, int n_streams, int max_channels, bool speedup_only, bool short_jobs = false,
                              bool lean = false, bool any_speed = false, bool short_window = false);
size_t spx_walk_fast_lds_bytes(const SpxPlanDev& P, int wcap);
bool spx_walk_fast_supports(const SpxPlanDev& P, int nwm);
void spx_launch_walk_fast(const SpxPlanDev& P, const SpxStreamDev* streams, int n_streams, const int16_t* in,
                          int16_t* out, int64_t* n_out, SpxStreamState* states, const float* scratch,
                          const int* speed_ready, int nwm, int nwc, int wcap, int max_channels, hipStream_t st, size_t lds_min = 0,
                          bool slow = false);
#define SPX_NOUT_LOST_PRODUCER INT64_MIN
size_t spx_tension_lds_bytes();
int spx_kernel_vgprs(const void* fn, int* scratch_bytes = nullptr);
int spx_tension_vgprs();
int spx_analysis_vgprs(const SpxPlanDev& P, int* scratch_bytes = nullptr);
int spx_walk_vgprs(const SpxPlanDev& P, int n_streams, int max_channels, bool speedup_only, bool lean = false, bool any_speed = false,
                   bool short_window = false);
int spx_walk_kernel_regs(const SpxPlanDev& P, int n_streams, int max_channels, bool speedup_only, bool short_jobs, bool lean,
                         int* scratch_bytes, bool any_speed = false, bool short_window = false);
void spx_launch_speed_from_tension(SpxStreamState* state, float tension, float Rg, float feedback, float* speed_out,
                                   hipStream_t st);
int spx_analysis_tile_frames();
int spx_analysis_small_tile_frames();
int spx_analysis_tiny_tile_frames();
int spx_analysis_prefers_small_tile(const SpxPlanDev& P);

struct spx_plan;
int64_t spx_internal_out_bound(const SpxPlanDev& P, int64_t n_in, float speed, bool nonlinear);
const SpxPlanDev* spx_internal_shared_plan(int sample_rate, int match_matlab);
bool spx_internal_analysis_fits(const SpxPlanDev& d);
int64_t spx_internal_frames_for(const SpxPlanDev& d, int64_t n_in);
```

speedy_amd/csrc/spx_tension.hip:

```cpp
#include "spx_internal.h"

#define SPX_CH 512
#ifndef SPX_TCH
#define SPX_TCH 16
#endif
#define SPX_TENSION_THREADS 256

__device__ __forceinline__ float iir_wave(const float* sA, float* sB, int n, float a, float b, float y) {
  const int lane = threadIdx.x;
  for (int b0 = 0; b0 < n; b0 += 64) {
    const int m = n - b0 < 64 ? n - b0 : 64;
    const float ax = a * ((lane < m) ? sA[b0 + lane] : 0.0f);
#ifndef SPX_TENSION_OLD_CHAIN
    if (m == 64) {
      if (lane == 0) {
#pragma unroll
        for (int j = 0; j < 64; j++) {
          const float s = __builtin_bit_cast(float, __builtin_amdgcn_readlane(__builtin_bit_cast(int, ax), j));
          y = s + b * y;
          sB[b0 + j] = y;
        }
      }
      y = __builtin_bit_cast(float, __builtin_amdgcn_readfirstlane(__builtin_bit_cast(int, y)));
      continue;
    }
#endif
#ifndef SPX_TENSION_OLD_CHAIN
    if (lane == 0) {
#pragma unroll
      for (int j = 0; j < 64; j++) {
        if (j < m) {
          const float s = __builtin_bit_cast(float, __builtin_amdgcn_readlane(__builtin_bit_cast(int, ax), j));
          y = s + b * y;
          sB[b0 + j] = y;
        }
      }
    }
    y = __builtin_bit_cast(float, __builtin_amdgcn_readfirstlane(__builtin_bit_cast(int, y)));
#else
    float out = 0.0f;
#pragma unroll
    for (int j = 0; j < 64; j++) {
      if (j < m) {
        const float s = __builtin_bit_cast(float, __builtin_amdgcn_readlane(__builtin_bit_cast(int, ax), j));
        y = s + b * y;
        out = (lane == j) ? y : out;
      }
    }
    if (lane < m) sB[b0 + lane] = out;
#endif
  }
  return y;
}

__global__ void __launch_bounds__(SPX_TENSION_THREADS)
spx_tension_kernel(SpxPlanDev P, const SpxStreamDev* __restrict__ streams, SpxStreamState* __restrict__ states,
                   const SpxFrameRec* __restrict__ rec_base, float* __restrict__ scratch_base, SpxTapsDev taps,
                   const int* tile_flags, int* speed_ready) {
  constexpr int NT = SPX_TENSION_THREADS;
  __shared__ float sA[SPX_CH];
  __shared__ float sB[SPX_CH];
  __shared__ int sWait;
  const int tid = threadIdx.x;
  const SpxStreamDev S = streams[blockIdx.x];
  const int Ttot = S.n_frames, F = P.F, Pp = P.Pp;
  const int t0 = S.unit_time0 ? 0 : 1;
  const float Rg = S.speed, nl = S.nonlinear, fb = S.feedback;
  if (nl == 0.0f) return;

  struct { float lp, lpf, cur_dur, des_dur; int first_k; } Z;
  if (S.flags & SPX_F_INIT) {
    Z.lp = 2.14204f;
    Z.lpf = 123.837f;
    Z.cur_dur = 0.0f; Z.des_dur = 0.0f;
    Z.first_k = -1;
  } else {
    const SpxStreamState& in = states[blockIdx.x];
    Z.lp = in.lp; Z.lpf = in.lpf; Z.cur_dur = in.cur_dur; Z.des_dur = in.des_dur;
    Z.first_k = in.tension_first;
  }
  const SpxFrameRec* rec = rec_base + S.frame_off;
  float* scr = scratch_base + (size_t)S.frame_off * 4;
  const float lowthr = (float)(0.04 * (double)1.41421f);
  float* tfeat = taps.features ? taps.features + (size_t)S.frame_off * SPX_FEATURE_COUNT : nullptr;

  int fa_c = S.frame_begin;
  int wch = SPX_TCH;
  bool ok_all = true;
  for (;;) {
    int T_c = Ttot;
    if (tile_flags != nullptr && Ttot - fa_c > wch) T_c = fa_c + wch;
    const bool last = T_c >= Ttot;
    if (tile_flags != nullptr && T_c > fa_c) {
      const int TF = P.tile_frames;
      const int i0 = (fa_c - S.frame_begin) / TF, i1 = (T_c - S.frame_begin + TF - 1) / TF;
      if (tid == 0) {
        int ok = 1;
        for (int i = i0; i < i1 && ok; i++) {
          unsigned spins = 0;
          while (__hip_atomic_load(&tile_flags[S.first_tile + i], __ATOMIC_RELAXED, __HIP_MEMORY_SCOPE_AGENT) == 0) {
            __builtin_amdgcn_s_sleep(32);
            if (++spins > (1u << 22)) { ok = 0; break; }
          }
        }
        __builtin_amdgcn_fence(__ATOMIC_ACQUIRE, "agent");
        asm volatile("s_waitcnt vmcnt(0)" ::: "memory");
        sWait = ok;
      }
      __syncthreads();
      if (sWait == 0) { ok_all = false; break; }
    }
    const int fa = fa_c, T = T_c;
    int K0 = (fa + t0 >= F) ? fa + t0 - F : 0;
    if (K0 < S.tension_skip) K0 = S.tension_skip;
    int K = (T + t0 >= F) ? T + t0 - F : 0;
    if (S.flags & SPX_F_TENSION_RANGE) {
      K0 = S.tension_skip;
      if (K > S.tension_to) K = S.tension_to;
    }
    if (Z.first_k < 0 && K > K0) Z.first_k = K0;
    const int first_k = Z.first_k;
    if (T > fa || (S.flags & SPX_F_TENSION_RANGE)) {
      float lp = Z.lp;
      for (int c0 = fa; c0 < T; c0 += SPX_CH) {
        const int n = min(SPX_CH, T - c0);
        for (int i = tid; i < n; i += NT) sA[i] = rec[c0 + i].energy;
        __syncthreads();
        if (tid < 64) lp = iir_wave(sA, sB, n, P.one_minus_alpha, P.alpha, lp);
        __syncthreads();
        for (int i = tid; i < n; i += NT) {
          const float e = sA[i], l = sB[i];
          const float local = e / l;
          const float comp = (float)__builtin_sqrt(local > 2 ? 2.0 : (double)local);
          const int j = c0 + i;
          scr[4 * j + 0] = comp;
          const int k = j + t0 - F;
          if (tfeat && k >= 0) {
            float* f = tfeat + (size_t)k * SPX_FEATURE_COUNT;
            f[1] = l; f[2] = local; f[3] = comp; f[12] = (float)(j + t0);
          }
        }
        if (n > 0) lp = sB[n - 1];
        __syncthreads();
      }
      Z.lp = lp;
      for (int k = K0 + tid; k < K; k += NT) {
        float future_max = 0.0f, past_max = 0.0f;
        for (int i = 0; i <= F; i++) {
          const int tau = k + i;
          float v = (tau >= t0) ? scr[4 * (tau - t0) + 0] : 0.0f;
          v *= P.taperF[i];
          if (v > future_max) future_max = v;
        }
        for (int i = 0; i <= Pp; i++) {
          const int tau = k - i;
          float v = (tau >= t0) ? scr[4 * (tau - t0) + 0] : 0.0f;
          v *= P.taperP[i];
          if (v > past_max) past_max = v;
        }
        const float hyst = (float)((double)(past_max + future_max) / 2.0);
        const float e_cur = (k < t0) ? 0.0f : rec[k - t0].energy;
        const bool low = e_cur <= lowthr || k == first_k;
        const float lsd = low ? 0.0f : rec[k - t0].lsd;
        const float ewld = low ? 0.0f : lsd * hyst;
        scr[4 * k + 1] = hyst;
        scr[4 * k + 2] = ewld;
        if (tfeat) {
          float* f = tfeat + (size_t)k * SPX_FEATURE_COUNT;
          f[0] = e_cur; f[4] = hyst; f[5] = low ? 1.0f : 0.0f; f[6] = lsd; f[7] = ewld;
          f[13] = (float)k; f[14] = lowthr;
        }
      }
      __syncthreads();
      float lpf = Z.lpf;
      for (int c0 = K0; c0 < K; c0 += SPX_CH) {
        const int n = min(SPX_CH, K - c0);
        for (int i = tid; i < n; i += NT) sA[i] = scr[4 * (c0 + i) + 2];
        __syncthreads();
        if (tid < 64) lpf = iir_wave(sA, sB, n, P.one_minus_alpha, P.alpha, lpf);
        __syncthreads();
        for (int i = tid; i < n; i += NT) {
          const int k = c0 + i;
          const float ewld = sA[i], l = sB[i];
          const float hyst = scr[4 * k + 1];
          const float e_cur = (k < t0) ? 0.0f : rec[k - t0].energy;
          const bool low = e_cur <= lowthr || k == first_k;
          float rel = 0.0f, sc = 0.0f;
          if (!low) {
            rel = (float)((double)ewld / ((double)l + 0.01 * (double)123.979f));
            sc = (float)fmin((double)rel, (double)(4 * 0.971975f));
          }
          const float a = 0.5f, b = 0.25f, M_E_ = 0.7f, M_S = 1.0f;
          const float tension = a * (hyst - M_E_) + b * (sc - M_S);
          float v;
          if ((double)Rg > 1.0) {
            v = (float)fmax(1.0, (double)(Rg + (1 - Rg) * tension));
          } else {
            v = (float)fmax(0.01, fmin(1.0, (double)(Rg - (1 - Rg) * tension)));
          }
          scr[4 * k + 2] = tension;
          scr[4 * k + 3] = v;
          if (tfeat) {
            float* f = tfeat + (size_t)k * SPX_FEATURE_COUNT;
            f[8] = l; f[9] = rel; f[10] = sc; f[11] = tension;
          }
          if (taps.tension) taps.tension[S.frame_off + k] = tension;
        }
        if (n > 0) lpf = sB[n - 1];
        __syncthreads();
      }
      Z.lpf = lpf;
      float cur_dur = Z.cur_dur, des_dur = Z.des_dur;
      const float fd = (float)(1.0 / 100.0);
      for (int c0 = K0; c0 < ((S.flags & SPX_F_NO_SPEED) ? K0 : K); c0 += SPX_CH) {
        const int n = min(SPX_CH, K - c0);
        for (int i = tid; i < n; i += NT) sA[i] = scr[4 * (c0 + i) + 3];
        __syncthreads();
        if (!(fb > 0)) {
          if (tid < 64) {
            const float cstep = fd / Rg;
            for (int b0 = 0; b0 < n; b0 += 64) {
              const int m = n - b0 < 64 ? n - b0 : 64;
              const float req = (tid < m) ? sA[b0 + tid] : 1.0f;
              const float q = fd / req;
              if (m == 64) {
#pragma unroll
                for (int j = 0; j < 64; j++) {
                  cur_dur += __builtin_bit_cast(float, __builtin_amdgcn_readlane(__builtin_bit_cast(int, q), j));
                  des_dur += cstep;
                }
              } else {
#pragma unroll
                for (int j = 0; j < 64; j++) {
                  if (j < m) {
                    cur_dur += __builtin_bit_cast(float, __builtin_amdgcn_readlane(__builtin_bit_cast(int, q), j));
                    des_dur += cstep;
                  }
                }
              }
              if (tid < m) sB[b0 + tid] = req * nl + Rg * (1 - nl);
            }
            if (tid == 0) { sA[0] = cur_dur; sA[1] = des_dur; }
          }
        } else if (tid == 0) {
          for (int i = 0; i < n; i++) {
            float req = sA[i];
            if (fb > 0) {
              const float excess = cur_dur - des_dur;
              req = (float)((double)req + fmax(0.01, (double)(fb * excess)));
            }
            cur_dur += fd / req;
            des_dur += fd / Rg;
            sB[i] = req * nl + Rg * (1 - nl);
          }
          sA[0] = cur_dur;
          sA[1] = des_dur;
        }
        __syncthreads();
        cur_dur = sA[0];
        des_dur = sA[1];
        for (int i = tid; i < n; i += NT) {
          scr[4 * (c0 + i) + 3] = sB[i];
          if (taps.speed) taps.speed[S.frame_off + c0 + i] = sB[i];
        }
        __syncthreads();
      }
      Z.cur_dur = cur_dur;
      Z.des_dur = des_dur;
    }
    if (speed_ready != nullptr) {
      asm volatile("s_waitcnt vmcnt(0)" ::: "memory");
      __syncthreads();
      if (tid == 0) {
        __builtin_amdgcn_fence(__ATOMIC_RELEASE, "agent");
        asm volatile("s_waitcnt vmcnt(0)" ::: "memory");
        __hip_atomic_store(&speed_ready[blockIdx.x], K, __ATOMIC_RELAXED, __HIP_MEMORY_SCOPE_AGENT);
      }
    } else {
      __syncthreads();
    }
    fa_c = T_c;
    if (last) break;
  }
  if (!ok_all && speed_ready != nullptr && tid == 0)
    __hip_atomic_store(&speed_ready[blockIdx.x], -1, __ATOMIC_RELAXED, __HIP_MEMORY_SCOPE_AGENT);
  if (tid == 0) {
    SpxStreamState& o = states[blockIdx.x];
    o.lp = Z.lp; o.lpf = Z.lpf; o.cur_dur = Z.cur_dur; o.des_dur = Z.des_dur;
    o.tension_first = Z.first_k;
  }
}

size_t spx_tension_lds_bytes() { return sizeof(float) * 2 * SPX_CH + 64; }
int spx_tension_vgprs() {
  return spx_kernel_vgprs(reinterpret_cast<const void*>(spx_tension_kernel));
}

__global__ void spx_speed_kernel(SpxStreamState* state, float tension, float Rg, float fb, float* speed_out) {
  if (threadIdx.x != 0) return;
  float v;
  if ((double)Rg > 1.0) {
    v = (float)fmax(1.0, (double)(Rg + (1 - Rg) * tension));
  } else {
    v = (float)fmax(0.01, fmin(1.0, (double)(Rg - (1 - Rg) * tension)));
  }
  float cur_dur = state->cur_dur, des_dur = state->des_dur;
  if (fb > 0) {
    const float excess = cur_dur - des_dur;
    v = (float)((double)v + fmax(0.01, (double)(fb * excess)));
  }
  const float fd = (float)(1.0 / 100.0);
  cur_dur += fd / v;
  des_dur += fd / Rg;
  state->cur_dur = cur_dur;
  state->des_dur = des_dur;
  *speed_out = v;
}
void spx_launch_speed_from_tension(SpxStreamState* state, float tension, float Rg, float feedback, float* speed_out,
                                   hipStream_t st) {
  hipLaunchKernelGGL(spx_speed_kernel, dim3(1), dim3(64), 0, st, state, tension, Rg, feedback, speed_out);
}

void spx_launch_tension(const SpxPlanDev& P, const SpxStreamDev* streams, int n_streams, SpxStreamState* states,
                        const SpxFrameRec* rec, float* scratch, SpxTapsDev taps, const int* tile_flags, int* speed_ready,
                        hipStream_t st) {
  if (n_streams <= 0) return;
  hipLaunchKernelGGL(spx_tension_kernel, dim3(n_streams), dim3(SPX_TENSION_THREADS), 0, st, P, streams, states, rec,
                     scratch, taps, tile_flags, speed_ready);
}
```

Baseline: 45320.

## Fuse tension pass into analysis kernel via last-tile-done finisher block

Adds a templated finisher variant of the analysis kernel. Each tile atomically counts completed tiles per stream, and the block that finishes a stream's last tile runs the tension/speed computation inline. This removes the separate tension kernel launch and its event handoff before the walk kernel in the ahead/walk2 path. The tension body moves into a shared header so both kernels can use it. In exchange the analysis kernel gets more register and LDS pressure, and the tension work is serialized onto whichever block finishes last.

```diff
diff --git a/include/speedy_hip.h b/include/speedy_hip.h
--- a/include/speedy_hip.h
+++ b/include/speedy_hip.h
@@ -119,6 +119,7 @@
 long long spx_debug_arith_check(unsigned seed, unsigned threads, unsigned per_thread);
 int spx_debug_log_check(unsigned first_block, unsigned end_block, unsigned long long* sums);
 int spx_debug_last_call_concurrent(void);
+int spx_debug_last_call_finisher(void);
 double spx_timing_last_tension_ms(void);
 double spx_timing_last_rate_ms(void);
 
diff --git a/speedy_amd/_lib.py b/speedy_amd/_lib.py
--- a/speedy_amd/_lib.py
+++ b/speedy_amd/_lib.py
@@ -75,6 +75,7 @@
     "spx_debug_last_walk_form": (C.c_int, []),
     "spx_debug_kernel_vgprs": (C.c_int, [C.c_int]),
     "spx_debug_last_call_concurrent": (C.c_int, []),
+    "spx_debug_last_call_finisher": (C.c_int, []),
     "spx_debug_fdiv_check": (C.c_longlong, [C.c_uint, C.c_uint, C.c_int, C.c_int]),
     "spx_debug_xfade_check": (C.c_longlong, [C.c_int, C.c_int]),
     "spx_debug_arith_check": (C.c_longlong, [C.c_uint, C.c_uint, C.c_uint]),
diff --git a/speedy_amd/csrc/spx_analysis.hip b/speedy_amd/csrc/spx_analysis.hip
--- a/speedy_amd/csrc/spx_analysis.hip
+++ b/speedy_amd/csrc/spx_analysis.hip
@@ -1,6 +1,7 @@
 #include <stdlib.h>
 
 #include "spx_internal.h"
+#include "spx_tension_body.h"
 #include "spx_walk_common.h"
 
 #ifndef SPX_TF
@@ -436,12 +437,12 @@
 #ifndef SPX_AN_W_BIG
 #define SPX_AN_W_BIG 2
 #endif
-template <int TF, int WCT>
+template <int TF, int WCT, bool FIN = false>
 __global__ void __launch_bounds__(SPX_BLOCK, (WCT == 240 || WCT == 120 || WCT == 180) ? 4 : WCT == 330 ? SPX_AN_W_330 : (WCT == 661 || WCT == 720) ? SPX_AN_W_BIG : (WCT == 480 || WCT == 360) ? 2 : 1)
 spx_analysis_kernel(SpxPlanDev P, const SpxStreamDev* __restrict__ streams, int n_streams,
                     const int16_t* __restrict__ in_base, SpxFrameRec* __restrict__ rec, SpxTapsDev taps,
                     const int* __restrict__ tile_order, int* tile_flags, const float* __restrict__ frames,
-                    int frame_mode) {
+                    int frame_mode, SpxFinishDev fin) {
   extern __shared__ __attribute__((aligned(16))) unsigned char lds[];
   const int W = WCT ? WCT : P.W, B = P.B, N = 2 * W;
   const int tid = threadIdx.x, lane = tid & 63, wave = tid >> 6;
@@ -1296,6 +1297,34 @@
       __hip_atomic_store(&tile_flags[tile], 1, __ATOMIC_RELAXED, __HIP_MEMORY_SCOPE_AGENT);
     }
   }
+  if constexpr (FIN) {
+    static_assert(WCT != 0, "the finisher is built for the compiled-in window sizes");
+    float* sA = reinterpret_cast<float*>(lds);
+    float* sB = sA + SPX_CH;
+    int* sLast = reinterpret_cast<int*>(sB + SPX_CH);
+    asm volatile("s_waitcnt vmcnt(0)" ::: "memory");
+    __syncthreads();
+    int tile2 = (int)blockIdx.x;
+    asm volatile("" : "+s"(tile2));
+    if (tile_order) tile2 = tile_order[tile2];
+    int si = 0, hi2 = n_streams - 1;
+    while (si < hi2) {
+      const int mid = (si + hi2 + 1) >> 1;
+      if (streams[mid].first_tile <= tile2) si = mid; else hi2 = mid - 1;
+    }
+    if (tid == 0) {
+      __builtin_amdgcn_fence(__ATOMIC_RELEASE, "agent");
+      asm volatile("s_waitcnt vmcnt(0)" ::: "memory");
+      const int n_tiles = (streams[si].n_frames - streams[si].frame_begin + TF - 1) / TF;
+      const int done = __hip_atomic_fetch_add(&fin.tiles_done[si], 1, __ATOMIC_RELAXED, __HIP_MEMORY_SCOPE_AGENT) + 1;
+      if (done == n_tiles) __builtin_amdgcn_fence(__ATOMIC_ACQUIRE, "agent");
+      *sLast = done == n_tiles;
+    }
+    __syncthreads();
+    if (*sLast) {
+      spx_tension_stream(P, streams, si, fin.states, rec, fin.scratch, taps, nullptr, fin.speed_ready, sA, sB, sLast);
+    }
+  }
   ASTAMP(7);
   ASTAMP_FLUSH
 }
@@ -1368,13 +1397,20 @@
 
 void spx_launch_analysis(const SpxPlanDev& P, const SpxStreamDev* streams, int n_streams, int n_tiles,
                          const int16_t* in, SpxFrameRec* rec, SpxTapsDev taps, const int* tile_order, int* tile_flags,
-                         hipStream_t st) {
+                         hipStream_t st, const SpxFinishDev* fin) {
   if (n_tiles <= 0) return;
   const size_t lds = spx_analysis_lds_bytes(P);
   const int ctw = plan_ct_window(P);
+  if (fin != nullptr) {
+    if (!spx_analysis_can_finish(P) || tile_flags != nullptr) abort();
+    hipLaunchKernelGGL((spx_analysis_kernel<SPX_TF, 240, true>), dim3(n_tiles), dim3(SPX_BLOCK), lds, st, P, streams, n_streams, in,
+                       rec, taps, tile_order, (int*)nullptr, (const float*)nullptr, 0, *fin);
+    return;
+  }
+  const SpxFinishDev no_fin = {nullptr, nullptr, nullptr, nullptr};
 #define SPX_LAUNCH_ANALYSIS(TFV, WV)                                                                                   \
   hipLaunchKernelGGL((spx_analysis_kernel<TFV, WV>), dim3(n_tiles), dim3(SPX_BLOCK), lds, st, P, streams, n_streams, in, \
-                     rec, taps, tile_order, tile_flags, (const float*)nullptr, 0)
+                     rec, taps, tile_order, tile_flags, (const float*)nullptr, 0, no_fin)
   if (P.tile_frames == SPX_TF_TINY) {
     SPX_LAUNCH_ANALYSIS(SPX_TF_TINY, 0);
   } else if (P.tile_frames == SPX_TF_SMALL) {
@@ -1390,6 +1426,14 @@
     else SPX_LAUNCH_ANALYSIS(SPX_TF, 0);
   }
 #undef SPX_LAUNCH_ANALYSIS
+}
+
+bool spx_analysis_can_finish(const SpxPlanDev& P) {
+  return P.tile_frames == SPX_TF && plan_ct_window(P) == 240 &&
+         work_bytes(240, SPX_TF, true) >= 2 * SPX_CH * sizeof(float) + sizeof(int);
+}
+int spx_analysis_finisher_vgprs(int* scratch_bytes) {
+  return spx_kernel_vgprs(reinterpret_cast<const void*>(spx_analysis_kernel<SPX_TF, 240, true>), scratch_bytes);
 }
 
 int spx_analysis_vgprs(const SpxPlanDev& P, int* scratch_bytes) {
@@ -1414,13 +1458,14 @@
   SpxPlanDev Q = P;
   if (Q.tile_frames != SPX_TF_SMALL && Q.tile_frames != SPX_TF_TINY) Q.tile_frames = SPX_TF;
   const size_t lds = analysis_lds_bytes(Q, false);
+  const SpxFinishDev no_fin = {nullptr, nullptr, nullptr, nullptr};
   if (Q.tile_frames == SPX_TF_TINY)
     hipLaunchKernelGGL((spx_analysis_kernel<SPX_TF_TINY, 0>), dim3(n_tiles), dim3(SPX_BLOCK), lds, st, Q, streams, 1,
-                       (const int16_t*)nullptr, rec, taps, (const int*)nullptr, (int*)nullptr, frames, preemph ? 1 : 2);
+                       (const int16_t*)nullptr, rec, taps, (const int*)nullptr, (int*)nullptr, frames, preemph ? 1 : 2, no_fin);
   else if (Q.tile_frames == SPX_TF_SMALL)
     hipLaunchKernelGGL((spx_analysis_kernel<SPX_TF_SMALL, 0>), dim3(n_tiles), dim3(SPX_BLOCK), lds, st, Q, streams, 1,
-                       (const int16_t*)nullptr, rec, taps, (const int*)nullptr, (int*)nullptr, frames, preemph ? 1 : 2);
+                       (const int16_t*)nullptr, rec, taps, (const int*)nullptr, (int*)nullptr, frames, preemph ? 1 : 2, no_fin);
   else
     hipLaunchKernelGGL((spx_analysis_kernel<SPX_TF, 0>), dim3(n_tiles), dim3(SPX_BLOCK), lds, st, Q, streams, 1,
-                       (const int16_t*)nullptr, rec, taps, (const int*)nullptr, (int*)nullptr, frames, preemph ? 1 : 2);
-}
+                       (const int16_t*)nullptr, rec, taps, (const int*)nullptr, (int*)nullptr, frames, preemph ? 1 : 2, no_fin);
+}
diff --git a/speedy_amd/csrc/spx_diag.hip b/speedy_amd/csrc/spx_diag.hip
--- a/speedy_amd/csrc/spx_diag.hip
+++ b/speedy_amd/csrc/spx_diag.hip
@@ -29,6 +29,7 @@
 }
 
 int spx_debug_last_call_concurrent(void) { return g_last_concurrent.load(std::memory_order_relaxed); }
+int spx_debug_last_call_finisher(void) { return g_last_finisher.load(std::memory_order_relaxed); }
 int spx_debug_kernel_vgprs(int which) {
   if (which == 0) return spx_tension_vgprs();
   const int rate = (which == 2 || which == 4) ? 22050 : 16000;
diff --git a/speedy_amd/csrc/spx_engine.h b/speedy_amd/csrc/spx_engine.h
--- a/speedy_amd/csrc/spx_engine.h
+++ b/speedy_amd/csrc/spx_engine.h
@@ -103,6 +103,7 @@
 
 struct EvPair { hipEvent_t a, b; int kind; };
 extern std::atomic<bool> g_timing;
+extern std::atomic<int> g_last_finisher;
 extern std::atomic<int> g_last_concurrent;
 extern std::atomic<int> g_concurrent;
 extern std::atomic<bool> g_chunks_set;
diff --git a/speedy_amd/csrc/spx_engine.hip b/speedy_amd/csrc/spx_engine.hip
--- a/speedy_amd/csrc/spx_engine.hip
+++ b/speedy_amd/csrc/spx_engine.hip
@@ -10,6 +10,7 @@
 
 std::atomic<bool> g_timing{false};
 std::atomic<int> g_last_concurrent{0};
+std::atomic<int> g_last_finisher{0};
 std::atomic<int> g_concurrent{1};
 std::atomic<bool> g_chunks_set{false};
 std::atomic<int> g_chunks{1};
@@ -86,7 +87,7 @@
   L.max_tiles = tf / TFr + n + 1;
   L.off_order = o;   o += ((sizeof(int) * (size_t)L.max_tiles + 255) & ~(size_t)255);
   L.off_flags = o;   o += ((sizeof(int) * (size_t)L.max_tiles + 255) & ~(size_t)255);
-  L.off_ready = o;   o += ((sizeof(int) * ((size_t)n + 1) + 255) & ~(size_t)255);
+  L.off_ready = o;   o += ((sizeof(int) * (2 * (size_t)n + 1) + 255) & ~(size_t)255);
   L.total = o;
   return L;
 }
@@ -195,7 +196,10 @@
   return 0;
 }
 
-int walk_stream_count() { return 2; }
+#ifndef SPX_WALK_STREAMS
+#define SPX_WALK_STREAMS 2
+#endif
+int walk_stream_count() { return SPX_WALK_STREAMS; }
 int dev_walk_streams(int dev, hipStream_t* w, int n) {
   static std::mutex mu;
   static hipStream_t s3[64][SPX_MAX_WALK_STREAMS];
@@ -487,6 +491,11 @@
       for (int i = 0; i < n; i++)
         if (t < cnt[i]) order.push_back(sv[i].first_tile + t);
   }
+  bool finisher = ahead && M.walk2 && !force && do_a && do_w && nch == 1 && tiles[0] > 0 && spx_analysis_can_finish(d);
+  for (int i = 0; i < n && finisher; i++)
+    if (sv[i].nonlinear != 0.0f && sv[i].n_frames <= sv[i].frame_begin) finisher = false;
+  const SpxFinishDev fin = {d_ready + n + 1, states, scratch, d_ready};
+  if (do_a && do_w) g_last_finisher.store(finisher ? 1 : 0, std::memory_order_relaxed);
   bool waited_prev = false;
   if ((ahead || chunk_ahead) && !force) {
     if (ring_wait(plan, sa, ws, st, &waited_prev)) return -2;
@@ -497,7 +506,7 @@
   const bool ahead_gate = ahead && !force && plan->ahead_started != nullptr && plan->ahead_n > 0 && !waited_prev &&
                           ring_previous_in_flight(plan);
   rc = stage_tables(plan, sv, opt.rate ? opt.rate->table : order, dstreams, opt.rate ? reinterpret_cast<int*>(opt.rate->d_table) : d_order, d_flags, concurrent ? (unsigned)tiles[0] : 0u, d_ready,
-                    (concurrent || ahead) ? (unsigned)n + 1u : 0u, (ahead || chunk_ahead) ? sa : st, &staged_ev,
+                    (concurrent || ahead) ? (unsigned)n + 1u + (finisher ? (unsigned)n : 0u) : 0u, (ahead || chunk_ahead) ? sa : st, &staged_ev,
                     ahead_gate ? plan->ahead_started : nullptr, plan->ahead_n, 8000u);
   if (rc) return rc;
   if (M.trial_slot >= 0) {
@@ -515,19 +524,22 @@
       hipLaunchKernelGGL(spx_gate_kernel, dim3(1), dim3(64), 0, sa, d_ready + n, n, 1200u);
     if (do_a && tiles[c] > 0) {
       SpxTimed tm(timed, 0, sa);
-      spx_launch_analysis(d, dj, n, tiles[c], in, rec, td, concurrent ? d_order : nullptr, concurrent ? d_flags : nullptr, sa);
+      spx_launch_analysis(d, dj, n, tiles[c], in, rec, td, concurrent ? d_order : nullptr, concurrent ? d_flags : nullptr, sa,
+                          finisher ? &fin : nullptr);
     }
     if (force && force->after_analysis && c == nch - 1) HIPCHK(hipEventRecord(force->after_analysis, sa));
     if (sa != st) HIPCHK(hipEventRecord(plan->ev_chunk[c], sa));
     if (sa != st && !concurrent && !ahead) HIPCHK(hipStreamWaitEvent(st, plan->ev_chunk[c], 0));
     if (do_w) {
       hipStream_t stn = concurrent ? plan->side2 : (ahead ? sa : st);
-      {
+      if (finisher) {
+        HIPCHK(hipStreamWaitEvent(stw, plan->ev_chunk[c], 0));
+      } else {
         SpxTimed tm(timed, 2, stn);
         spx_launch_tension(d, dj, n, states, rec, scratch, td, concurrent ? d_flags : nullptr, (concurrent || ahead) ? d_ready : nullptr, stn);
       }
-      if (concurrent || ahead) HIPCHK(hipEventRecord(plan->ev_tension, stn));
-      if (ahead) HIPCHK(hipStreamWaitEvent(stw, plan->ev_tension, 0));
+      if ((concurrent || ahead) && !finisher) HIPCHK(hipEventRecord(plan->ev_tension, stn));
+      if (ahead && !finisher) HIPCHK(hipStreamWaitEvent(stw, plan->ev_tension, 0));
       {
         SpxTimed tm(timed, 1, stw);
         spx_launch_walk(d, dj, n, maxC, in, out, opt.rate ? opt.rate->d_tsm_n : n_out, states, scratch, (concurrent || ahead) ? d_ready : nullptr,
diff --git a/speedy_amd/csrc/spx_internal.h b/speedy_amd/csrc/spx_internal.h
--- a/speedy_amd/csrc/spx_internal.h
+++ b/speedy_amd/csrc/spx_internal.h
@@ -133,9 +133,17 @@
   float* normalized;
 };
 
+struct SpxFinishDev {
+  int* tiles_done;
+  SpxStreamState* states;
+  float* scratch;
+  int* speed_ready;
+};
 void spx_launch_analysis(const SpxPlanDev& P, const SpxStreamDev* streams, int n_streams, int n_tiles,
                          const int16_t* in, SpxFrameRec* rec, SpxTapsDev taps, const int* tile_order, int* tile_flags,
-                         hipStream_t st);
+                         hipStream_t st, const SpxFinishDev* fin = nullptr);
+bool spx_analysis_can_finish(const SpxPlanDev& P);
+int spx_analysis_finisher_vgprs(int* scratch_bytes = nullptr);
 void spx_launch_analysis_frames(const SpxPlanDev& P, const SpxStreamDev* streams, int n_tiles, const float* frames,
                                 bool preemph, SpxFrameRec* rec, SpxTapsDev taps, hipStream_t st);
 void spx_launch_tension(const SpxPlanDev& P, const SpxStreamDev* streams, int n_streams, SpxStreamState* states,
diff --git a/speedy_amd/csrc/spx_tension.hip b/speedy_amd/csrc/spx_tension.hip
--- a/speedy_amd/csrc/spx_tension.hip
+++ b/speedy_amd/csrc/spx_tension.hip
@@ -1,294 +1,14 @@
 #include "spx_internal.h"
-
-#define SPX_CH 512
-#ifndef SPX_TCH
-#define SPX_TCH 16
-#endif
-#define SPX_TENSION_THREADS 256
-
-__device__ __forceinline__ float iir_wave(const float* sA, float* sB, int n, float a, float b, float y) {
-  const int lane = threadIdx.x;
-  for (int b0 = 0; b0 < n; b0 += 64) {
-    const int m = n - b0 < 64 ? n - b0 : 64;
-    const float ax = a * ((lane < m) ? sA[b0 + lane] : 0.0f);
-#ifndef SPX_TENSION_OLD_CHAIN
-    if (m == 64) {
-      if (lane == 0) {
-#pragma unroll
-        for (int j = 0; j < 64; j++) {
-          const float s = __builtin_bit_cast(float, __builtin_amdgcn_readlane(__builtin_bit_cast(int, ax), j));
-          y = s + b * y;
-          sB[b0 + j] = y;
-        }
-      }
-      y = __builtin_bit_cast(float, __builtin_amdgcn_readfirstlane(__builtin_bit_cast(int, y)));
-      continue;
-    }
-#endif
-#ifndef SPX_TENSION_OLD_CHAIN
-    if (lane == 0) {
-#pragma unroll
-      for (int j = 0; j < 64; j++) {
-        if (j < m) {
-          const float s = __builtin_bit_cast(float, __builtin_amdgcn_readlane(__builtin_bit_cast(int, ax), j));
-          y = s + b * y;
-          sB[b0 + j] = y;
-        }
-      }
-    }
-    y = __builtin_bit_cast(float, __builtin_amdgcn_readfirstlane(__builtin_bit_cast(int, y)));
-#else
-    float out = 0.0f;
-#pragma unroll
-    for (int j = 0; j < 64; j++) {
-      if (j < m) {
-        const float s = __builtin_bit_cast(float, __builtin_amdgcn_readlane(__builtin_bit_cast(int, ax), j));
-        y = s + b * y;
-        out = (lane == j) ? y : out;
-      }
-    }
-    if (lane < m) sB[b0 + lane] = out;
-#endif
-  }
-  return y;
-}
+#include "spx_tension_body.h"
 
 __global__ void __launch_bounds__(SPX_TENSION_THREADS)
 spx_tension_kernel(SpxPlanDev P, const SpxStreamDev* __restrict__ streams, SpxStreamState* __restrict__ states,
                    const SpxFrameRec* __restrict__ rec_base, float* __restrict__ scratch_base, SpxTapsDev taps,
                    const int* tile_flags, int* speed_ready) {
-  constexpr int NT = SPX_TENSION_THREADS;
   __shared__ float sA[SPX_CH];
   __shared__ float sB[SPX_CH];
   __shared__ int sWait;
-  const int tid = threadIdx.x;
-  const SpxStreamDev S = streams[blockIdx.x];
-  const int Ttot = S.n_frames, F = P.F, Pp = P.Pp;
-  const int t0 = S.unit_time0 ? 0 : 1;
-  const float Rg = S.speed, nl = S.nonlinear, fb = S.feedback;
-  if (nl == 0.0f) return;
-
-  struct { float lp, lpf, cur_dur, des_dur; int first_k; } Z;
-  if (S.flags & SPX_F_INIT) {
-    Z.lp = 2.14204f;
-    Z.lpf = 123.837f;
-    Z.cur_dur = 0.0f; Z.des_dur = 0.0f;
-    Z.first_k = -1;
-  } else {
-    const SpxStreamState& in = states[blockIdx.x];
-    Z.lp = in.lp; Z.lpf = in.lpf; Z.cur_dur = in.cur_dur; Z.des_dur = in.des_dur;
-    Z.first_k = in.tension_first;
-  }
-  const SpxFrameRec* rec = rec_base + S.frame_off;
-  float* scr = scratch_base + (size_t)S.frame_off * 4;
-  const float lowthr = (float)(0.04 * (double)1.41421f);
-  float* tfeat = taps.features ? taps.features + (size_t)S.frame_off * SPX_FEATURE_COUNT : nullptr;
-
-  int fa_c = S.frame_begin;
-  int wch = SPX_TCH;
-  bool ok_all = true;
-  for (;;) {
-    int T_c = Ttot;
-    if (tile_flags != nullptr && Ttot - fa_c > wch) T_c = fa_c + wch;
-    const bool last = T_c >= Ttot;
-    if (tile_flags != nullptr && T_c > fa_c) {
-      const int TF = P.tile_frames;
-      const int i0 = (fa_c - S.frame_begin) / TF, i1 = (T_c - S.frame_begin + TF - 1) / TF;
-      if (tid == 0) {
-        int ok = 1;
-        for (int i = i0; i < i1 && ok; i++) {
-          unsigned spins = 0;
-          while (__hip_atomic_load(&tile_flags[S.first_tile + i], __ATOMIC_RELAXED, __HIP_MEMORY_SCOPE_AGENT) == 0) {
-            __builtin_amdgcn_s_sleep(32);
-            if (++spins > (1u << 22)) { ok = 0; break; }
-          }
-        }
-        __builtin_amdgcn_fence(__ATOMIC_ACQUIRE, "agent");
-        asm volatile("s_waitcnt vmcnt(0)" ::: "memory");
-        sWait = ok;
-      }
-      __syncthreads();
-      if (sWait == 0) { ok_all = false; break; }
-    }
-    const int fa = fa_c, T = T_c;
-    int K0 = (fa + t0 >= F) ? fa + t0 - F : 0;
-    if (K0 < S.tension_skip) K0 = S.tension_skip;
-    int K = (T + t0 >= F) ? T + t0 - F : 0;
-    if (S.flags & SPX_F_TENSION_RANGE) {
-      K0 = S.tension_skip;
-      if (K > S.tension_to) K = S.tension_to;
-    }
-    if (Z.first_k < 0 && K > K0) Z.first_k = K0;
-    const int first_k = Z.first_k;
-    if (T > fa || (S.flags & SPX_F_TENSION_RANGE)) {
-      float lp = Z.lp;
-      for (int c0 = fa; c0 < T; c0 += SPX_CH) {
-        const int n = min(SPX_CH, T - c0);
-        for (int i = tid; i < n; i += NT) sA[i] = rec[c0 + i].energy;
-        __syncthreads();
-        if (tid < 64) lp = iir_wave(sA, sB, n, P.one_minus_alpha, P.alpha, lp);
-        __syncthreads();
-        for (int i = tid; i < n; i += NT) {
-          const float e = sA[i], l = sB[i];
-          const float local = e / l;
-          const float comp = (float)__builtin_sqrt(local > 2 ? 2.0 : (double)local);
-          const int j = c0 + i;
-          scr[4 * j + 0] = comp;
-          const int k = j + t0 - F;
-          if (tfeat && k >= 0) {
-            float* f = tfeat + (size_t)k * SPX_FEATURE_COUNT;
-            f[1] = l; f[2] = local; f[3] = comp; f[12] = (float)(j + t0);
-          }
-        }
-        if (n > 0) lp = sB[n - 1];
-        __syncthreads();
-      }
-      Z.lp = lp;
-      for (int k = K0 + tid; k < K; k += NT) {
-        float future_max = 0.0f, past_max = 0.0f;
-        for (int i = 0; i <= F; i++) {
-          const int tau = k + i;
-          float v = (tau >= t0) ? scr[4 * (tau - t0) + 0] : 0.0f;
-          v *= P.taperF[i];
-          if (v > future_max) future_max = v;
-        }
-        for (int i = 0; i <= Pp; i++) {
-          const int tau = k - i;
-          float v = (tau >= t0) ? scr[4 * (tau - t0) + 0] : 0.0f;
-          v *= P.taperP[i];
-          if (v > past_max) past_max = v;
-        }
-        const float hyst = (float)((double)(past_max + future_max) / 2.0);
-        const float e_cur = (k < t0) ? 0.0f : rec[k - t0].energy;
-        const bool low = e_cur <= lowthr || k == first_k;
-        const float lsd = low ? 0.0f : rec[k - t0].lsd;
-        const float ewld = low ? 0.0f : lsd * hyst;
-        scr[4 * k + 1] = hyst;
-        scr[4 * k + 2] = ewld;
-        if (tfeat) {
-          float* f = tfeat + (size_t)k * SPX_FEATURE_COUNT;
-          f[0] = e_cur; f[4] = hyst; f[5] = low ? 1.0f : 0.0f; f[6] = lsd; f[7] = ewld;
-          f[13] = (float)k; f[14] = lowthr;
-        }
-      }
-      __syncthreads();
-      float lpf = Z.lpf;
-      for (int c0 = K0; c0 < K; c0 += SPX_CH) {
-        const int n = min(SPX_CH, K - c0);
-        for (int i = tid; i < n; i += NT) sA[i] = scr[4 * (c0 + i) + 2];
-        __syncthreads();
-        if (tid < 64) lpf = iir_wave(sA, sB, n, P.one_minus_alpha, P.alpha, lpf);
-        __syncthreads();
-        for (int i = tid; i < n; i += NT) {
-          const int k = c0 + i;
-          const float ewld = sA[i], l = sB[i];
-          const float hyst = scr[4 * k + 1];
-          const float e_cur = (k < t0) ? 0.0f : rec[k - t0].energy;
-          const bool low = e_cur <= lowthr || k == first_k;
-          float rel = 0.0f, sc = 0.0f;
-          if (!low) {
-            rel = (float)((double)ewld / ((double)l + 0.01 * (double)123.979f));
-            sc = (float)fmin((double)rel, (double)(4 * 0.971975f));
-          }
-          const float a = 0.5f, b = 0.25f, M_E_ = 0.7f, M_S = 1.0f;
-          const float tension = a * (hyst - M_E_) + b * (sc - M_S);
-          float v;
-          if ((double)Rg > 1.0) {
-            v = (float)fmax(1.0, (double)(Rg + (1 - Rg) * tension));
-          } else {
-            v = (float)fmax(0.01, fmin(1.0, (double)(Rg - (1 - Rg) * tension)));
-          }
-          scr[4 * k + 2] = tension;
-          scr[4 * k + 3] = v;
-          if (tfeat) {
-            float* f = tfeat + (size_t)k * SPX_FEATURE_COUNT;
-            f[8] = l; f[9] = rel; f[10] = sc; f[11] = tension;
-          }
-          if (taps.tension) taps.tension[S.frame_off + k] = tension;
-        }
-        if (n > 0) lpf = sB[n - 1];
-        __syncthreads();
-      }
-      Z.lpf = lpf;
-      float cur_dur = Z.cur_dur, des_dur = Z.des_dur;
-      const float fd = (float)(1.0 / 100.0);
-      for (int c0 = K0; c0 < ((S.flags & SPX_F_NO_SPEED) ? K0 : K); c0 += SPX_CH) {
-        const int n = min(SPX_CH, K - c0);
-        for (int i = tid; i < n; i += NT) sA[i] = scr[4 * (c0 + i) + 3];
-        __syncthreads();
-        if (!(fb > 0)) {
-          if (tid < 64) {
-            const float cstep = fd / Rg;
-            for (int b0 = 0; b0 < n; b0 += 64) {
-              const int m = n - b0 < 64 ? n - b0 : 64;
-              const float req = (tid < m) ? sA[b0 + tid] : 1.0f;
-              const float q = fd / req;
-              if (m == 64) {
-#pragma unroll
-                for (int j = 0; j < 64; j++) {
-                  cur_dur += __builtin_bit_cast(float, __builtin_amdgcn_readlane(__builtin_bit_cast(int, q), j));
-                  des_dur += cstep;
-                }
-              } else {
-#pragma unroll
-                for (int j = 0; j < 64; j++) {
-                  if (j < m) {
-                    cur_dur += __builtin_bit_cast(float, __builtin_amdgcn_readlane(__builtin_bit_cast(int, q), j));
-                    des_dur += cstep;
-                  }
-                }
-              }
-              if (tid < m) sB[b0 + tid] = req * nl + Rg * (1 - nl);
-            }
-            if (tid == 0) { sA[0] = cur_dur; sA[1] = des_dur; }
-          }
-        } else if (tid == 0) {
-          for (int i = 0; i < n; i++) {
-            float req = sA[i];
-            if (fb > 0) {
-              const float excess = cur_dur - des_dur;
-              req = (float)((double)req + fmax(0.01, (double)(fb * excess)));
-            }
-            cur_dur += fd / req;
-            des_dur += fd / Rg;
-            sB[i] = req * nl + Rg * (1 - nl);
-          }
-          sA[0] = cur_dur;
-          sA[1] = des_dur;
-        }
-        __syncthreads();
-        cur_dur = sA[0];
-        des_dur = sA[1];
-        for (int i = tid; i < n; i += NT) {
-          scr[4 * (c0 + i) + 3] = sB[i];
-          if (taps.speed) taps.speed[S.frame_off + c0 + i] = sB[i];
-        }
-        __syncthreads();
-      }
-      Z.cur_dur = cur_dur;
-      Z.des_dur = des_dur;
-    }
-    if (speed_ready != nullptr) {
-      asm volatile("s_waitcnt vmcnt(0)" ::: "memory");
-      __syncthreads();
-      if (tid == 0) {
-        __builtin_amdgcn_fence(__ATOMIC_RELEASE, "agent");
-        asm volatile("s_waitcnt vmcnt(0)" ::: "memory");
-        __hip_atomic_store(&speed_ready[blockIdx.x], K, __ATOMIC_RELAXED, __HIP_MEMORY_SCOPE_AGENT);
-      }
-    } else {
-      __syncthreads();
-    }
-    fa_c = T_c;
-    if (last) break;
-  }
-  if (!ok_all && speed_ready != nullptr && tid == 0)
-    __hip_atomic_store(&speed_ready[blockIdx.x], -1, __ATOMIC_RELAXED, __HIP_MEMORY_SCOPE_AGENT);
-  if (tid == 0) {
-    SpxStreamState& o = states[blockIdx.x];
-    o.lp = Z.lp; o.lpf = Z.lpf; o.cur_dur = Z.cur_dur; o.des_dur = Z.des_dur;
-    o.tension_first = Z.first_k;
-  }
+  spx_tension_stream(P, streams, blockIdx.x, states, rec_base, scratch_base, taps, tile_flags, speed_ready, sA, sB, &sWait);
 }
 
 size_t spx_tension_lds_bytes() { return sizeof(float) * 2 * SPX_CH + 64; }
diff --git a/speedy_amd/csrc/spx_tension_body.h b/speedy_amd/csrc/spx_tension_body.h
--- /dev/null
+++ b/speedy_amd/csrc/spx_tension_body.h
@@ -0,0 +1,290 @@
+#pragma once
+#include "spx_internal.h"
+
+#define SPX_CH 512
+#ifndef SPX_TCH
+#define SPX_TCH 16
+#endif
+#define SPX_TENSION_THREADS 256
+
+__device__ __forceinline__ float iir_wave(const float* sA, float* sB, int n, float a, float b, float y) {
+  const int lane = threadIdx.x;
+  for (int b0 = 0; b0 < n; b0 += 64) {
+    const int m = n - b0 < 64 ? n - b0 : 64;
+    const float ax = a * ((lane < m) ? sA[b0 + lane] : 0.0f);
+#ifndef SPX_TENSION_OLD_CHAIN
+    if (m == 64) {
+      if (lane == 0) {
+#pragma unroll
+        for (int j = 0; j < 64; j++) {
+          const float s = __builtin_bit_cast(float, __builtin_amdgcn_readlane(__builtin_bit_cast(int, ax), j));
+          y = s + b * y;
+          sB[b0 + j] = y;
+        }
+      }
+      y = __builtin_bit_cast(float, __builtin_amdgcn_readfirstlane(__builtin_bit_cast(int, y)));
+      continue;
+    }
+#endif
+#ifndef SPX_TENSION_OLD_CHAIN
+    if (lane == 0) {
+#pragma unroll
+      for (int j = 0; j < 64; j++) {
+        if (j < m) {
+          const float s = __builtin_bit_cast(float, __builtin_amdgcn_readlane(__builtin_bit_cast(int, ax), j));
+          y = s + b * y;
+          sB[b0 + j] = y;
+        }
+      }
+    }
+    y = __builtin_bit_cast(float, __builtin_amdgcn_readfirstlane(__builtin_bit_cast(int, y)));
+#else
+    float out = 0.0f;
+#pragma unroll
+    for (int j = 0; j < 64; j++) {
+      if (j < m) {
+        const float s = __builtin_bit_cast(float, __builtin_amdgcn_readlane(__builtin_bit_cast(int, ax), j));
+        y = s + b * y;
+        out = (lane == j) ? y : out;
+      }
+    }
+    if (lane < m) sB[b0 + lane] = out;
+#endif
+  }
+  return y;
+}
+
+__device__ __forceinline__ void spx_tension_stream(const SpxPlanDev& P, const SpxStreamDev* __restrict__ streams, int si,
+                                                   SpxStreamState* __restrict__ states, const SpxFrameRec* __restrict__ rec_base,
+                                                   float* __restrict__ scratch_base, const SpxTapsDev& taps, const int* tile_flags,
+                                                   int* speed_ready, float* sA, float* sB, int* sWait) {
+  constexpr int NT = SPX_TENSION_THREADS;
+  const int tid = threadIdx.x;
+  const SpxStreamDev S = streams[si];
+  const int Ttot = S.n_frames, F = P.F, Pp = P.Pp;
+  const int t0 = S.unit_time0 ? 0 : 1;
+  const float Rg = S.speed, nl = S.nonlinear, fb = S.feedback;
+  if (nl == 0.0f) return;
+
+  struct { float lp, lpf, cur_dur, des_dur; int first_k; } Z;
+  if (S.flags & SPX_F_INIT) {
+    Z.lp = 2.14204f;
+    Z.lpf = 123.837f;
+    Z.cur_dur = 0.0f; Z.des_dur = 0.0f;
+    Z.first_k = -1;
+  } else {
+    const SpxStreamState& in = states[si];
+    Z.lp = in.lp; Z.lpf = in.lpf; Z.cur_dur = in.cur_dur; Z.des_dur = in.des_dur;
+    Z.first_k = in.tension_first;
+  }
+  const SpxFrameRec* rec = rec_base + S.frame_off;
+  float* scr = scratch_base + (size_t)S.frame_off * 4;
+  const float lowthr = (float)(0.04 * (double)1.41421f);
+  float* tfeat = taps.features ? taps.features + (size_t)S.frame_off * SPX_FEATURE_COUNT : nullptr;
+
+  int fa_c = S.frame_begin;
+  int wch = SPX_TCH;
+  bool ok_all = true;
+  for (;;) {
+    int T_c = Ttot;
+    if (tile_flags != nullptr && Ttot - fa_c > wch) T_c = fa_c + wch;
+    const bool last = T_c >= Ttot;
+    if (tile_flags != nullptr && T_c > fa_c) {
+      const int TF = P.tile_frames;
+      const int i0 = (fa_c - S.frame_begin) / TF, i1 = (T_c - S.frame_begin + TF - 1) / TF;
+      if (tid == 0) {
+        int ok = 1;
+        for (int i = i0; i < i1 && ok; i++) {
+          unsigned spins = 0;
+          while (__hip_atomic_load(&tile_flags[S.first_tile + i], __ATOMIC_RELAXED, __HIP_MEMORY_SCOPE_AGENT) == 0) {
+            __builtin_amdgcn_s_sleep(32);
+            if (++spins > (1u << 22)) { ok = 0; break; }
+          }
+        }
+        __builtin_amdgcn_fence(__ATOMIC_ACQUIRE, "agent");
+        asm volatile("s_waitcnt vmcnt(0)" ::: "memory");
+        *sWait = ok;
+      }
+      __syncthreads();
+      if (*sWait == 0) { ok_all = false; break; }
+    }
+    const int fa = fa_c, T = T_c;
+    int K0 = (fa + t0 >= F) ? fa + t0 - F : 0;
+    if (K0 < S.tension_skip) K0 = S.tension_skip;
+    int K = (T + t0 >= F) ? T + t0 - F : 0;
+    if (S.flags & SPX_F_TENSION_RANGE) {
+      K0 = S.tension_skip;
+      if (K > S.tension_to) K = S.tension_to;
+    }
+    if (Z.first_k < 0 && K > K0) Z.first_k = K0;
+    const int first_k = Z.first_k;
+    if (T > fa || (S.flags & SPX_F_TENSION_RANGE)) {
+      float lp = Z.lp;
+      for (int c0 = fa; c0 < T; c0 += SPX_CH) {
+        const int n = min(SPX_CH, T - c0);
+        for (int i = tid; i < n; i += NT) sA[i] = rec[c0 + i].energy;
+        __syncthreads();
+        if (tid < 64) lp = iir_wave(sA, sB, n, P.one_minus_alpha, P.alpha, lp);
+        __syncthreads();
+        for (int i = tid; i < n; i += NT) {
+          const float e = sA[i], l = sB[i];
+          const float local = e / l;
+          const float comp = (float)__builtin_sqrt(local > 2 ? 2.0 : (double)local);
+          const int j = c0 + i;
+          scr[4 * j + 0] = comp;
+          const int k = j + t0 - F;
+          if (tfeat && k >= 0) {
+            float* f = tfeat + (size_t)k * SPX_FEATURE_COUNT;
+            f[1] = l; f[2] = local; f[3] = comp; f[12] = (float)(j + t0);
+          }
+        }
+        if (n > 0) lp = sB[n - 1];
+        __syncthreads();
+      }
+      Z.lp = lp;
+      for (int k = K0 + tid; k < K; k += NT) {
+        float future_max = 0.0f, past_max = 0.0f;
+        for (int i = 0; i <= F; i++) {
+          const int tau = k + i;
+          float v = (tau >= t0) ? scr[4 * (tau - t0) + 0] : 0.0f;
+          v *= P.taperF[i];
+          if (v > future_max) future_max = v;
+        }
+        for (int i = 0; i <= Pp; i++) {
+          const int tau = k - i;
+          float v = (tau >= t0) ? scr[4 * (tau - t0) + 0] : 0.0f;
+          v *= P.taperP[i];
+          if (v > past_max) past_max = v;
+        }
+        const float hyst = (float)((double)(past_max + future_max) / 2.0);
+        const float e_cur = (k < t0) ? 0.0f : rec[k - t0].energy;
+        const bool low = e_cur <= lowthr || k == first_k;
+        const float lsd = low ? 0.0f : rec[k - t0].lsd;
+        const float ewld = low ? 0.0f : lsd * hyst;
+        scr[4 * k + 1] = hyst;
+        scr[4 * k + 2] = ewld;
+        if (tfeat) {
+          float* f = tfeat + (size_t)k * SPX_FEATURE_COUNT;
+          f[0] = e_cur; f[4] = hyst; f[5] = low ? 1.0f : 0.0f; f[6] = lsd; f[7] = ewld;
+          f[13] = (float)k; f[14] = lowthr;
+        }
+      }
+      __syncthreads();
+      float lpf = Z.lpf;
+      for (int c0 = K0; c0 < K; c0 += SPX_CH) {
+        const int n = min(SPX_CH, K - c0);
+        for (int i = tid; i < n; i += NT) sA[i] = scr[4 * (c0 + i) + 2];
+        __syncthreads();
+        if (tid < 64) lpf = iir_wave(sA, sB, n, P.one_minus_alpha, P.alpha, lpf);
+        __syncthreads();
+        for (int i = tid; i < n; i += NT) {
+          const int k = c0 + i;
+          const float ewld = sA[i], l = sB[i];
+          const float hyst = scr[4 * k + 1];
+          const float e_cur = (k < t0) ? 0.0f : rec[k - t0].energy;
+          const bool low = e_cur <= lowthr || k == first_k;
+          float rel = 0.0f, sc = 0.0f;
+          if (!low) {
+            rel = (float)((double)ewld / ((double)l + 0.01 * (double)123.979f));
+            sc = (float)fmin((double)rel, (double)(4 * 0.971975f));
+          }
+          const float a = 0.5f, b = 0.25f, M_E_ = 0.7f, M_S = 1.0f;
+          const float tension = a * (hyst - M_E_) + b * (sc - M_S);
+          float v;
+          if ((double)Rg > 1.0) {
+            v = (float)fmax(1.0, (double)(Rg + (1 - Rg) * tension));
+          } else {
+            v = (float)fmax(0.01, fmin(1.0, (double)(Rg - (1 - Rg) * tension)));
+          }
+          scr[4 * k + 2] = tension;
+          scr[4 * k + 3] = v;
+          if (tfeat) {
+            float* f = tfeat + (size_t)k * SPX_FEATURE_COUNT;
+            f[8] = l; f[9] = rel; f[10] = sc; f[11] = tension;
+          }
+          if (taps.tension) taps.tension[S.frame_off + k] = tension;
+        }
+        if (n > 0) lpf = sB[n - 1];
+        __syncthreads();
+      }
+      Z.lpf = lpf;
+      float cur_dur = Z.cur_dur, des_dur = Z.des_dur;
+      const float fd = (float)(1.0 / 100.0);
+      for (int c0 = K0; c0 < ((S.flags & SPX_F_NO_SPEED) ? K0 : K); c0 += SPX_CH) {
+        const int n = min(SPX_CH, K - c0);
+        for (int i = tid; i < n; i += NT) sA[i] = scr[4 * (c0 + i) + 3];
+        __syncthreads();
+        if (!(fb > 0)) {
+          if (tid < 64) {
+            const float cstep = fd / Rg;
+            for (int b0 = 0; b0 < n; b0 += 64) {
+              const int m = n - b0 < 64 ? n - b0 : 64;
+              const float req = (tid < m) ? sA[b0 + tid] : 1.0f;
+              const float q = fd / req;
+              if (m == 64) {
+#pragma unroll
+                for (int j = 0; j < 64; j++) {
+                  cur_dur += __builtin_bit_cast(float, __builtin_amdgcn_readlane(__builtin_bit_cast(int, q), j));
+                  des_dur += cstep;
+                }
+              } else {
+#pragma unroll
+                for (int j = 0; j < 64; j++) {
+                  if (j < m) {
+                    cur_dur += __builtin_bit_cast(float, __builtin_amdgcn_readlane(__builtin_bit_cast(int, q), j));
+                    des_dur += cstep;
+                  }
+                }
+              }
+              if (tid < m) sB[b0 + tid] = req * nl + Rg * (1 - nl);
+            }
+            if (tid == 0) { sA[0] = cur_dur; sA[1] = des_dur; }
+          }
+        } else if (tid == 0) {
+          for (int i = 0; i < n; i++) {
+            float req = sA[i];
+            if (fb > 0) {
+              const float excess = cur_dur - des_dur;
+              req = (float)((double)req + fmax(0.01, (double)(fb * excess)));
+            }
+            cur_dur += fd / req;
+            des_dur += fd / Rg;
+            sB[i] = req * nl + Rg * (1 - nl);
+          }
+          sA[0] = cur_dur;
+          sA[1] = des_dur;
+        }
+        __syncthreads();
+        cur_dur = sA[0];
+        des_dur = sA[1];
+        for (int i = tid; i < n; i += NT) {
+          scr[4 * (c0 + i) + 3] = sB[i];
+          if (taps.speed) taps.speed[S.frame_off + c0 + i] = sB[i];
+        }
+        __syncthreads();
+      }
+      Z.cur_dur = cur_dur;
+      Z.des_dur = des_dur;
+    }
+    if (speed_ready != nullptr) {
+      asm volatile("s_waitcnt vmcnt(0)" ::: "memory");
+      __syncthreads();
+      if (tid == 0) {
+        __builtin_amdgcn_fence(__ATOMIC_RELEASE, "agent");
+        asm volatile("s_waitcnt vmcnt(0)" ::: "memory");
+        __hip_atomic_store(&speed_ready[si], K, __ATOMIC_RELAXED, __HIP_MEMORY_SCOPE_AGENT);
+      }
+    } else {
+      __syncthreads();
+    }
+    fa_c = T_c;
+    if (last) break;
+  }
+  if (!ok_all && speed_ready != nullptr && tid == 0)
+    __hip_atomic_store(&speed_ready[si], -1, __ATOMIC_RELAXED, __HIP_MEMORY_SCOPE_AGENT);
+  if (tid == 0) {
+    SpxStreamState& o = states[si];
+    o.lp = Z.lp; o.lpf = Z.lpf; o.cur_dur = Z.cur_dur; o.des_dur = Z.des_dur;
+    o.tension_first = Z.first_k;
+  }
+}
```

Measured after the change: 29320. 0.647x the previous value.
